# huawei-noah/Speech-Backbones

Measured on NVIDIA B200. Metric: mel-frames/sec at N=50 reverse-diffusion steps, higher is better.
Workload: dtype f32

## Files before the change

### speech-backbones_b200/csrc/sbk_api.cu

```cuda
#include "../../include/sbk.h"
#include "sbk_internal.h"

#include <cuda_fp16.h>
#include <math.h>
#include <stdarg.h>
#include <stdio.h>
#include <stdlib.h>
#include <string.h>

#include <algorithm>
#include <map>
#include <string>
#include <vector>

using namespace sbk;

static thread_local char g_err[1024] = "";
static int fail(int code, const char* fmt, ...) {
    va_list ap;
    va_start(ap, fmt);
    vsnprintf(g_err, sizeof(g_err), fmt, ap);
    va_end(ap);
    return code;
}
int sbk_set_error(int code, const char* fmt, ...) {
    va_list ap;
    va_start(ap, fmt);
    vsnprintf(g_err, sizeof(g_err), fmt, ap);
    va_end(ap);
    return code;
}
#define CU(x)                                                                                          \
    do {                                                                                               \
        cudaError_t e_ = (x);                                                                          \
        if (e_ != cudaSuccess)                                                                         \
            return fail(SBK_ERR_CUDA, "%s failed: %s (%s:%d)", #x, cudaGetErrorString(e_), __FILE__, __LINE__); \
    } while (0)

#define TRY_RC(x) do { int rc__ = (x); if (rc__ != SBK_OK) return rc__; } while (0)

namespace {

struct WSpec { std::string name; std::vector<int64_t> shape; };
struct ResnetInfo { std::string prefix; int cin, cout; };
struct AttnInfo { std::string prefix; int c; };

__global__ void k_set_int(int* p, int v) { *p = v; }
__global__ void k_set_ptr(const float** p, const float* v) { *p = v; }
__global__ void k_loop_cond(cudaGraphConditionalHandle handle, const int* step_next, const int* step_end) {
    cudaGraphSetConditional(handle, *step_next < *step_end ? 1u : 0u);
}

struct Arena {
    char* base = nullptr; size_t cap = 0, off = 0;
    void* take(size_t bytes) {
        off = (off + 255) & ~size_t(255);
        void* r = base ? base + off : nullptr;
        off += bytes;
        return r;
    }
};

enum OpKind { OP_FIRST, OP_IGEMM, OP_RESFINAL, OP_CTX, OP_MIX, OP_FINAL, OP_CONVTC, OP_GNACT };
struct Op {
    OpKind kind; std::string name;
    FirstConvParams fc; IgemmParams ig; ConvTcParams tc; GnActParams ga; ResFinalParams rf; AttnCtxParams cx; AttnMixParams mx; FinalParams fn;
    const float* dbg_ptr = nullptr; int64_t dbg_numel = 0;
    int dbg_fmt = 0;
    double flops = 0, bytes = 0;
    float* dbg_copy = nullptr;
};

struct Plan {
    int B = 0, T = 0, tb_rows = 0, noise_cap_steps = 0;
    void* mem = nullptr; size_t bytes = 0, cap = 0;
    std::vector<Op> ops;
    int final_op = -1;
    float *xt = nullptr, *mu = nullptr, *mask = nullptr, *spk_s = nullptr, *spk_in = nullptr;
    double* stats = nullptr; int n_stat_doubles = 0;
    float *tb = nullptr, *t_rows = nullptr; float4* coef = nullptr;
    int* step_cur = nullptr; int* step_next = nullptr;
    const float** noise_pp = nullptr;
    float *vc_cond = nullptr, *vc_wextra = nullptr, *vc_rextra = nullptr;
    int first_op = -1, first_res_op = -1;
    int tb_stride = 0;
    cudaGraphExec_t gexec[4] = {nullptr, nullptr, nullptr, nullptr};
    cudaGraphExec_t gloop[4] = {nullptr, nullptr, nullptr, nullptr};
    int loop_state[4] = {0, 0, 0, 0};
    int* step_end = nullptr;
    int launches_per_step = 0;
};

}

struct sbk_handle {
    sbk_config cfg;
    std::vector<WSpec> spec;
    std::vector<ResnetInfo> resnets;
    std::vector<AttnInfo> attns;
    std::map<std::string, float*> raw;
    std::map<std::string, float*> packed;
    std::vector<void*> owned;
    float* d_freqs = nullptr;
    float* d_zero = nullptr;
    void* ref_mem = nullptr; size_t ref_bytes = 0;
    bool is_packed = false;
    Plan plan;
    cudaStream_t cap_stream = nullptr;
    int64_t last_launches = 0;
    int last_host_launches = 0;
    bool capture = false;
    int tb_off[16];
    int tb_total = 0;
};

static void build_spec(sbk_handle* h) {
    const sbk_config& c = h->cfg;
    const int dim = c.dim;
    const bool vc = c.model == SBK_MODEL_DIFFVC;
    const int d[4] = {vc ? 2 + c.dim_cond : 2 + (c.n_spks > 1 ? 1 : 0), dim, dim * 2, dim * 4};
    auto add = [&](const std::string& n, std::vector<int64_t> s) { h->spec.push_back({n, s}); };
    auto resnet = [&](const std::string& p, int cin, int cout) {
        add(p + ".mlp.1.weight", {cout, dim});
        add(p + ".mlp.1.bias", {cout});
        const char* blk[2] = {"block1", "block2"};
        for (int k = 0; k < 2; ++k) {
            const int ci = k == 0 ? cin : cout;
            add(p + "." + blk[k] + ".block.0.weight", {cout, ci, 3, 3});
            add(p + "." + blk[k] + ".block.0.bias", {cout});
            add(p + "." + blk[k] + ".block.1.weight", {cout});
            add(p + "." + blk[k] + ".block.1.bias", {cout});
        }
        if (cin != cout) {
            add(p + ".res_conv.weight", {cout, cin, 1, 1});
            add(p + ".res_conv.bias", {cout});
        }
        h->resnets.push_back({p, cin, cout});
    };
    auto attn = [&](const std::string& p, int ch) {
        add(p + ".fn.g", {1});
        add(p + ".fn.fn.to_qkv.weight", {kAttnHidden * 3, ch, 1, 1});
        add(p + ".fn.fn.to_out.weight", {ch, kAttnHidden, 1, 1});
        add(p + ".fn.fn.to_out.bias", {ch});
        h->attns.push_back({p, ch});
    };
    if (c.n_spks > 1) {
        add("estimator.spk_mlp.0.weight", {c.spk_emb_dim * 4, c.spk_emb_dim});
        add("estimator.spk_mlp.0.bias", {c.spk_emb_dim * 4});
        add("estimator.spk_mlp.2.weight", {c.n_feats, c.spk_emb_dim * 4});
        add("estimator.spk_mlp.2.bias", {c.n_feats});
    }
    add("estimator.mlp.0.weight", {dim * 4, dim});
    add("estimator.mlp.0.bias", {dim * 4});
    add("estimator.mlp.2.weight", {dim, dim * 4});
    add("estimator.mlp.2.bias", {dim});
    if (vc) {
        const int dc = c.dim_cond, base = dc / 4;
        int cond_total = dim + 256;
        if (c.use_ref_t) {
            add("estimator.ref_block.mlp1.1.weight", {base, dim}); add("estimator.ref_block.mlp1.1.bias", {base});
            add("estimator.ref_block.mlp2.1.weight", {2 * base, dim}); add("estimator.ref_block.mlp2.1.bias", {2 * base});
            const char* nm[6] = {"block11", "block12", "block21", "block22", "block31", "block32"};
            const int ci[6] = {1, base, base, 2 * base, 2 * base, 4 * base}, co[6] = {2 * base, 2 * base, 4 * base, 4 * base, 8 * base, 8 * base};
            for (int k = 0; k < 6; ++k) {
                const std::string q = std::string("estimator.ref_block.") + nm[k];
                add(q + ".0.weight", {co[k], ci[k], 3, 3}); add(q + ".0.bias", {co[k]});
                add(q + ".1.weight", {co[k]}); add(q + ".1.bias", {co[k]});
            }
            add("estimator.ref_block.final_conv.weight", {dc, 4 * base, 1, 1});
            add("estimator.ref_block.final_conv.bias", {dc});
            cond_total += dc;
        }
        add("estimator.cond_block.0.weight", {4 * dc, cond_total}); add("estimator.cond_block.0.bias", {4 * dc});
        add("estimator.cond_block.2.weight", {dc, 4 * dc}); add("estimator.cond_block.2.bias", {dc});
    }
    for (int l = 0; l < 3; ++l) {
        const std::string p = "estimator.downs." + std::to_string(l);
        resnet(p + ".0", d[l], d[l + 1]);
        resnet(p + ".1", d[l + 1], d[l + 1]);
        attn(p + ".2", d[l + 1]);
        if (l < 2) {
            add(p + ".3.conv.weight", {d[l + 1], d[l + 1], 3, 3});
            add(p + ".3.conv.bias", {d[l + 1]});
        }
    }
    resnet("estimator.mid_block1", d[3], d[3]);
    attn("estimator.mid_attn", d[3]);
    resnet("estimator.mid_block2", d[3], d[3]);
    const int up_in[2] = {d[2], d[1]}, up_out[2] = {d[3], d[2]};
    for (int j = 0; j < 2; ++j) {
        const std::string p = "estimator.ups." + std::to_string(j);
        resnet(p + ".0", up_out[j] * 2, up_in[j]);
        resnet(p + ".1", up_in[j], up_in[j]);
        attn(p + ".2", up_in[j]);
        add(p + ".3.conv.weight", {up_in[j], up_in[j], 4, 4});
        add(p + ".3.conv.bias", {up_in[j]});
    }
    add("estimator.final_block.block.0.weight", {dim, dim, 3, 3});
    add("estimator.final_block.block.0.bias", {dim});
    add("estimator.final_block.block.1.weight", {dim});
    add("estimator.final_block.block.1.bias", {dim});
    add("estimator.final_conv.weight", {1, dim, 1, 1});
    add("estimator.final_conv.bias", {1});
    int off = 0;
    for (size_t k = 0; k < h->resnets.size(); ++k) { h->tb_off[k] = off; off += h->resnets[k].cout; }
    h->tb_total = off;
}

static int64_t numel_of(const std::vector<int64_t>& s) { int64_t n = 1; for (auto v : s) n *= v; return n; }

extern "C" const char* sbk_last_error(void) { return g_err; }
extern "C" const char* sbk_version(void) { return "sbk 0.1 (sm_100a)"; }

extern "C" int sbk_create(const sbk_config* cfg, sbk_handle** out) {
    if (!cfg || !out) return fail(SBK_ERR_ARG, "sbk_create: null argument");
    if (cfg->model != SBK_MODEL_GRADTTS && cfg->model != SBK_MODEL_DIFFVC) return fail(SBK_ERR_UNSUPPORTED, "sbk_create: model %d not supported", cfg->model);
    if (cfg->model == SBK_MODEL_DIFFVC && (cfg->dim_cond <= 0 || cfg->dim_cond % 4 != 0)) return fail(SBK_ERR_ARG, "sbk_create: DiffVC needs dim_cond > 0 (multiple of 4), got %d", cfg->dim_cond);
    if (cfg->model == SBK_MODEL_DIFFVC && cfg->use_ref_t && cfg->dim_cond % 128 != 0)
        return fail(SBK_ERR_ARG, "sbk_create: the native RefBlock needs dim_cond to be a multiple of 128 (its first conv writes 64-channel "
                                 "tiles and every conv reads 32-channel K stages), got %d", cfg->dim_cond);
    if (cfg->dim <= 0 || cfg->dim % 64 != 0) return fail(SBK_ERR_ARG, "sbk_create: dim must be a positive multiple of 64 (got %d)", cfg->dim);
    if (cfg->n_feats <= 0 || cfg->n_feats % 4 != 0) return fail(SBK_ERR_ARG, "sbk_create: n_feats must be a multiple of 4 (two stride-2 levels), got %d", cfg->n_feats);
    if (cfg->n_spks < 1 || cfg->spk_emb_dim <= 0) return fail(SBK_ERR_ARG, "sbk_create: bad speaker configuration");
    if (cfg->precision < SBK_PREC_FP32 || cfg->precision > SBK_PREC_FP32X3) return fail(SBK_ERR_ARG, "sbk_create: unknown precision %d", cfg->precision);
    sbk_handle* h = new sbk_handle();
    h->cfg = *cfg;
    build_spec(h);
    *out = h;
    return SBK_OK;
}

static void free_plan(sbk_handle* h, bool release_arena = true) {
    Plan& p = h->plan;
    for (int i = 0; i < 4; ++i) if (p.gexec[i]) { cudaGraphExecDestroy(p.gexec[i]); p.gexec[i] = nullptr; }
    for (int i = 0; i < 4; ++i) if (p.gloop[i]) { cudaGraphExecDestroy(p.gloop[i]); p.gloop[i] = nullptr; }
    for (auto& op : p.ops) if (op.dbg_copy) cudaFree(op.dbg_copy);
    void* mem = p.mem; const size_t cap = p.cap;
    if (mem && release_arena) { cudaFree(mem); mem = nullptr; }
    p = Plan();
    if (mem) { p.mem = mem; p.cap = cap; }
}

extern "C" void sbk_destroy(sbk_handle* h) {
    if (!h) return;
    free_plan(h);
    for (auto& kv : h->raw) cudaFree(kv.second);
    for (void* p : h->owned) cudaFree(p);
    if (h->ref_mem) cudaFree(h->ref_mem);
    if (h->cap_stream) cudaStreamDestroy(h->cap_stream);
    delete h;
}

extern "C" int sbk_num_weights(const sbk_handle* h) { return h ? (int)h->spec.size() : 0; }
extern "C" const char* sbk_weight_name(const sbk_handle* h, int i) {
    if (!h || i < 0 || i >= (int)h->spec.size()) return nullptr;
    return h->spec[i].name.c_str();
}

extern "C" int sbk_set_weight(sbk_handle* h, const char* name, const void* data, const int64_t* shape, int ndim) {
    if (!h || !name || !data || !shape) return fail(SBK_ERR_ARG, "sbk_set_weight: null argument");
    const WSpec* ws = nullptr;
    for (auto& s : h->spec) if (s.name == name) { ws = &s; break; }
    if (!ws) return fail(SBK_ERR_ARG, "sbk_set_weight: unexpected key '%s' (strict)", name);
    if ((int)ws->shape.size() != ndim) return fail(SBK_ERR_ARG, "sbk_set_weight: '%s' rank %d, expected %d", name, ndim, (int)ws->shape.size());
    for (int i = 0; i < ndim; ++i)
        if (ws->shape[i] != shape[i]) return fail(SBK_ERR_ARG, "sbk_set_weight: '%s' dim %d is %lld, expected %lld", name, i, (long long)shape[i], (long long)ws->shape[i]);
    CU(cudaSetDevice(h->cfg.device));
    const size_t bytes = numel_of(ws->shape) * sizeof(float);
    float*& dst = h->raw[name];
    if (!dst) CU(cudaMalloc(&dst, bytes));
    CU(cudaMemcpy(dst, data, bytes, cudaMemcpyDefault));
    h->is_packed = false;
    return SBK_OK;
}

template <class F>
static int repack(sbk_handle* h, const std::string& src, const std::string& key, size_t out_floats, F f) {
    const WSpec* ws = nullptr;
    for (auto& s : h->spec) if (s.name == src) { ws = &s; break; }
    if (!ws) return fail(SBK_ERR_STATE, "repack: no spec for %s", src.c_str());
    std::vector<float> hs(numel_of(ws->shape)), hd(out_floats);
    CU(cudaMemcpy(hs.data(), h->raw[src], hs.size() * sizeof(float), cudaMemcpyDeviceToHost));
    f(hd.data(), hs.data(), ws->shape);
    float*& d = h->packed[key];
    if (!d) { CU(cudaMalloc(&d, out_floats * sizeof(float))); h->owned.push_back(d); }
    CU(cudaMemcpy(d, hd.data(), out_floats * sizeof(float), cudaMemcpyHostToDevice));
    return SBK_OK;
}

static int attn_x3_chunk_items(int items_per_sample, int B) {
    (void)items_per_sample; (void)B;
    return 4;
}

static uint32_t f32_to_tf32_rna(float x) {
    uint32_t u; memcpy(&u, &x, 4);
    if ((u & 0x7F800000u) != 0x7F800000u) u += 0x1000u;
    return u & 0xFFFFE000u;
}
static uint16_t f32_to_f16_rn(float x) {
    if (x > 65504.f) x = 65504.f;
    if (x < -65504.f) x = -65504.f;
    const __half h = __float2half_rn(x);
    uint16_t u; memcpy(&u, &h, 2);
    return u;
}
static uint16_t f32_to_bf16_rn(float x) {
    uint32_t u; memcpy(&u, &x, 4);
    if ((u & 0x7FFFFFFFu) > 0x7F800000u) return (uint16_t)((u >> 16) | 0x40);
    u += 0x7FFFu + ((u >> 16) & 1u);
    return (uint16_t)(u >> 16);
}
static int pack_tc_host(sbk_handle* h, const std::vector<float>& hs, const std::string& key, int cout, int cin, int geom, bool bf16, int nt_override = 0);
static bool packs_x3(const sbk_handle* h) { return h->cfg.precision == SBK_PREC_FP32X3 || h->cfg.precision == SBK_PREC_FP32; }
static int pack_tc_rs(sbk_handle* h, const std::vector<float>& hs, const std::string& key, int cout, int cin, bool bf16) {
    const bool x3 = !bf16 && packs_x3(h);
    const int NT = 64, CPS = conv_tc_stage_channels(G_C3, bf16 ? 1 : 0), EPC = bf16 ? 8 : 4, KCHK = CPS / EPC, ksteps = cin / CPS;
    const size_t esz = bf16 ? 2 : 4, img = (size_t)3 * KCHK * 3 * NT * EPC;
    std::vector<uint8_t> hd((size_t)cout * cin * 9 * esz * (x3 ? 2 : 1));
    for (int nt = 0; nt < cout / NT; ++nt) for (int ks = 0; ks < ksteps; ++ks) for (int sx = 0; sx < 3; ++sx)
        for (int k = 0; k < KCHK; ++k) for (int kr = 0; kr < 3; ++kr) for (int col = 0; col < NT; ++col) for (int e = 0; e < EPC; ++e) {
            const int co = nt * NT + col, ci = ks * CPS + k * EPC + e;
            const float w = hs[((size_t)co * cin + ci) * 9 + kr * 3 + sx];
            const size_t in_img = ((((size_t)sx * KCHK + k) * 3 + (2 - kr)) * NT + col) * EPC + e;
            const size_t stage = ((size_t)nt * ksteps + ks) * (x3 ? 2 : 1);
            if (x3) {
                const uint32_t uh = f32_to_tf32_rna(w);
                float fh; memcpy(&fh, &uh, 4);
                reinterpret_cast<uint32_t*>(hd.data())[stage * img + in_img] = uh;
                uint16_t* cc = reinterpret_cast<uint16_t*>(hd.data()) + 2 * ((stage + 1) * img + in_img - e);
                cc[e] = f32_to_f16_rn(w);
                cc[4 + e] = f32_to_f16_rn((w - fh) * 4096.f);
            } else if (bf16) {
                reinterpret_cast<uint16_t*>(hd.data())[stage * img + in_img] = f32_to_bf16_rn(w);
            } else {
                reinterpret_cast<uint32_t*>(hd.data())[stage * img + in_img] = f32_to_tf32_rna(w);
            }
        }
    float*& d = h->packed[key];
    if (!d) { CU(cudaMalloc(&d, hd.size())); h->owned.push_back(d); }
    CU(cudaMemcpy(d, hd.data(), hd.size(), cudaMemcpyHostToDevice));
    return SBK_OK;
}
static int pack_tc(sbk_handle* h, const std::string& src, const std::string& key, int cout, int cin, int geom, bool bf16) {
    const int taps = conv_tc_taps(geom);
    std::vector<float> hs((size_t)cout * cin * taps);
    CU(cudaMemcpy(hs.data(), h->raw[src], hs.size() * sizeof(float), cudaMemcpyDeviceToHost));
    TRY_RC(pack_tc_host(h, hs, key, cout, cin, geom, bf16));
    if (geom == G_C3 && conv_tc_ntile(geom, cout) == 128) TRY_RC(pack_tc_host(h, hs, key + "64", cout, cin, geom, bf16, 64));
    if (geom == G_C3 && conv_tc_ntile(geom, cout) == 64) TRY_RC(pack_tc_host(h, hs, key + "32", cout, cin, geom, bf16, 32));
    if (geom == G_C3 && conv_tc_ntile(geom, cout) == 64) TRY_RC(pack_tc_rs(h, hs, key + "rs", cout, cin, bf16));
    return SBK_OK;
}
static int pack_tc_kv(sbk_handle* h, const std::string& src, const std::string& key, int C, bool bf16) {
    std::vector<float> q((size_t)384 * C);
    CU(cudaMemcpy(q.data(), h->raw[src], q.size() * sizeof(float), cudaMemcpyDeviceToHost));
    const int EPC = bf16 ? 8 : 4, CPS = 8 * EPC;
    std::vector<uint8_t> m((size_t)256 * C * (bf16 ? 2 : 4));
    for (int ks = 0; ks < C / CPS; ++ks) for (int kv = 0; kv < 2; ++kv) for (int k = 0; k < 8; ++k)
        for (int row = 0; row < 128; ++row) for (int e = 0; e < EPC; ++e) {
            const size_t idx = ((((size_t)ks * 2 + kv) * 8 + k) * 128 + row) * EPC + e;
            const float w = q[(size_t)(128 + kv * 128 + row) * C + ks * CPS + k * EPC + e];
            if (bf16) reinterpret_cast<uint16_t*>(m.data())[idx] = f32_to_bf16_rn(w);
            else reinterpret_cast<uint32_t*>(m.data())[idx] = f32_to_tf32_rna(w);
        }
    float*& d = h->packed[key];
    if (!d) { CU(cudaMalloc(&d, m.size())); h->owned.push_back(d); }
    CU(cudaMemcpy(d, m.data(), m.size(), cudaMemcpyHostToDevice));
    return SBK_OK;
}
static int pack_tc_kvx(sbk_handle* h, const std::string& src, const std::string& key, int C) {
    std::vector<float> q((size_t)384 * C);
    CU(cudaMemcpy(q.data(), h->raw[src], q.size() * sizeof(float), cudaMemcpyDeviceToHost));
    std::vector<uint8_t> m((size_t)2 * 256 * C * 4);
    for (int ks = 0; ks < C / 32; ++ks) for (int kv = 0; kv < 2; ++kv) for (int k = 0; k < 8; ++k)
        for (int row = 0; row < 128; ++row) for (int e = 0; e < 4; ++e) {
            const size_t chunk_hi = (((((size_t)ks * 2 + 0) * 2 + kv) * 8 + k) * 128 + row) * 4;
            const size_t chunk_c = (((((size_t)ks * 2 + 1) * 2 + kv) * 8 + k) * 128 + row) * 4;
            const float w = q[(size_t)(128 + kv * 128 + row) * C + ks * 32 + k * 4 + e];
            const uint32_t uh = f32_to_tf32_rna(w);
            float fh; memcpy(&fh, &uh, 4);
            reinterpret_cast<uint32_t*>(m.data())[chunk_hi + e] = uh;
            uint16_t* cc = reinterpret_cast<uint16_t*>(m.data()) + 2 * chunk_c;
            cc[e] = f32_to_f16_rn(w);
            cc[4 + e] = f32_to_f16_rn((w - fh) * 4096.f);
        }
    float*& d = h->packed[key];
    if (!d) { CU(cudaMalloc(&d, m.size())); h->owned.push_back(d); }
    CU(cudaMemcpy(d, m.data(), m.size(), cudaMemcpyHostToDevice));
    return SBK_OK;
}
static int pack_tc_up(sbk_handle* h, const std::string& src, const std::string& key, int C, bool bf16) {
    std::vector<float> w((size_t)C * C * 16), m((size_t)C * C * 16);
    CU(cudaMemcpy(w.data(), h->raw[src], w.size() * sizeof(float), cudaMemcpyDeviceToHost));
    for (int ci = 0; ci < C; ++ci) for (int co = 0; co < C; ++co) for (int t = 0; t < 16; ++t)
        m[((size_t)co * C + ci) * 16 + t] = w[((size_t)ci * C + co) * 16 + t];
    return pack_tc_host(h, m, key, C, C, G_UP, bf16);
}
static int pack_tc_host(sbk_handle* h, const std::vector<float>& hs, const std::string& key, int cout, int cin, int geom, bool bf16, int nt_override) {
    const int taps = conv_tc_taps(geom);
    const bool x3 = !bf16 && packs_x3(h);
    const int NT = nt_override ? nt_override : (x3 ? conv_tc_ntile_x3(geom, cout) : conv_tc_ntile(geom, cout)), CPS = conv_tc_stage_channels(geom, bf16 ? 1 : 0), EPC = bf16 ? 8 : 4, KCHK = CPS / EPC;
    const int ksteps = cin / CPS;
    const size_t esz = bf16 ? 2 : 4;
    std::vector<uint8_t> hd((size_t)cout * cin * taps * esz * (x3 ? 2 : 1));
    for (int nt = 0; nt < cout / NT; ++nt) for (int ks = 0; ks < ksteps; ++ks) for (int tap = 0; tap < taps; ++tap)
        for (int k = 0; k < KCHK; ++k) for (int col = 0; col < NT; ++col) for (int e = 0; e < EPC; ++e) {
            const int co = nt * NT + col, ci = ks * CPS + k * EPC + e;
            const float w = hs[((size_t)co * cin + ci) * taps + tap];
            if (x3) {
                const size_t ih = ((((((size_t)nt * ksteps + ks) * 2) * taps + tap) * KCHK + k) * NT + col) * EPC + e;
                const uint32_t uh = f32_to_tf32_rna(w);
                float fh; memcpy(&fh, &uh, 4);
                reinterpret_cast<uint32_t*>(hd.data())[ih] = uh;
                uint16_t* cc = reinterpret_cast<uint16_t*>(hd.data()) + 2 * ((ih - e) + (size_t)taps * KCHK * NT * EPC);
                cc[e] = f32_to_f16_rn(w);
                cc[4 + e] = f32_to_f16_rn((w - fh) * 4096.f);
                continue;
            }
            const size_t idx = (((((size_t)nt * ksteps + ks) * taps + tap) * KCHK + k) * NT + col) * EPC + e;
            if (bf16) reinterpret_cast<uint16_t*>(hd.data())[idx] = f32_to_bf16_rn(w);
            else reinterpret_cast<uint32_t*>(hd.data())[idx] = f32_to_tf32_rna(w);
        }
    float*& d = h->packed[key];
    if (!d) { CU(cudaMalloc(&d, hd.size())); h->owned.push_back(d); }
    CU(cudaMemcpy(d, hd.data(), hd.size(), cudaMemcpyHostToDevice));
    return SBK_OK;
}

#define TRY(x) do { int rc_ = (x); if (rc_ != SBK_OK) return rc_; } while (0)

extern "C" int sbk_pack(sbk_handle* h) {
    if (!h) return fail(SBK_ERR_ARG, "sbk_pack: null handle");
    for (auto& s : h->spec)
        if (!h->raw.count(s.name)) return fail(SBK_ERR_STATE, "sbk_pack: missing key '%s' (strict)", s.name.c_str());
    CU(cudaSetDevice(h->cfg.device));
    auto conv_pack = [](float* d, const float* s, const std::vector<int64_t>& sh) {
        const int64_t co = sh[0], ci = sh[1], kk = sh[2] * sh[3];
        for (int64_t o = 0; o < co; ++o) for (int64_t i = 0; i < ci; ++i) for (int64_t t = 0; t < kk; ++t)
            d[(t * ci + i) * co + o] = s[(o * ci + i) * kk + t];
    };
    auto convt_pack = [](float* d, const float* s, const std::vector<int64_t>& sh) {
        const int64_t ci = sh[0], co = sh[1], kk = sh[2] * sh[3];
        for (int64_t i = 0; i < ci; ++i) for (int64_t o = 0; o < co; ++o) for (int64_t t = 0; t < kk; ++t)
            d[(t * ci + i) * co + o] = s[(i * co + o) * kk + t];
    };
    auto first_pack = [](float* d, const float* s, const std::vector<int64_t>& sh) {
        const int64_t co = sh[0], ci = sh[1];
        for (int64_t o = 0; o < co; ++o) for (int64_t i = 0; i < ci; ++i) for (int64_t t = 0; t < 9; ++t)
            d[(i * 9 + t) * co + o] = s[(o * ci + i) * 9 + t];
    };
    auto kv_pack = [](float* d, const float* s, const std::vector<int64_t>& sh) {
        const int64_t C = sh[1];
        for (int64_t ci = 0; ci < C; ++ci) for (int hd = 0; hd < kHeads; ++hd) for (int x = 0; x < 32; ++x) {
            d[ci * 256 + hd * 64 + x] = s[(128 + hd * 32 + x) * C + ci];
            d[ci * 256 + hd * 64 + 32 + x] = s[(256 + hd * 32 + x) * C + ci];
        }
    };
    for (size_t k = 0; k < h->resnets.size(); ++k) {
        const ResnetInfo& r = h->resnets[k];
        if (k == 0) TRY(repack(h, r.prefix + ".block1.block.0.weight", r.prefix + ".block1.w", (size_t)r.cin * 9 * r.cout, first_pack));
        else TRY(repack(h, r.prefix + ".block1.block.0.weight", r.prefix + ".block1.w", (size_t)r.cin * 9 * r.cout, conv_pack));
        TRY(repack(h, r.prefix + ".block2.block.0.weight", r.prefix + ".block2.w", (size_t)r.cout * 9 * r.cout, conv_pack));
        if (r.cin != r.cout) TRY(repack(h, r.prefix + ".res_conv.weight", r.prefix + ".res.w", (size_t)r.cin * r.cout, conv_pack));
    }
    const bool x3 = h->cfg.precision == SBK_PREC_FP32X3;
    if (h->cfg.precision != SBK_PREC_FP32) {
        const bool bf = h->cfg.precision == SBK_PREC_BF16;
        const int cps3 = conv_tc_stage_channels(G_C3, bf ? 1 : 0), cps1 = conv_tc_stage_channels(G_PW, bf ? 1 : 0);
        for (auto& r : h->resnets) {
            if (r.cin % cps3 == 0) TRY(pack_tc(h, r.prefix + ".block1.block.0.weight", r.prefix + ".block1.wtc", r.cout, r.cin, G_C3, bf));
            TRY(pack_tc(h, r.prefix + ".block2.block.0.weight", r.prefix + ".block2.wtc", r.cout, r.cout, G_C3, bf));
            if (r.cin != r.cout && r.cin % cps1 == 0) TRY(pack_tc(h, r.prefix + ".res_conv.weight", r.prefix + ".res.wtc", r.cout, r.cin, G_PW, bf));
        }
        TRY(pack_tc(h, "estimator.final_block.block.0.weight", "estimator.final_block.wtc", h->cfg.dim, h->cfg.dim, G_C3, bf));
        for (auto& a : h->attns)
            if (a.c % cps1 == 0) {
                if (x3) TRY(pack_tc_kvx(h, a.prefix + ".fn.fn.to_qkv.weight", a.prefix + ".kvx.wtc", a.c));
                else TRY(pack_tc_kv(h, a.prefix + ".fn.fn.to_qkv.weight", a.prefix + ".kv.wtc", a.c, bf));
            }
        for (int l = 0; l < 2; ++l) {
            const std::string p = "estimator.downs." + std::to_string(l) + ".3.conv";
            TRY(pack_tc(h, p + ".weight", p + ".wtc", h->cfg.dim << l, h->cfg.dim << l, G_DOWN, bf));
        }
        for (int j = 0; j < 2; ++j) {
            const std::string p = "estimator.ups." + std::to_string(j) + ".3.conv";
            TRY(pack_tc_up(h, p + ".weight", p + ".wtc", h->cfg.dim << (1 - j), bf));
        }
    }
    if (h->cfg.model == SBK_MODEL_DIFFVC && h->cfg.use_ref_t) {
        const int base = h->cfg.dim_cond / 4;
        const char* nm[5] = {"block12", "block21", "block22", "block31", "block32"};
        const int ci[5] = {base, base, 2 * base, 2 * base, 4 * base}, co[5] = {2 * base, 4 * base, 4 * base, 8 * base, 8 * base};
        for (int k = 0; k < 5; ++k) {
            const std::string q = std::string("estimator.ref_block.") + nm[k];
            TRY(pack_tc(h, q + ".0.weight", q + ".wtc", co[k], ci[k], G_C3, false));
        }
        TRY(repack(h, "estimator.ref_block.block11.0.weight", "estimator.ref_block.block11.w", (size_t)9 * 2 * base, first_pack));
    }
    for (auto& a : h->attns) TRY(repack(h, a.prefix + ".fn.fn.to_qkv.weight", a.prefix + ".kv.w", (size_t)a.c * 256, kv_pack));
    for (int l = 0; l < 2; ++l) {
        const std::string p = "estimator.downs." + std::to_string(l) + ".3.conv";
        const int c = h->cfg.dim << l;
        TRY(repack(h, p + ".weight", p + ".w", (size_t)c * c * 9, conv_pack));
    }
    for (int j = 0; j < 2; ++j) {
        const std::string p = "estimator.ups." + std::to_string(j) + ".3.conv";
        const int c = h->cfg.dim << (1 - j);
        TRY(repack(h, p + ".weight", p + ".w", (size_t)c * c * 16, convt_pack));
    }
    TRY(repack(h, "estimator.final_block.block.0.weight", "estimator.final_block.w", (size_t)h->cfg.dim * h->cfg.dim * 9, conv_pack));
    {
        const int half = h->cfg.dim / 2;
        std::vector<float> f(half);
        const float neg = (float)(-(log(10000.0) / (double)(half - 1)));
        for (int j = 0; j < half; ++j) f[j] = expf((float)j * neg);
        if (!h->d_freqs) { CU(cudaMalloc(&h->d_freqs, half * sizeof(float))); h->owned.push_back(h->d_freqs); }
        CU(cudaMemcpy(h->d_freqs, f.data(), half * sizeof(float), cudaMemcpyHostToDevice));
    }
    if (!h->d_zero) {
        CU(cudaMalloc(&h->d_zero, 8192));
        h->owned.push_back(h->d_zero);
        CU(cudaMemset(h->d_zero, 0, 8192));
    }
    free_plan(h, false);
    h->is_packed = true;
    return SBK_OK;
}

namespace {
struct Bufs {
    float *A[3], *Bf[3], *X[3], *Y[3], *S[3], *D[3], *U1;
    float *kv_part, *ctx, *w_eff, *b_eff;
    std::map<const void*, float*> lo;
};
}

static size_t layout(const sbk_handle* h, int B, int T, int tb_rows, Arena& ar, Bufs* bf, Plan* pl) {
    const sbk_config& c = h->cfg;
    const int dim = c.dim, H = c.n_feats;
    const size_t P[3] = {(size_t)H * T, (size_t)(H / 2) * (T / 2), (size_t)(H / 4) * (T / 4)};
    const int C[3] = {dim, dim * 2, dim * 4};
    auto f = [&](size_t n) { return (float*)ar.take(n * sizeof(float)); };
    const size_t osz = c.precision == SBK_PREC_BF16 ? 2 : 4;
    const bool x3 = c.precision == SBK_PREC_FP32X3;
    Bufs b{};
    auto fo = [&](size_t n) {
        float* r = (float*)ar.take(n * osz);
        if (x3) { float* l = (float*)ar.take(n * osz); if (r) b.lo[r] = l; }
        return r;
    };
    for (int l = 0; l < 3; ++l) {
        const size_t n = (size_t)B * P[l] * C[l];
        b.A[l] = f(n); b.Bf[l] = fo(n); b.X[l] = fo(n); b.Y[l] = fo(n);
        b.S[l] = l > 0 ? fo(n) : nullptr;
        b.D[l] = l > 0 ? fo((size_t)B * P[l] * C[l - 1]) : nullptr;
    }
    b.U1 = fo((size_t)B * P[1] * C[1]);
    size_t mt0 = (P[0] + 127) / 128;
    if (x3) {
        mt0 = 0;
        for (int l = 0; l < 3; ++l) {
            const int items = (int)((P[l] + attn_kv_x3_item_pixels() - 1) / attn_kv_x3_item_pixels());
            const int ci = attn_x3_chunk_items(items, B);
            mt0 = std::max(mt0, (size_t)((items + ci - 1) / ci));
        }
    }
    b.kv_part = f((size_t)B * mt0 * kHeads * kKvPartFloats);
    b.ctx = f((size_t)B * kHeads * 1024);
    b.w_eff = f((size_t)B * C[2] * C[2] * (x3 ? 2 : 1));
    b.b_eff = f(C[2]);
    if (bf) *bf = b;
    Plan dummy;
    Plan& p = pl ? *pl : dummy;
    p.xt = f((size_t)B * H * T); p.mu = f((size_t)B * H * T); p.mask = f((size_t)B * T);
    p.spk_s = f((size_t)B * H); p.spk_in = f((size_t)B * c.spk_emb_dim);
    p.n_stat_doubles = 25 * B * kGroups * 2;
    p.stats = (double*)ar.take(p.n_stat_doubles * sizeof(double));
    p.tb_stride = h->tb_total;
    p.tb = f((size_t)tb_rows * h->tb_total);
    p.t_rows = f(tb_rows);
    p.coef = (float4*)ar.take((size_t)tb_rows * sizeof(float4));
    p.step_cur = (int*)ar.take(sizeof(int));
    p.step_next = (int*)ar.take(sizeof(int));
    p.step_end = (int*)ar.take(sizeof(int));
    p.noise_pp = (const float**)ar.take(sizeof(float*));
    if (c.model == SBK_MODEL_DIFFVC) {
        p.vc_cond = f((size_t)tb_rows * B * c.dim_cond);
        p.vc_wextra = f((size_t)tb_rows * B * 9 * dim);
        p.vc_rextra = f((size_t)tb_rows * B * dim);
    }
    return ar.off + 256;
}

static int table_rows(int B, int n_timesteps) { const int r = B > n_timesteps ? B : n_timesteps; return r < 64 ? 64 : r; }

extern "C" size_t sbk_workspace_bytes_n(const sbk_handle* h, int B, int T, int n_timesteps) {
    if (!h || B <= 0 || T <= 0 || T % 4 != 0 || n_timesteps < 1) return 0;
    Arena ar;
    return layout(h, B, T, table_rows(B, n_timesteps), ar, nullptr, nullptr);
}
extern "C" size_t sbk_workspace_bytes(const sbk_handle* h, int B, int T) { return sbk_workspace_bytes_n(h, B, T, 1024); }

static int build_plan(sbk_handle* h, int B, int T, int tb_rows) {
    free_plan(h, false);
    Plan& pl = h->plan;
    const sbk_config& c = h->cfg;
    Arena probe;
    const size_t bytes = layout(h, B, T, tb_rows, probe, nullptr, nullptr);
    if (bytes > pl.cap) {
        if (pl.mem) { cudaFree(pl.mem); pl.mem = nullptr; pl.cap = 0; }
        const cudaError_t e = cudaMalloc(&pl.mem, bytes);
        if (e != cudaSuccess) {
            pl.mem = nullptr;
            cudaGetLastError();
            return fail(SBK_ERR_CUDA, "out of memory: the (B=%d, T=%d) workspace needs %zu bytes (%s); free cached blocks "
                                      "(torch.cuda.empty_cache()) or split the batch", B, T, bytes, cudaGetErrorString(e));
        }
        pl.cap = bytes;
    }
    pl.bytes = bytes;
    Arena ar; ar.base = (char*)pl.mem; ar.cap = bytes;
    Bufs bf;
    layout(h, B, T, tb_rows, ar, &bf, &pl);
    pl.B = B; pl.T = T; pl.tb_rows = tb_rows;

    const int dim = c.dim, H0 = c.n_feats;
    const int Hs[3] = {H0, H0 / 2, H0 / 4}, Ws[3] = {T, T / 2, T / 4};
    const bool vc = c.model == SBK_MODEL_DIFFVC;
    const int cin0 = vc ? 3 : 2 + (c.n_spks > 1 ? 1 : 0);
    int gn_slot = 0;
    auto stats_slot = [&]() { return pl.stats + (size_t)(gn_slot++) * B * kGroups * 2; };
    auto W = [&](const std::string& k) -> const float* {
        auto it = h->packed.find(k);
        if (it != h->packed.end()) return it->second;
        auto it2 = h->raw.find(k);
        return it2 != h->raw.end() ? it2->second : nullptr;
    };
    auto gnref = [&](const double* st, const std::string& blk, int C, int lvl) {
        GnRef g; g.stats = st; g.gamma = W(blk + ".block.1.weight"); g.beta = W(blk + ".block.1.bias");
        g.inv_count = 1.0f / ((float)(C / kGroups) * (float)Hs[lvl] * (float)Ws[lvl]);
        return g;
    };
    auto base_ig = [&](int geom, int lvl_in, int lvl_out) {
        IgemmParams p; memset(&p, 0, sizeof(p));
        p.geom = geom; p.B = B; p.T = T;
        p.Hin = Hs[lvl_in]; p.Win = Ws[lvl_in]; p.Hout = Hs[lvl_out]; p.Wout = Ws[lvl_out];
        p.in_lvl = lvl_in; p.out_lvl = lvl_out; p.mask = pl.mask; p.step = pl.step_cur;
        return p;
    };
    const bool use_tc = c.precision != SBK_PREC_FP32;
    const bool x3 = c.precision == SBK_PREC_FP32X3;
    auto LO = [&](const void* q) -> float* { auto it = bf.lo.find(q); return it == bf.lo.end() ? nullptr : it->second; };
    int num_sms = 148;
    cudaDeviceGetAttribute(&num_sms, cudaDevAttrMultiProcessorCount, c.device);
    const bool b16 = c.precision == SBK_PREC_BF16;
    const double osz = b16 ? 2.0 : 4.0;
    const int fmt_raw = use_tc ? 1 : 0, fmt_opnd = b16 ? 2 : fmt_raw;
    const int tc_cps3 = conv_tc_stage_channels(G_C3, b16 ? 1 : 0), tc_cps1 = conv_tc_stage_channels(G_PW, b16 ? 1 : 0);
    auto push = [&](Op& op, const float* dbg, int64_t numel) {
        op.dbg_ptr = dbg; op.dbg_numel = numel;
        const bool raw_out = op.kind == OP_FIRST || op.kind == OP_CTX || (op.kind == OP_CONVTC && op.tc.geom == G_C3) ||
                             (op.kind == OP_IGEMM && op.ig.epi == EPI_PLAIN && op.ig.ostats);
        op.dbg_fmt = raw_out ? fmt_raw : fmt_opnd;
        if (op.kind == OP_IGEMM) {
            const IgemmParams& p = op.ig;
            const double cin = p.c0 + p.c1, opx = (double)B * p.Hout * p.Wout, ipx = (double)B * p.Hin * p.Win;
            const double taps = p.geom == G_PW ? 1 : (p.geom == G_UP ? 4 : 9);
            op.flops = 2.0 * opx * p.Cout * cin * taps;
            op.bytes = 4.0 * (ipx * cin + (p.epi == EPI_KV ? 0.0 : opx * p.Cout) + (p.epi == EPI_RES ? opx * p.Cout : 0.0));
        } else if (op.kind == OP_FIRST) {
            op.flops = 2.0 * B * H0 * T * op.fc.C * op.fc.cin * 9;
            op.bytes = 4.0 * B * H0 * T * (op.fc.cin + op.fc.C);
        } else if (op.kind == OP_RESFINAL) {
            op.bytes = (4.0 + (op.rf.x ? osz : 0.0) + osz) * B * op.rf.H * op.rf.W * op.rf.C;
        } else if (op.kind == OP_FINAL) {
            op.flops = 2.0 * B * H0 * T * op.fn.C;
            op.bytes = 4.0 * B * H0 * T * (op.fn.C + 3.0);
        }
        pl.ops.push_back(op);
    };
    auto npix = [&](int lvl) { return (int64_t)B * Hs[lvl] * Ws[lvl]; };

    auto tc_conv = [&](const std::string& name, int geom, const std::string& wkey, const std::string& bkey, int lvl,
                       const float* in0, int c0, const float* in1, int c1, int cout, float* out, double* st) {
        Op op; op.name = name; op.kind = OP_CONVTC;
        ConvTcParams& p = op.tc; memset(&p, 0, sizeof(p));
        p.geom = geom; p.in0 = in0; p.c0 = c0; p.in1 = in1; p.c1 = c1; p.H = Hs[lvl]; p.W = Ws[lvl]; p.B = B;
        p.Ho = p.H; p.Wo = p.W;
        p.wpk = W(wkey); p.bias = bkey.empty() ? nullptr : W(bkey); p.out = out; p.Cout = cout;
        p.epi = EPI_PLAIN; p.ostats = st; p.mask = pl.mask; p.T = T; p.lvl = lvl; p.zero_page = h->d_zero;
        p.bf16 = b16 ? 1 : 0;
        if (x3) {
            p.x3 = 1; p.in0_lo = LO(in0); p.in1_lo = LO(in1); p.out_lo = geom != G_C3 ? LO(out) : nullptr;
            static const int flush_env = getenv("SBK_X3_FLUSH") ? atoi(getenv("SBK_X3_FLUSH")) : 0;
            p.flush = flush_env;
        }
        if (geom == G_C3 && conv_tc_ntile(geom, cout) == 128 && getenv("SBK_FORCE_PAIR") == nullptr) {
            const long long tiles = (long long)B * ((Ws[lvl] + 127) / 128) * ((Hs[lvl] + 1) / 2) * (cout / 128);
            if (tiles * 2 <= num_sms && h->packed.count(wkey + "64")) { p.nt = 64; p.wpk = W(wkey + "64"); }
        }
        if (geom == G_C3 && conv_tc_ntile(geom, cout) == 64 && h->packed.count(wkey + "rs") && getenv("SBK_FORCE_PAIR") == nullptr &&
            ((!x3 && getenv("SBK_NO_RS") == nullptr) || getenv("SBK_FORCE_RS") != nullptr)) {
            p.rs = 1; p.wpk = W(wkey + "rs");
        }
        if (geom == G_C3 && !p.nt && !p.rs) {
            const bool no_pair = getenv("SBK_NO_PAIR") != nullptr, force_pair = getenv("SBK_FORCE_PAIR") != nullptr;
            const int ntile = conv_tc_ntile(geom, cout);
            const std::string half = wkey + (ntile == 128 ? "64" : "32");
            const long long ptiles = (long long)B * conv_tc_pair_tiles(Hs[lvl], Ws[lvl]) * (cout / ntile);
            if (!no_pair && h->packed.count(half) && (force_pair || (!b16 && ptiles >= num_sms / 2))) { p.pair = 1; p.wpk = W(half); }
        }
        const double taps = geom == G_PW ? 1.0 : (geom == G_UP ? 4.0 : 9.0);
        op.flops = 2.0 * B * Hs[lvl] * Ws[lvl] * cout * (c0 + c1) * taps;
        op.bytes = (double)B * Hs[lvl] * Ws[lvl] * (osz * (c0 + c1) + (geom == G_C3 ? 4.0 : osz) * cout);
        return op;
    };
    auto ffma_block_conv = [&](const std::string& name, const std::string& wkey, const std::string& bkey, int lvl,
                               const float* in0, int c0, const float* in1, int c1, int cout, float* out, double* st,
                               int pro, const GnRef* pgn, int tb_k) {
        Op op; op.name = name; op.kind = OP_IGEMM;
        op.ig = base_ig(G_C3, lvl, lvl);
        IgemmParams& p = op.ig;
        p.in0 = in0; p.c0 = c0; p.in1 = in1; p.c1 = c1; p.w = W(wkey); p.bias = W(bkey);
        p.out = out; p.Cout = cout; p.pro = pro; p.epi = EPI_PLAIN; p.ostats = st;
        if (pgn) { p.pgn = *pgn; p.tb = pl.tb + h->tb_off[tb_k]; p.tb_stride = pl.tb_stride; }
        push(op, out, npix(lvl) * cout);
    };
    auto resnet = [&](int k, int lvl, const float* in0, int c0, const float* in1, int c1, float* out, bool store_masked) {
        const ResnetInfo& r = h->resnets[k];
        float* A = bf.A[lvl]; float* Bb = bf.Bf[lvl];
        double* st1 = stats_slot(); double* st2 = stats_slot();
        const bool tc1 = use_tc && k != 0 && (c0 + c1) % tc_cps3 == 0 && c0 % tc_cps3 == 0;
        if (k == 0) {
            Op op; op.kind = OP_FIRST; op.name = r.prefix + ".block1.raw";
            FirstConvParams& p = op.fc; memset(&p, 0, sizeof(p));
            p.mu = pl.mu; p.xt = pl.xt; p.spk_s = pl.spk_s; p.mask = pl.mask;
            p.w = W(r.prefix + ".block1.w"); p.bias = W(r.prefix + ".block1.block.0.bias");
            p.out = A; p.ostats = st1; p.B = B; p.H = H0; p.T = T; p.cin = cin0; p.C = r.cout; p.chw4 = use_tc ? 1 : 0;
            if (vc) { p.w_extra = pl.vc_wextra; p.step = pl.step_cur; }
            pl.first_op = (int)pl.ops.size();
            push(op, A, npix(lvl) * r.cout);
        } else if (tc1) {
            Op op = tc_conv(r.prefix + ".block1.raw", G_C3, r.prefix + ".block1.wtc", r.prefix + ".block1.block.0.bias", lvl,
                            in0, c0, in1, c1, r.cout, A, st1);
            push(op, A, npix(lvl) * r.cout);
        } else {
            ffma_block_conv(r.prefix + ".block1.raw", r.prefix + ".block1.w", r.prefix + ".block1.block.0.bias", lvl,
                            in0, c0, in1, c1, r.cout, A, st1, PRO_MASK, nullptr, k);
        }
        const GnRef g1 = gnref(st1, r.prefix + ".block1", r.cout, lvl);
        float* h2 = Bb;
        if (use_tc) {
            {
                Op op; op.kind = OP_GNACT; op.name = r.prefix + ".block1.act";
                GnActParams& p = op.ga; memset(&p, 0, sizeof(p));
                p.raw = A; p.gn = g1; p.tb = pl.tb + h->tb_off[k]; p.tb_stride = pl.tb_stride; p.step = pl.step_cur;
                p.mask = pl.mask; p.T = T; p.lvl = lvl; p.out = Bb; p.B = B; p.H = Hs[lvl]; p.W = Ws[lvl]; p.C = r.cout;
                p.round_tf32 = (b16 || x3) ? 0 : 1; p.chw4 = 1; p.out_bf16 = b16 ? 1 : 0; p.out_lo = LO(Bb);
                op.bytes = (4.0 + osz) * npix(lvl) * r.cout;
                push(op, nullptr, 0);
            }
            Op op = tc_conv(r.prefix + ".block2.raw", G_C3, r.prefix + ".block2.wtc", r.prefix + ".block2.block.0.bias", lvl,
                            Bb, r.cout, nullptr, 0, r.cout, A, st2);
            push(op, A, npix(lvl) * r.cout);
            h2 = A;
        } else {
            ffma_block_conv(r.prefix + ".block2.raw", r.prefix + ".block2.w", r.prefix + ".block2.block.0.bias", lvl,
                            A, r.cout, nullptr, 0, r.cout, Bb, st2, PRO_GN, &g1, k);
        }
        const GnRef g2 = gnref(st2, r.prefix + ".block2", r.cout, lvl);
        if (k == 0 || r.cin == r.cout) {
            Op op; op.kind = OP_RESFINAL; op.name = r.prefix + ".out";
            ResFinalParams& p = op.rf; memset(&p, 0, sizeof(p));
            p.h2raw = h2; p.gn = g2;
            p.mask = pl.mask; p.T = T; p.lvl = lvl; p.out = out; p.B = B; p.H = Hs[lvl]; p.W = Ws[lvl]; p.C = r.cout;
            p.out_mask = store_masked ? 1 : 0; p.chw4 = use_tc ? 1 : 0; p.bf16 = b16 ? 1 : 0; p.out_lo = LO(out);
            if (k == 0) {
                p.x = nullptr; p.mu = pl.mu; p.xt = pl.xt; p.spk_s = pl.spk_s; p.cin = cin0;
                p.wres = W(r.prefix + ".res.w"); p.bres = W(r.prefix + ".res_conv.bias");
                if (vc) { p.r_extra = pl.vc_rextra; p.step = pl.step_cur; }
                pl.first_res_op = (int)pl.ops.size();
            } else {
                p.x = in0;
            }
            op.bytes = (4.0 + (k == 0 ? 0.0 : osz) + osz) * npix(lvl) * r.cout;
            push(op, out, npix(lvl) * r.cout);
        } else if (use_tc && (c0 + c1) % tc_cps1 == 0 && c0 % tc_cps1 == 0) {
            Op op = tc_conv(r.prefix + ".out", G_PW, r.prefix + ".res.wtc", r.prefix + ".res_conv.bias", lvl,
                            in0, c0, in1, c1, r.cout, out, nullptr);
            op.tc.epi = EPI_RES; op.tc.rraw = h2; op.tc.rgn = g2; op.tc.out_mask = store_masked ? 1 : 0;
            op.bytes += 4.0 * npix(lvl) * r.cout;
            push(op, out, npix(lvl) * r.cout);
        } else {
            Op op; op.kind = OP_IGEMM; op.name = r.prefix + ".out";
            op.ig = base_ig(G_PW, lvl, lvl);
            IgemmParams& p = op.ig;
            p.in0 = in0; p.c0 = c0; p.in1 = in1; p.c1 = c1;
            p.w = W(r.prefix + ".res.w"); p.bias = W(r.prefix + ".res_conv.bias");
            p.out = out; p.Cout = r.cout; p.pro = PRO_MASK; p.epi = EPI_RES;
            p.rraw = h2; p.rgn = g2; p.out_mask = store_masked ? 1 : 0;
            push(op, out, npix(lvl) * r.cout);
        }
    };
    auto attention = [&](int k, int lvl, const float* x, float* out) {
        const AttnInfo& a = h->attns[k];
        int mt = igemm_mtiles(G_PW, Hs[lvl], Ws[lvl], Hs[lvl], Ws[lvl]);
        const bool tc_apply = use_tc && a.c % tc_cps1 == 0;
        if (tc_apply && x3) {
            Op op = tc_conv(a.prefix + ".kvpart", G_PW, a.prefix + ".kvx.wtc", "", lvl, x, a.c, nullptr, 0, 256, nullptr, nullptr);
            const int items = (Hs[lvl] * Ws[lvl] + attn_kv_x3_item_pixels() - 1) / attn_kv_x3_item_pixels();
            const int chunk_items = attn_x3_chunk_items(items, B);
            mt = (items + chunk_items - 1) / chunk_items;
            op.tc.epi = EPI_KV; op.tc.kv_part = bf.kv_part; op.tc.Ho = chunk_items; op.tc.Wo = mt;
            op.bytes = 8.0 * npix(lvl) * a.c;
            op.flops += 2.0 * npix(lvl) * 4096.0;
            push(op, nullptr, 0);
        } else if (tc_apply) {
            Op op = tc_conv(a.prefix + ".kvpart", G_PW, a.prefix + ".kv.wtc", "", lvl, x, a.c, nullptr, 0, 256, nullptr, nullptr);
            op.tc.epi = EPI_KV; op.tc.kv_part = bf.kv_part;
            op.bytes = osz * npix(lvl) * a.c;
            op.flops += 2.0 * npix(lvl) * 4096.0;
            mt = (Hs[lvl] * Ws[lvl] + attn_kv_tile_pixels() - 1) / attn_kv_tile_pixels();
            push(op, nullptr, 0);
        } else {
            Op op; op.kind = OP_IGEMM; op.name = a.prefix + ".kvpart";
            op.ig = base_ig(G_PW, lvl, lvl);
            IgemmParams& p = op.ig;
            p.in0 = x; p.c0 = a.c; p.w = W(a.prefix + ".kv.w"); p.Cout = 256; p.pro = PRO_NONE; p.epi = EPI_KV;
            p.kv_part = bf.kv_part; p.out = nullptr;
            push(op, nullptr, 0);
        }
        {
            Op op; op.kind = OP_CTX; op.name = a.prefix + ".ctx";
            op.cx.kv_part = bf.kv_part; op.cx.mtiles = mt; op.cx.ctx = bf.ctx; op.cx.B = B;
            push(op, bf.ctx, (int64_t)B * kHeads * 1024);
        }
        {
            Op op; op.kind = OP_MIX; op.name = a.prefix + ".mix";
            AttnMixParams& p = op.mx; memset(&p, 0, sizeof(p));
            p.ctx = bf.ctx; p.wq = W(a.prefix + ".fn.fn.to_qkv.weight"); p.wout = W(a.prefix + ".fn.fn.to_out.weight");
            p.bout = W(a.prefix + ".fn.fn.to_out.bias"); p.g = W(a.prefix + ".fn.g");
            p.w_eff = bf.w_eff; p.b_eff = bf.b_eff; p.B = B; p.C = a.c;
            if (tc_apply) { p.tc_nt = x3 ? conv_tc_ntile_x3(G_PW, a.c) : conv_tc_ntile(G_PW, a.c); p.tc_cps = tc_cps1; p.tc_bf16 = b16 ? 1 : 0; p.tc_x3 = x3 ? 1 : 0; }
            push(op, nullptr, 0);
        }
        if (tc_apply) {
            Op op = tc_conv(a.prefix + ".out", G_PW, "", "", lvl, x, a.c, nullptr, 0, a.c, out, nullptr);
            op.tc.wpk = bf.w_eff; op.tc.w_bstride_bytes = (long long)a.c * a.c * (b16 ? 2 : (x3 ? 8 : 4)); op.tc.bias = bf.b_eff;
            op.tc.out_mask = 1; op.tc.addin = x;
            op.bytes += osz * npix(lvl) * a.c;
            push(op, out, npix(lvl) * a.c);
        } else {
            Op op; op.kind = OP_IGEMM; op.name = a.prefix + ".out";
            op.ig = base_ig(G_PW, lvl, lvl);
            IgemmParams& p = op.ig;
            p.in0 = x; p.c0 = a.c; p.w = bf.w_eff; p.w_bstride = (long long)a.c * a.c; p.bias = bf.b_eff;
            p.out = out; p.Cout = a.c; p.pro = PRO_NONE; p.epi = EPI_PLAIN; p.out_mask = use_tc ? 1 : 0;
            push(op, out, npix(lvl) * a.c);
        }
    };
    auto resample = [&](int geom, const std::string& pre, int lvl_in, int lvl_out, const float* x, int C, float* out) {
        if (use_tc && C % tc_cps3 == 0 && C % 64 == 0) {
            Op op = tc_conv(pre + ".out", geom, pre + ".conv.wtc", pre + ".conv.bias", lvl_in, x, C, nullptr, 0, C, out, nullptr);
            op.tc.Ho = Hs[lvl_out]; op.tc.Wo = Ws[lvl_out]; op.tc.lvl = lvl_out; op.tc.out_mask = 1;
            op.flops = 2.0 * npix(lvl_out) * C * C * (geom == G_UP ? 4.0 : 9.0);
            op.bytes = osz * C * (npix(lvl_in) + npix(lvl_out));
            push(op, out, npix(lvl_out) * C);
            return;
        }
        Op op; op.kind = OP_IGEMM; op.name = pre + ".out";
        op.ig = base_ig(geom, lvl_in, lvl_out);
        IgemmParams& p = op.ig;
        p.in0 = x; p.c0 = C; p.w = W(pre + ".conv.w"); p.bias = W(pre + ".conv.bias");
        p.out = out; p.Cout = C; p.pro = PRO_MASK; p.epi = EPI_PLAIN; p.out_mask = use_tc ? 1 : 0;
        push(op, out, npix(lvl_out) * C);
    };

    const int C1 = dim, C2 = dim * 2, C3 = dim * 4;
    const bool sm = use_tc;
    resnet(0, 0, nullptr, cin0, nullptr, 0, bf.X[0], sm);
    resnet(1, 0, bf.X[0], C1, nullptr, 0, bf.Y[0], false);
    attention(0, 0, bf.Y[0], bf.X[0]);
    resample(G_DOWN, "estimator.downs.0.3", 0, 1, bf.X[0], C1, bf.D[1]);
    resnet(2, 1, bf.D[1], C1, nullptr, 0, bf.X[1], sm);
    resnet(3, 1, bf.X[1], C2, nullptr, 0, bf.Y[1], false);
    attention(1, 1, bf.Y[1], bf.S[1]);
    resample(G_DOWN, "estimator.downs.1.3", 1, 2, bf.S[1], C2, bf.D[2]);
    resnet(4, 2, bf.D[2], C2, nullptr, 0, bf.X[2], sm);
    resnet(5, 2, bf.X[2], C3, nullptr, 0, bf.Y[2], false);
    attention(2, 2, bf.Y[2], bf.S[2]);
    resnet(6, 2, bf.S[2], C3, nullptr, 0, bf.X[2], false);
    attention(3, 2, bf.X[2], bf.Y[2]);
    resnet(7, 2, bf.Y[2], C3, nullptr, 0, bf.X[2], sm);
    resnet(8, 2, bf.X[2], C3, bf.S[2], C3, bf.Y[2], sm);
    resnet(9, 2, bf.Y[2], C2, nullptr, 0, bf.X[2], false);
    attention(4, 2, bf.X[2], bf.Y[2]);
    resample(G_UP, "estimator.ups.0.3", 2, 1, bf.Y[2], C2, bf.U1);
    resnet(10, 1, bf.U1, C2, bf.S[1], C2, bf.X[1], sm);
    resnet(11, 1, bf.X[1], C1, nullptr, 0, bf.Y[1], false);
    attention(5, 1, bf.Y[1], bf.X[1]);
    resample(G_UP, "estimator.ups.1.3", 1, 0, bf.X[1], C1, bf.Y[0]);
    double* stf = stats_slot();
    if (use_tc) {
        Op op = tc_conv("estimator.final_block.raw", G_C3, "estimator.final_block.wtc", "estimator.final_block.block.0.bias", 0,
                        bf.Y[0], C1, nullptr, 0, C1, bf.A[0], stf);
        push(op, bf.A[0], npix(0) * C1);
    } else {
        ffma_block_conv("estimator.final_block.raw", "estimator.final_block.w", "estimator.final_block.block.0.bias", 0,
                        bf.Y[0], C1, nullptr, 0, C1, bf.A[0], stf, PRO_MASK, nullptr, 0);
    }
    {
        Op op; op.kind = OP_FINAL; op.name = "estimator.out";
        FinalParams& p = op.fn; memset(&p, 0, sizeof(p));
        p.raw = bf.A[0]; p.gn = gnref(stf, "estimator.final_block", C1, 0);
        p.wfin = W("estimator.final_conv.weight"); p.bfin = W("estimator.final_conv.bias");
        p.mask = pl.mask; p.mu = pl.mu; p.xt_in = pl.xt; p.xt_out = pl.xt;
        p.coef = pl.coef; p.step = pl.step_cur; p.B = B; p.H = H0; p.T = T; p.C = C1; p.chw4 = use_tc ? 1 : 0; p.exact = x3 ? 1 : 0;
        pl.final_op = (int)pl.ops.size();
        push(op, nullptr, 0);
    }
    pl.launches_per_step = (int)pl.ops.size() + 1;
    return SBK_OK;
}

static int launch_op(const Op& op, cudaStream_t s) {
    switch (op.kind) {
        case OP_FIRST: return launch_first_conv(op.fc, s);
        case OP_IGEMM: return launch_igemm(op.ig, s);
        case OP_RESFINAL: return launch_resfinal(op.rf, s);
        case OP_CTX: return launch_attn_ctx(op.cx, s);
        case OP_MIX: return launch_attn_mix(op.mx, s);
        case OP_FINAL: return launch_final(op.fn, s);
        case OP_CONVTC: return launch_conv_tc(op.tc, s);
        case OP_GNACT: return launch_gn_act(op.ga, s);
    }
    return -1;
}

static int run_ops(sbk_handle* h, cudaStream_t s) {
    Plan& pl = h->plan;
    StepBeginParams sb{pl.stats, pl.n_stat_doubles, pl.step_cur, pl.step_next};
    int n = launch_step_begin(sb, s);
    for (auto& op : pl.ops) {
        const int k = launch_op(op, s);
        if (k < 0) { fail(SBK_ERR_CUDA, "launch of '%s' was refused (device attribute / layout)", op.name.c_str()); return -1; }
        n += k;
        if (h->capture && op.dbg_ptr && op.dbg_numel > 0) {
            const size_t esz = op.dbg_fmt == 2 ? 2 : 4;
            if (!op.dbg_copy) cudaMalloc(&op.dbg_copy, op.dbg_numel * esz);
            cudaMemcpyAsync(op.dbg_copy, op.dbg_ptr, op.dbg_numel * esz, cudaMemcpyDeviceToDevice, s);
        }
    }
    return n;
}

static int ensure_plan(sbk_handle* h, int B, int T, int rows) {
    if (!h->is_packed) return fail(SBK_ERR_STATE, "weights not packed: call sbk_set_weight for every key, then sbk_pack");
    if (B <= 0 || T <= 0 || T % 4 != 0) return fail(SBK_ERR_ARG, "B must be > 0 and T a positive multiple of 4 (fix_len_compatibility), got B=%d T=%d", B, T);
    CU(cudaSetDevice(h->cfg.device));
    Plan& pl = h->plan;
    if (pl.mem && pl.B == B && pl.T == T && pl.tb_rows >= rows) return SBK_OK;
    int cap = rows < 64 ? 64 : rows;
    if (pl.mem && pl.B == B && pl.T == T && cap < pl.tb_rows) cap = pl.tb_rows;
    return build_plan(h, B, T, cap);
}

static int time_table(sbk_handle* h, int rows, cudaStream_t s) {
    Plan& pl = h->plan;
    TimeTableParams p; memset(&p, 0, sizeof(p));
    p.t_rows = pl.t_rows; p.rows = rows; p.freqs = h->d_freqs; p.pe_scale = h->cfg.pe_scale; p.dim = h->cfg.dim;
    p.w0 = h->raw["estimator.mlp.0.weight"]; p.b0 = h->raw["estimator.mlp.0.bias"];
    p.w2 = h->raw["estimator.mlp.2.weight"]; p.b2 = h->raw["estimator.mlp.2.bias"];
    p.nproj = (int)h->resnets.size();
    for (int k = 0; k < p.nproj; ++k) {
        p.pw[k] = h->raw[h->resnets[k].prefix + ".mlp.1.weight"];
        p.pb[k] = h->raw[h->resnets[k].prefix + ".mlp.1.bias"];
        p.pc[k] = h->resnets[k].cout; p.poff[k] = h->tb_off[k];
    }
    p.tb = pl.tb; p.tb_stride = pl.tb_stride;
    return launch_time_table(p, s);
}

static int speaker(sbk_handle* h, const float* spk, int B, cudaStream_t s) {
    if (h->cfg.n_spks < 2) return 0;
    Plan& pl = h->plan;
    SpkParams p; p.spk = spk; p.B = B; p.E = h->cfg.spk_emb_dim; p.n_feats = h->cfg.n_feats; p.out = pl.spk_s;
    p.w0 = h->raw["estimator.spk_mlp.0.weight"]; p.b0 = h->raw["estimator.spk_mlp.0.bias"];
    p.w2 = h->raw["estimator.spk_mlp.2.weight"]; p.b2 = h->raw["estimator.spk_mlp.2.bias"];
    return launch_spk(p, s);
}

static void set_mode(Plan& pl, int mode, bool per_sample_t, float* out) {
    for (auto& op : pl.ops)
        if (op.kind == OP_IGEMM && op.ig.pro == PRO_GN) op.ig.tb_per_sample = per_sample_t ? 1 : 0;
    for (auto& op : pl.ops)
        if (op.kind == OP_GNACT) op.ga.tb_per_sample = per_sample_t ? 1 : 0;
    if (pl.first_op >= 0) pl.ops[pl.first_op].fc.extra_per_sample_row = per_sample_t ? 1 : 0;
    if (pl.first_res_op >= 0) pl.ops[pl.first_res_op].rf.extra_per_sample_row = per_sample_t ? 1 : 0;
    FinalParams& f = pl.ops[pl.final_op].fn;
    f.mode = mode; f.xt_out = out; f.noise_pp = pl.noise_pp;
}

extern "C" int sbk_estimator(sbk_handle* h, const float* x, const float* mask, const float* mu, const float* t,
                             const float* spk, float* out, int B, int T, void* stream) {
    if (!h || !x || !mask || !mu || !t || !out) return fail(SBK_ERR_ARG, "sbk_estimator: null argument");
    if (h->cfg.model != SBK_MODEL_GRADTTS) return fail(SBK_ERR_ARG, "sbk_estimator: this handle is a DiffVC model, use sbk_vc_*");
    if (h->cfg.n_spks > 1 && !spk) return fail(SBK_ERR_ARG, "sbk_estimator: spk is required when n_spks > 1");
    TRY(ensure_plan(h, B, T, B));
    cudaStream_t s = (cudaStream_t)stream;
    Plan& pl = h->plan;
    const size_t nb = (size_t)B * h->cfg.n_feats * T * sizeof(float);
    CU(cudaMemcpyAsync(pl.xt, x, nb, cudaMemcpyDeviceToDevice, s));
    CU(cudaMemcpyAsync(pl.mu, mu, nb, cudaMemcpyDeviceToDevice, s));
    CU(cudaMemcpyAsync(pl.mask, mask, (size_t)B * T * sizeof(float), cudaMemcpyDeviceToDevice, s));
    CU(cudaMemcpyAsync(pl.t_rows, t, (size_t)B * sizeof(float), cudaMemcpyDeviceToDevice, s));
    int64_t n = 0;
    n += speaker(h, spk, B, s);
    n += time_table(h, B, s);
    set_mode(pl, 0, true, out);
    k_set_int<<<1, 1, 0, s>>>(pl.step_next, 0); ++n;
    { const int k = run_ops(h, s); if (k < 0) return SBK_ERR_CUDA; n += k; }
    CU(cudaGetLastError());
    h->last_launches = n;
    return SBK_OK;
}

static void step_coefs(const sbk_config& c, int n_timesteps, int i, float* t_out, float4* cf) {
    const double hd = 1.0 / n_timesteps;
    const float t = (float)(1.0 - (i + 0.5) * hd);
    const float beta = c.beta_min + (float)((double)c.beta_max - (double)c.beta_min) * t;
    const float hf = (float)hd;
    *t_out = t;
    *cf = make_float4(beta, hf, sqrtf(beta * hf), 0.f);
}

static bool build_loop_graph(sbk_handle* h, int mode) {
    Plan& pl = h->plan;
    if (pl.loop_state[mode] != 0) return pl.loop_state[mode] > 0;
    pl.loop_state[mode] = -1;
    if (!h->cap_stream && cudaStreamCreateWithFlags(&h->cap_stream, cudaStreamNonBlocking) != cudaSuccess) return false;
    cudaGraph_t g = nullptr;
    cudaGraphExec_t exec = nullptr;
    bool ok = false;
    do {
        if (cudaGraphCreate(&g, 0) != cudaSuccess) break;
        cudaGraphConditionalHandle handle;
        if (cudaGraphConditionalHandleCreate(&handle, g, 1, cudaGraphCondAssignDefault) != cudaSuccess) break;
        cudaGraphNodeParams np = {cudaGraphNodeTypeConditional};
        np.type = cudaGraphNodeTypeConditional;
        np.conditional.handle = handle;
        np.conditional.type = cudaGraphCondTypeWhile;
        np.conditional.size = 1;
        cudaGraphNode_t node;
        if (cudaGraphAddNode(&node, g, nullptr, 0, &np) != cudaSuccess) break;
        cudaGraph_t body = np.conditional.phGraph_out[0];
        if (cudaStreamBeginCaptureToGraph(h->cap_stream, body, nullptr, nullptr, 0, cudaStreamCaptureModeThreadLocal) != cudaSuccess) break;
        const int k = run_ops(h, h->cap_stream);
        k_loop_cond<<<1, 1, 0, h->cap_stream>>>(handle, pl.step_next, pl.step_end);
        cudaGraph_t dummy = nullptr;
        if (cudaStreamEndCapture(h->cap_stream, &dummy) != cudaSuccess || k < 0) break;
        if (cudaGraphInstantiate(&exec, g, 0) != cudaSuccess) break;
        ok = true;
    } while (0);
    if (!ok) {
        const cudaError_t e = cudaGetLastError();
        fail(SBK_ERR_CUDA, "single-launch loop graph unavailable (%s): falling back to one graph launch per step", cudaGetErrorString(e));
        if (exec) cudaGraphExecDestroy(exec);
    } else {
        pl.gloop[mode] = exec;
        pl.loop_state[mode] = 1;
    }
    if (g) cudaGraphDestroy(g);
    return ok;
}

static int run_steps(sbk_handle* h, const float* noise, int B, int T, int N, int s0, int s1, int stoc, cudaStream_t s, int64_t* launches) {
    Plan& pl = h->plan;
    const int mode = h->cfg.model == SBK_MODEL_DIFFVC ? 3 : (stoc ? 2 : 1);
    set_mode(pl, mode, false, pl.xt);
    const float* nbase = noise ? noise - (long long)s0 * B * h->cfg.n_feats * T : nullptr;
    k_set_int<<<1, 1, 0, s>>>(pl.step_next, s0);
    k_set_ptr<<<1, 1, 0, s>>>(pl.noise_pp, nbase);
    *launches += 2;
    h->last_host_launches = s1 - s0;
    if (h->cfg.use_graph && s1 > s0 && build_loop_graph(h, mode)) {
        k_set_int<<<1, 1, 0, s>>>(pl.step_end, s1);
        CU(cudaGraphLaunch(pl.gloop[mode], s));
        *launches += 1 + (int64_t)(s1 - s0) * (pl.launches_per_step + 1);
        h->last_host_launches = 1;
    } else if (h->cfg.use_graph) {
        if (!pl.gexec[mode]) {
            if (!h->cap_stream) CU(cudaStreamCreateWithFlags(&h->cap_stream, cudaStreamNonBlocking));
            cudaGraph_t g = nullptr;
            CU(cudaStreamBeginCapture(h->cap_stream, cudaStreamCaptureModeThreadLocal));
            const int k = run_ops(h, h->cap_stream);
            CU(cudaStreamEndCapture(h->cap_stream, &g));
            if (k < 0) { if (g) cudaGraphDestroy(g); return SBK_ERR_CUDA; }
            CU(cudaGraphInstantiate(&pl.gexec[mode], g, 0));
            CU(cudaGraphDestroy(g));
        }
        for (int i = s0; i < s1; ++i) CU(cudaGraphLaunch(pl.gexec[mode], s));
        *launches += (int64_t)(s1 - s0) * pl.launches_per_step;
    } else {
        for (int i = s0; i < s1; ++i) { const int k = run_ops(h, s); if (k < 0) return SBK_ERR_CUDA; *launches += k; }
    }
    CU(cudaGetLastError());
    (void)N;
    return SBK_OK;
}

static int prepare_loop(sbk_handle* h, const float* mask, const float* mu, const float* spk, int B, int T, int N,
                        cudaStream_t s, int64_t* launches) {
    Plan& pl = h->plan;
    const size_t nb = (size_t)B * h->cfg.n_feats * T * sizeof(float);
    if (mu != pl.mu) CU(cudaMemcpyAsync(pl.mu, mu, nb, cudaMemcpyDeviceToDevice, s));
    if (mask != pl.mask) CU(cudaMemcpyAsync(pl.mask, mask, (size_t)B * T * sizeof(float), cudaMemcpyDeviceToDevice, s));
    std::vector<float> tr(N); std::vector<float4> cf(N);
    for (int i = 0; i < N; ++i) step_coefs(h->cfg, N, i, &tr[i], &cf[i]);
    CU(cudaMemcpyAsync(pl.t_rows, tr.data(), N * sizeof(float), cudaMemcpyHostToDevice, s));
    CU(cudaMemcpyAsync(pl.coef, cf.data(), N * sizeof(float4), cudaMemcpyHostToDevice, s));
    *launches += speaker(h, spk, B, s);
    *launches += time_table(h, N, s);
    return SBK_OK;
}

extern "C" int sbk_reverse_steps(sbk_handle* h, float* xt, const float* mask, const float* mu, const float* spk,
                                 const float* noise, int B, int T, int n_timesteps, int step_begin, int step_end,
                                 int stoc, void* stream) {
    if (!h || !xt || !mask || !mu) return fail(SBK_ERR_ARG, "sbk_reverse_steps: null argument");
    if (n_timesteps < 1 || step_begin < 0 || step_end > n_timesteps || step_begin > step_end)
        return fail(SBK_ERR_ARG, "sbk_reverse_steps: bad step range [%d,%d) of %d", step_begin, step_end, n_timesteps);
    if (stoc && !noise) return fail(SBK_ERR_ARG, "sbk_reverse_steps: stoc=1 needs a noise buffer");
    if (h->cfg.model != SBK_MODEL_GRADTTS) return fail(SBK_ERR_ARG, "sbk_reverse_steps: this handle is a DiffVC model, use sbk_vc_*");
    if (h->cfg.n_spks > 1 && !spk) return fail(SBK_ERR_ARG, "sbk_reverse_steps: spk is required when n_spks > 1");
    TRY(ensure_plan(h, B, T, n_timesteps));
    cudaStream_t s = (cudaStream_t)stream;
    Plan& pl = h->plan;
    int64_t n = 0;
    const size_t nb = (size_t)B * h->cfg.n_feats * T * sizeof(float);
    CU(cudaMemcpyAsync(pl.xt, xt, nb, cudaMemcpyDeviceToDevice, s));
    TRY(prepare_loop(h, mask, mu, spk, B, T, n_timesteps, s, &n));
    TRY(run_steps(h, noise, B, T, n_timesteps, step_begin, step_end, stoc, s, &n));
    CU(cudaMemcpyAsync(xt, pl.xt, nb, cudaMemcpyDeviceToDevice, s));
    h->last_launches = n;
    return SBK_OK;
}

extern "C" int sbk_reverse_diffusion(sbk_handle* h, const float* z, const float* mask, const float* mu, const float* spk,
                                     const float* noise, float* out, int B, int T, int n_timesteps, int stoc, void* stream) {
    if (!h || !z || !mask || !mu || !out) return fail(SBK_ERR_ARG, "sbk_reverse_diffusion: null argument");
    if (n_timesteps < 1) return fail(SBK_ERR_ARG, "sbk_reverse_diffusion: n_timesteps must be >= 1");
    if (stoc && !noise) return fail(SBK_ERR_ARG, "sbk_reverse_diffusion: stoc=1 needs a noise buffer");
    if (h->cfg.model != SBK_MODEL_GRADTTS) return fail(SBK_ERR_ARG, "sbk_reverse_diffusion: this handle is a DiffVC model, use sbk_vc_*");
    if (h->cfg.n_spks > 1 && !spk) return fail(SBK_ERR_ARG, "sbk_reverse_diffusion: spk is required when n_spks > 1");
    TRY(ensure_plan(h, B, T, n_timesteps));
    cudaStream_t s = (cudaStream_t)stream;
    Plan& pl = h->plan;
    int64_t n = 0;
    const size_t nb = (size_t)B * h->cfg.n_feats * T * sizeof(float);
    TRY(prepare_loop(h, mask, mu, spk, B, T, n_timesteps, s, &n));
    n += launch_scale_mask(z, pl.mask, pl.xt, 0, B, h->cfg.n_feats, T, s);
    TRY(run_steps(h, noise, B, T, n_timesteps, 0, n_timesteps, stoc, s, &n));
    CU(cudaMemcpyAsync(out, pl.xt, nb, cudaMemcpyDeviceToDevice, s));
    h->last_launches = n;
    return SBK_OK;
}

extern "C" int sbk_reverse_diffusion_host(sbk_handle* h, const float* z, const float* mask, const float* mu, const float* spk,
                                          const float* noise, float* out, int B, int T, int n_timesteps, int stoc) {
    if (!h || !z || !mask || !mu || !out) return fail(SBK_ERR_ARG, "sbk_reverse_diffusion_host: null argument");
    if (n_timesteps < 1) return fail(SBK_ERR_ARG, "sbk_reverse_diffusion_host: n_timesteps must be >= 1");
    if (stoc && !noise) return fail(SBK_ERR_ARG, "sbk_reverse_diffusion_host: stoc=1 needs a noise buffer");
    if (h->cfg.model != SBK_MODEL_GRADTTS) return fail(SBK_ERR_ARG, "sbk_reverse_diffusion_host: this handle is a DiffVC model, use sbk_vc_*");
    if (h->cfg.n_spks > 1 && !spk) return fail(SBK_ERR_ARG, "sbk_reverse_diffusion_host: spk is required when n_spks > 1");
    TRY(ensure_plan(h, B, T, n_timesteps));
    if (!h->cap_stream) CU(cudaStreamCreateWithFlags(&h->cap_stream, cudaStreamNonBlocking));
    cudaStream_t s = h->cap_stream;
    Plan& pl = h->plan;
    const size_t nb = (size_t)B * h->cfg.n_feats * T * sizeof(float);
    float* d_z = nullptr; float* d_noise = nullptr;
    CU(cudaMallocAsync(&d_z, nb, s));
    CU(cudaMemcpyAsync(d_z, z, nb, cudaMemcpyHostToDevice, s));
    CU(cudaMemcpyAsync(pl.mu, mu, nb, cudaMemcpyHostToDevice, s));
    CU(cudaMemcpyAsync(pl.mask, mask, (size_t)B * T * sizeof(float), cudaMemcpyHostToDevice, s));
    if (spk) CU(cudaMemcpyAsync(pl.spk_in, spk, (size_t)B * h->cfg.spk_emb_dim * sizeof(float), cudaMemcpyHostToDevice, s));
    if (stoc) {
        CU(cudaMallocAsync(&d_noise, nb * n_timesteps, s));
        CU(cudaMemcpyAsync(d_noise, noise, nb * n_timesteps, cudaMemcpyHostToDevice, s));
    }
    int64_t n = 0;
    TRY(prepare_loop(h, pl.mask, pl.mu, spk ? pl.spk_in : nullptr, B, T, n_timesteps, s, &n));
    n += launch_scale_mask(d_z, pl.mask, pl.xt, 0, B, h->cfg.n_feats, T, s);
    TRY(run_steps(h, d_noise, B, T, n_timesteps, 0, n_timesteps, stoc, s, &n));
    CU(cudaMemcpyAsync(out, pl.xt, nb, cudaMemcpyDeviceToHost, s));
    CU(cudaFreeAsync(d_z, s));
    if (d_noise) CU(cudaFreeAsync(d_noise, s));
    CU(cudaStreamSynchronize(s));
    h->last_launches = n;
    return SBK_OK;
}

extern "C" int sbk_profile_ops(sbk_handle* h, float* ms, double* flops, double* bytes, int cap, int* n_ops) {
    if (!h || !ms || !n_ops) return fail(SBK_ERR_ARG, "sbk_profile_ops: null argument");
    Plan& pl = h->plan;
    if (pl.ops.empty()) return fail(SBK_ERR_STATE, "sbk_profile_ops: no plan yet (run a sampler call first)");
    const int n = (int)pl.ops.size();
    if (cap < n) return fail(SBK_ERR_ARG, "sbk_profile_ops: need room for %d launches", n);
    CU(cudaSetDevice(h->cfg.device));
    if (!h->cap_stream) CU(cudaStreamCreateWithFlags(&h->cap_stream, cudaStreamNonBlocking));
    cudaStream_t s = h->cap_stream;
    CU(cudaDeviceSynchronize());
    std::vector<cudaEvent_t> ev(n + 1);
    for (auto& e : ev) CU(cudaEventCreate(&e));
    StepBeginParams sb{pl.stats, pl.n_stat_doubles, pl.step_cur, pl.step_next};
    k_set_int<<<1, 1, 0, s>>>(pl.step_next, 0);
    launch_step_begin(sb, s);
    for (int i = 0; i < n; ++i) {
        CU(cudaEventRecord(ev[i], s));
        if (launch_op(pl.ops[i], s) < 0) return fail(SBK_ERR_CUDA, "sbk_profile_ops: launch of '%s' was refused", pl.ops[i].name.c_str());
    }
    CU(cudaEventRecord(ev[n], s));
    CU(cudaStreamSynchronize(s));
    CU(cudaGetLastError());
    for (int i = 0; i < n; ++i) {
        CU(cudaEventElapsedTime(&ms[i], ev[i], ev[i + 1]));
        if (flops) flops[i] = pl.ops[i].flops;
        if (bytes) bytes[i] = pl.ops[i].bytes;
    }
    for (auto& e : ev) cudaEventDestroy(e);
    *n_ops = n;
    return SBK_OK;
}

static void vc_step_coefs(const sbk_config& c, int N, int i, int mode, float* t_out, float4* cf) {
    const double h = 1.0 / N, t = 1.0 - i * h;
    const double bmin = c.beta_min, bmax = c.beta_max;
    auto gamma = [&](double s, double tt, double p) {
        double bi = bmin + 0.5 * (bmax - bmin) * (tt + s);
        bi *= (tt - s);
        return exp(-0.5 * p * bi);
    };
    const double beta_t = bmin + (bmax - bmin) * t;
    double A, Bc, sigma;
    if (mode == 0) { A = 0.5 * beta_t * h; Bc = 0.5 * beta_t * h; sigma = 0.0; }
    else if (mode == 2) {
        double kappa = gamma(0, t - h, 1.0) * (1.0 - gamma(t - h, t, 2.0));
        kappa /= (gamma(0, t, 1.0) * beta_t * h);
        kappa -= 1.0;
        const double ct = 1.0 - gamma(0, t, 2.0);
        const double nu = gamma(0, t - h, 1.0) * (1.0 - gamma(t - h, t, 2.0)) / ct;
        const double mu = gamma(t - h, t, 1.0) * (1.0 - gamma(0, t - h, 2.0)) / ct;
        double omega = nu / gamma(0, t, 1.0);
        omega += mu;
        omega -= (0.5 * beta_t * h + 1.0);
        sigma = sqrt((1.0 - gamma(0, t - h, 2.0)) * (1.0 - gamma(t - h, t, 2.0)) / ct);
        A = 0.5 * beta_t * h + omega; Bc = (1.0 + kappa) * (beta_t * h);
    } else { A = 0.5 * beta_t * h; Bc = beta_t * h; sigma = sqrt(beta_t * h); }
    *t_out = (float)t;
    *cf = make_float4((float)A, (float)Bc, (float)sigma, 0.f);
}

static int vc_fold(sbk_handle* h, const float* cond, int rows, int B, cudaStream_t s) {
    Plan& pl = h->plan;
    const sbk_config& c = h->cfg;
    CU(cudaMemcpyAsync(pl.vc_cond, cond, (size_t)rows * B * c.dim_cond * sizeof(float), cudaMemcpyDeviceToDevice, s));
    CondFoldParams p;
    p.cond = pl.vc_cond; p.w1 = h->raw["estimator.downs.0.0.block1.block.0.weight"];
    p.wres = h->raw["estimator.downs.0.0.res_conv.weight"];
    p.w_extra = pl.vc_wextra; p.r_extra = pl.vc_rextra; p.rows = rows; p.B = B; p.dc = c.dim_cond; p.C = c.dim;
    return launch_cond_fold(p, s);
}

extern "C" int sbk_vc_estimator(sbk_handle* h, const float* x, const float* mask, const float* mean, const float* cond,
                                const float* t, float* out, int B, int T, void* stream) {
    if (!h || !x || !mask || !mean || !cond || !t || !out) return fail(SBK_ERR_ARG, "sbk_vc_estimator: null argument");
    if (h->cfg.model != SBK_MODEL_DIFFVC) return fail(SBK_ERR_ARG, "sbk_vc_estimator: this handle is not a DiffVC model");
    TRY(ensure_plan(h, B, T, B));
    cudaStream_t s = (cudaStream_t)stream;
    Plan& pl = h->plan;
    const size_t nb = (size_t)B * h->cfg.n_feats * T * sizeof(float);
    CU(cudaMemcpyAsync(pl.xt, x, nb, cudaMemcpyDeviceToDevice, s));
    CU(cudaMemcpyAsync(pl.mu, mean, nb, cudaMemcpyDeviceToDevice, s));
    CU(cudaMemcpyAsync(pl.mask, mask, (size_t)B * T * sizeof(float), cudaMemcpyDeviceToDevice, s));
    CU(cudaMemcpyAsync(pl.t_rows, t, (size_t)B * sizeof(float), cudaMemcpyDeviceToDevice, s));
    int64_t n = 0;
    n += vc_fold(h, cond, 1, B, s);
    n += time_table(h, B, s);
    set_mode(pl, 0, true, out);
    k_set_int<<<1, 1, 0, s>>>(pl.step_next, 0); ++n;
    { const int k = run_ops(h, s); if (k < 0) return SBK_ERR_CUDA; n += k; }
    CU(cudaGetLastError());
    h->last_launches = n;
    return SBK_OK;
}

extern "C" int sbk_vc_reverse_diffusion(sbk_handle* h, const float* z, const float* mask, const float* mean, const float* cond,
                                        const float* noise, float* out, int B, int T, int n_timesteps, int mode, void* stream) {
    if (!h || !z || !mask || !mean || !cond || !out) return fail(SBK_ERR_ARG, "sbk_vc_reverse_diffusion: null argument");
    if (h->cfg.model != SBK_MODEL_DIFFVC) return fail(SBK_ERR_ARG, "sbk_vc_reverse_diffusion: this handle is not a DiffVC model");
    if (mode < 0 || mode > 2) return fail(SBK_ERR_ARG, "sbk_vc_reverse_diffusion: mode must be 0 (pf), 1 (em) or 2 (ml)");
    if (n_timesteps < 1) return fail(SBK_ERR_ARG, "sbk_vc_reverse_diffusion: n_timesteps must be >= 1");
    if (mode != 0 && !noise) return fail(SBK_ERR_ARG, "sbk_vc_reverse_diffusion: modes em/ml need a noise buffer");
    TRY(ensure_plan(h, B, T, n_timesteps));
    cudaStream_t s = (cudaStream_t)stream;
    Plan& pl = h->plan;
    const int N = n_timesteps;
    const size_t nb = (size_t)B * h->cfg.n_feats * T * sizeof(float);
    int64_t n = 0;
    CU(cudaMemcpyAsync(pl.mu, mean, nb, cudaMemcpyDeviceToDevice, s));
    CU(cudaMemcpyAsync(pl.mask, mask, (size_t)B * T * sizeof(float), cudaMemcpyDeviceToDevice, s));
    std::vector<float> tr(N); std::vector<float4> cf(N);
    for (int i = 0; i < N; ++i) vc_step_coefs(h->cfg, N, i, mode, &tr[i], &cf[i]);
    CU(cudaMemcpyAsync(pl.t_rows, tr.data(), N * sizeof(float), cudaMemcpyHostToDevice, s));
    CU(cudaMemcpyAsync(pl.coef, cf.data(), N * sizeof(float4), cudaMemcpyHostToDevice, s));
    n += vc_fold(h, cond, N, B, s);
    n += time_table(h, N, s);
    n += launch_scale_mask(z, pl.mask, pl.xt, 0, B, h->cfg.n_feats, T, s);
    TRY(run_steps(h, noise, B, T, N, 0, N, mode != 0, s, &n));
    CU(cudaMemcpyAsync(out, pl.xt, nb, cudaMemcpyDeviceToDevice, s));
    h->last_launches = n;
    return SBK_OK;
}

extern "C" int sbk_vc_conditioning(sbk_handle* h, const float* ref, const float* ref_mask, const float* mean_ref, const float* c,
                                   float* cond_out, int B, int Tr, int n_timesteps, void* stream) {
    if (!h || !ref || !ref_mask || !mean_ref || !c || !cond_out) return fail(SBK_ERR_ARG, "sbk_vc_conditioning: null argument");
    if (h->cfg.model != SBK_MODEL_DIFFVC) return fail(SBK_ERR_ARG, "sbk_vc_conditioning: this handle is not a DiffVC model");
    if (!h->is_packed) return fail(SBK_ERR_STATE, "sbk_vc_conditioning: weights not packed");
    if (h->cfg.use_ref_t && h->cfg.dim_cond % 128 != 0) return fail(SBK_ERR_ARG, "sbk_vc_conditioning: dim_cond must be a multiple of 128");
    const bool x3 = packs_x3(h);
    if (B <= 0 || Tr <= 0 || n_timesteps < 1) return fail(SBK_ERR_ARG, "sbk_vc_conditioning: bad sizes");
    CU(cudaSetDevice(h->cfg.device));
    cudaStream_t s = (cudaStream_t)stream;
    const sbk_config& cf = h->cfg;
    const int H = cf.n_feats, dc = cf.dim_cond, base = dc / 4, N = n_timesteps, dim = cf.dim;
    const size_t px = (size_t)B * H * Tr;
    Arena probe;
    float* act_lo = nullptr;
    auto carve = [&](Arena& ar, float*& xt_ref, float*& raw, float*& act, double*& st, double*& ys, float*& tb, float*& trows) {
        xt_ref = (float*)ar.take(px * sizeof(float));
        raw = (float*)ar.take(px * 8 * base * sizeof(float));
        act = (float*)ar.take(px * 4 * base * sizeof(float));
        act_lo = x3 ? (float*)ar.take(px * 4 * base * sizeof(float)) : nullptr;
        st = (double*)ar.take((size_t)B * 8 * base * 2 * sizeof(double));
        ys = (double*)ar.take((size_t)B * dc * 2 * sizeof(double));
        tb = (float*)ar.take((size_t)N * 3 * base * sizeof(float));
        trows = (float*)ar.take((size_t)N * sizeof(float));
    };
    float *xt_ref, *raw, *act, *tb, *trows; double *st, *ys;
    carve(probe, xt_ref, raw, act, st, ys, tb, trows);
    const size_t need = probe.off + 256;
    if (need > h->ref_bytes) {
        if (h->ref_mem) CU(cudaFree(h->ref_mem));
        h->ref_mem = nullptr; h->ref_bytes = 0;
        CU(cudaMalloc(&h->ref_mem, need));
        h->ref_bytes = need;
    }
    Arena ar; ar.base = (char*)h->ref_mem; ar.cap = h->ref_bytes;
    carve(ar, xt_ref, raw, act, st, ys, tb, trows);
    std::vector<float> tr(N);
    for (int i = 0; i < N; ++i) tr[i] = (float)(1.0 - i * (1.0 / N));
    CU(cudaMemcpyAsync(trows, tr.data(), N * sizeof(float), cudaMemcpyHostToDevice, s));
    int64_t n = 0;
    if (cf.use_ref_t) {
        TimeTableParams tp; memset(&tp, 0, sizeof(tp));
        tp.t_rows = trows; tp.rows = N; tp.freqs = h->d_freqs; tp.pe_scale = 1000.0f; tp.dim = dim;
        tp.w0 = h->raw["estimator.mlp.0.weight"]; tp.b0 = h->raw["estimator.mlp.0.bias"];
        tp.w2 = h->raw["estimator.mlp.2.weight"]; tp.b2 = h->raw["estimator.mlp.2.bias"];
        tp.nproj = 2;
        tp.pw[0] = h->raw["estimator.ref_block.mlp1.1.weight"]; tp.pb[0] = h->raw["estimator.ref_block.mlp1.1.bias"]; tp.pc[0] = base; tp.poff[0] = 0;
        tp.pw[1] = h->raw["estimator.ref_block.mlp2.1.weight"]; tp.pb[1] = h->raw["estimator.ref_block.mlp2.1.bias"]; tp.pc[1] = 2 * base; tp.poff[1] = base;
        tp.tb = tb; tp.tb_stride = 3 * base;
        n += launch_time_table(tp, s);
    }
    auto W = [&](const std::string& k) -> const float* {
        auto it = h->packed.find(k);
        if (it != h->packed.end()) return it->second;
        auto it2 = h->raw.find(k);
        return it2 != h->raw.end() ? it2->second : nullptr;
    };
    auto gamma0 = [&](double t) {
        double bi = cf.beta_min + 0.5 * ((double)cf.beta_max - cf.beta_min) * t;
        bi *= t;
        return exp(-0.5 * bi);
    };
    auto conv = [&](const char* name, int cin, int cout) {
        ConvTcParams p; memset(&p, 0, sizeof(p));
        const std::string q = std::string("estimator.ref_block.") + name;
        p.geom = G_C3; p.in0 = act; p.c0 = cin; p.H = H; p.W = Tr; p.B = B; p.Ho = H; p.Wo = Tr;
        p.wpk = W(q + ".wtc"); p.bias = W(q + ".0.bias"); p.out = raw; p.Cout = cout; p.epi = EPI_PLAIN;
        p.mask = ref_mask; p.T = Tr; p.zero_page = h->d_zero;
        if (x3) { p.x3 = 1; p.in0_lo = act_lo; }
        return launch_conv_tc(p, s);
    };
    auto norm_glu = [&](const char* name, int C, const float* tbias) {
        const std::string q = std::string("estimator.ref_block.") + name;
        ChanStatsParams cs{raw, st, B, H, Tr, C};
        int k = launch_chan_stats(cs, s);
        InGluParams g; memset(&g, 0, sizeof(g));
        g.raw = raw; g.stats = st; g.gamma = W(q + ".1.weight"); g.beta = W(q + ".1.bias"); g.tb = tbias;
        g.mask = ref_mask; g.T = Tr; g.out = act; g.out_lo = act_lo; g.B = B; g.H = H; g.W = Tr; g.C = C;
        return k + launch_in_glu(g, s);
    };
    for (int i = 0; i < N; ++i) {
        if (cf.use_ref_t) {
            DiffMeanParams dm{ref, mean_ref, ref_mask, xt_ref, (float)gamma0(1.0 - i * (1.0 / N)), B, H, Tr};
            n += launch_diff_mean(dm, s);
            FirstConvParams fc; memset(&fc, 0, sizeof(fc));
            fc.mu = xt_ref; fc.xt = xt_ref; fc.mask = ref_mask; fc.w = W("estimator.ref_block.block11.w");
            fc.bias = W("estimator.ref_block.block11.0.bias"); fc.out = raw; fc.ostats = nullptr;
            fc.B = B; fc.H = H; fc.T = Tr; fc.cin = 1; fc.C = 2 * base; fc.chw4 = 1;
            n += launch_first_conv(fc, s);
            n += norm_glu("block11", 2 * base, nullptr);
            n += conv("block12", base, 2 * base);
            n += norm_glu("block12", 2 * base, tb + (size_t)i * 3 * base);
            n += conv("block21", base, 4 * base);
            n += norm_glu("block21", 4 * base, nullptr);
            n += conv("block22", 2 * base, 4 * base);
            n += norm_glu("block22", 4 * base, tb + (size_t)i * 3 * base + base);
            n += conv("block31", 2 * base, 8 * base);
            n += norm_glu("block31", 8 * base, nullptr);
            n += conv("block32", 4 * base, 8 * base);
            n += norm_glu("block32", 8 * base, nullptr);
            ChanStatsParams ysm{act, ys, B, H, Tr, 4 * base};
            n += launch_chan_stats(ysm, s);
        }
        VcCondParams vp; memset(&vp, 0, sizeof(vp));
        vp.ysum = ys; vp.mask = ref_mask; vp.Tr = Tr; vp.H = H;
        vp.wf = W("estimator.ref_block.final_conv.weight"); vp.bf = W("estimator.ref_block.final_conv.bias");
        vp.c = c; vp.freqs = h->d_freqs; vp.t = tr[i]; vp.dim = dim;
        vp.w0 = W("estimator.cond_block.0.weight"); vp.b0 = W("estimator.cond_block.0.bias");
        vp.w2 = W("estimator.cond_block.2.weight"); vp.b2 = W("estimator.cond_block.2.bias");
        vp.out = cond_out + (size_t)i * B * dc; vp.B = B; vp.dc = dc; vp.use_ref = cf.use_ref_t ? 1 : 0;
        n += launch_vc_cond(vp, s);
    }
    CU(cudaGetLastError());
    h->last_launches = n;
    return SBK_OK;
}

extern "C" int sbk_prior_expand(const float* mu_x, const float* w_ceil, const float* x_mask, const int64_t* y_lengths,
                                const float* noise_tf, float temperature, int B, int F, int Tx, int Ty,
                                float* mu_y, float* z, float* y_mask, float* attn, void* stream) {
    if (!mu_x || !w_ceil || !x_mask || !y_lengths || !mu_y || !z || !y_mask) return fail(SBK_ERR_ARG, "sbk_prior_expand: null argument");
    if (B <= 0 || F <= 0 || Tx <= 0 || Ty <= 0) return fail(SBK_ERR_ARG, "sbk_prior_expand: bad sizes B=%d F=%d Tx=%d Ty=%d", B, F, Tx, Ty);
    if (Tx > 12000) return fail(SBK_ERR_ARG, "sbk_prior_expand: Tx=%d exceeds the 12000-token shared-memory table", Tx);
    if (noise_tf && !(temperature > 0.f)) return fail(SBK_ERR_ARG, "sbk_prior_expand: temperature must be > 0");
    PriorExpandParams p;
    p.mu_x = mu_x; p.w_ceil = w_ceil; p.x_mask = x_mask; p.y_len = reinterpret_cast<const long long*>(y_lengths);
    p.noise_tf = noise_tf; p.temperature = temperature; p.B = B; p.F = F; p.Tx = Tx; p.Ty = Ty;
    p.mu_y = mu_y; p.z = z; p.y_mask = y_mask; p.attn = attn;
    launch_prior_expand(p, (cudaStream_t)stream);
    CU(cudaGetLastError());
    return SBK_OK;
}

extern "C" int64_t sbk_last_launch_count(const sbk_handle* h) { return h ? h->last_launches : 0; }
extern "C" int sbk_last_host_launches(const sbk_handle* h) { return h ? h->last_host_launches : 0; }

extern "C" int sbk_debug_capture(sbk_handle* h, int on) {
    if (!h) return fail(SBK_ERR_ARG, "sbk_debug_capture: null handle");
    h->capture = on != 0;
    return SBK_OK;
}
extern "C" int sbk_debug_layout(const sbk_handle* h) { return (h && h->cfg.precision != SBK_PREC_FP32) ? 1 : 0; }
extern "C" int sbk_debug_op_layout(const sbk_handle* h, const char* name) {
    if (!h || !name) return -1;
    for (auto& op : h->plan.ops) if (op.name == name) return op.dbg_fmt;
    return -1;
}
extern "C" int sbk_debug_num(const sbk_handle* h) { return h ? (int)h->plan.ops.size() : 0; }
extern "C" const char* sbk_debug_name(const sbk_handle* h, int i) {
    if (!h || i < 0 || i >= (int)h->plan.ops.size()) return nullptr;
    return h->plan.ops[i].name.c_str();
}
extern "C" int sbk_debug_read(sbk_handle* h, const char* name, float* dst, int64_t* numel) {
    if (!h || !name) return fail(SBK_ERR_ARG, "sbk_debug_read: null argument");
    for (auto& op : h->plan.ops) {
        if (op.name != name) continue;
        if (numel) *numel = op.dbg_numel;
        if (dst && op.dbg_ptr && op.dbg_numel > 0) {
            CU(cudaDeviceSynchronize());
            const void* src = op.dbg_copy ? (const void*)op.dbg_copy : (const void*)op.dbg_ptr;
            if (op.dbg_fmt == 2) {
                std::vector<uint16_t> tmp(op.dbg_numel);
                CU(cudaMemcpy(tmp.data(), src, op.dbg_numel * 2, cudaMemcpyDeviceToHost));
                for (int64_t i = 0; i < op.dbg_numel; ++i) { const uint32_t u = (uint32_t)tmp[i] << 16; memcpy(&dst[i], &u, 4); }
            } else {
                CU(cudaMemcpy(dst, src, op.dbg_numel * sizeof(float), cudaMemcpyDefault));
            }
        }
        return SBK_OK;
    }
    return fail(SBK_ERR_ARG, "sbk_debug_read: no intermediate named '%s'", name);
}
```

### speech-backbones_b200/csrc/sbk_conv_tc.cu

```cuda
#include "sbk_tc.cuh"

#include <type_traits>

namespace sbk {

namespace tc {

constexpr int ROWS = 2;
constexpr int TPX = 128;
constexpr int NPROD = 256;
constexpr int NTHREADS = NPROD + 64;

template <int GEOM> struct Geo;
template <> struct Geo<G_C3> { static constexpr int HR = ROWS + 2, PXP = TPX + 2, TAPS = 9, KCH = 2, NACC = ROWS; };
template <> struct Geo<G_PW> { static constexpr int HR = ROWS, PXP = TPX, TAPS = 1, KCH = 8, NACC = ROWS; };
template <> struct Geo<G_DOWN> { static constexpr int HR = 2 * ROWS + 1, PXP = 2 * (TPX + 1), TAPS = 9, KCH = 2, NACC = ROWS; };
template <> struct Geo<G_UP> { static constexpr int HR = ROWS + 2, PXP = TPX + 2, TAPS = 16, KCH = 2, NACC = 4 * ROWS; };

template <int K> struct GeoC1 { static constexpr int HR = 1, PXP = ROWS * TPX + 64, TAPS = K, KCH = 2, NACC = ROWS; };
template <> struct Geo<G_C1K3> : GeoC1<3> {};
template <> struct Geo<G_C1K7> : GeoC1<7> {};
template <> struct Geo<G_C1K11> : GeoC1<11> {};

}

using namespace tc;


constexpr int pow2_cols(int c) { return c <= 32 ? 32 : c <= 64 ? 64 : c <= 128 ? 128 : c <= 256 ? 256 : 512; }
template <int GEOM, int NT, bool X3 = false, bool PAIR = false> struct Depth {
    static constexpr int NB = PAIR ? NT / 2 : NT;
    static constexpr int STAGE_BYTES = Geo<GEOM>::KCH * Geo<GEOM>::HR * Geo<GEOM>::PXP * 16 + Geo<GEOM>::TAPS * Geo<GEOM>::KCH * NB * 16;
    static constexpr int SLOT_COLS = Geo<GEOM>::NACC * NT;
    static constexpr int FIT2 = (108 * 1024) / STAGE_BYTES;
    static constexpr int FIT1 = (220 * 1024) / STAGE_BYTES;
    static constexpr bool TMSUM = X3 && (GEOM == G_C3 || GEOM == G_PW);
    static constexpr bool TWO = X3 ? (TMSUM && 4 * NT <= 256 && FIT2 >= 3)
                                   : (FIT2 >= 2 && SLOT_COLS <= 256 && !(GEOM == G_C3 && NT == 128));
    static constexpr int NSLOT = TMSUM ? 2 : (TWO ? (2 * SLOT_COLS <= 256 ? 2 : 1) : (2 * SLOT_COLS <= 512 ? 2 : 1));
    static constexpr int TMEM_COLS = TMSUM ? 4 * NT : pow2_cols(NSLOT * SLOT_COLS);
    static constexpr int STAGES = TWO ? (FIT2 > 4 ? 4 : FIT2) : (FIT1 > 6 ? 6 : FIT1);
    static constexpr int MINB = TWO ? 2 : 1;
    static constexpr size_t SMEM = (size_t)STAGES * STAGE_BYTES + (3 * STAGES + 2 * NSLOT + 2) * 8 + 128 * 4 + 16 + 3 * NT * 4 + 64;
};

template <int GEOM, bool BF16, int NT, bool RES, bool X3, bool PAIR = false, bool RS = false>
__device__ __forceinline__ void conv_tc_body(const ConvTcParams& p) {
    static_assert(!(X3 && BF16), "fp32x3 runs on tf32 operands");
    static_assert(!PAIR || (GEOM == G_C3 && !RES), "CTA pairs: 3x3 convs only");
    static_assert(!RS || (GEOM == G_C3 && NT == 64 && !RES && !PAIR), "row-shared issue order: 64-channel 3x3 convs on single CTAs");
    using G = Geo<GEOM>;
    using D = Depth<GEOM, NT, X3, PAIR>;
    constexpr int NB = D::NB;
    constexpr bool TMSUM = D::TMSUM;
    constexpr bool CHUNKED = X3 && GEOM == G_DOWN;
    const int FLUSH = p.flush > 0 ? p.flush : 6;
    constexpr int STAGES = D::STAGES, NSLOT = D::NSLOT, SLOT_COLS = D::SLOT_COLS;
    constexpr int LAG = STAGES >= 3 ? STAGES - 2 : 0;
    static_assert(STAGES >= 2, "need at least 2 stages");
    constexpr int HR = G::HR, PXP = G::PXP, TAPS = G::TAPS, KCH = G::KCH;
    constexpr int EPC = BF16 ? 8 : 4;
    constexpr int CPS = KCH * EPC;
    constexpr bool OUT16 = BF16 && GEOM != G_C3;
    constexpr int PLANE = HR * PXP * 16;
    constexpr int A_STAGE_BYTES = KCH * PLANE;
    constexpr int B_STAGE_BYTES = TAPS * KCH * NB * 16;
    constexpr bool BULK = GEOM != G_DOWN;
    constexpr bool C1 = geom_is_c1(GEOM);
    constexpr int SPAN = C1 ? ROWS * TPX : TPX;

    extern __shared__ __align__(1024) uint8_t smem[];
    uint8_t* sA = smem;
    uint8_t* sB = sA + STAGES * A_STAGE_BYTES;
    uint64_t* bars = reinterpret_cast<uint64_t*>(sB + STAGES * B_STAGE_BYTES);
    float* s_st = reinterpret_cast<float*>(bars + 3 * STAGES + 2 * NSLOT + 2);
    uint32_t* s_tmem = reinterpret_cast<uint32_t*>(s_st + 128);
    float* s_rg = reinterpret_cast<float*>(s_tmem + 4);

    const int tid = threadIdx.x, warp = tid >> 5, lane = tid & 31;
    const int Cin = p.c0 + p.c1;
    const int HW = p.H * p.W;
    const int ksteps = Cin / CPS;
    const int ksteps_t = X3 ? 2 * ksteps : ksteps;
    const int nchunks = (CHUNKED || TMSUM) ? (ksteps_t + FLUSH - 1) / FLUSH : 1;
    const int wt_w = (GEOM == G_DOWN ? p.Wo : p.W), wt_h = (GEOM == G_DOWN ? p.Ho : p.H);
    const int wtiles = (wt_w + SPAN - 1) / SPAN;
    constexpr int TROWS = PAIR ? 2 * ROWS : ROWS;
    const int mtiles = GEOM == G_PW ? (HW + ROWS * TPX - 1) / (ROWS * TPX) : wtiles * ((wt_h + TROWS - 1) / TROWS);
    const int ntn = p.Cout / NT;
    const int total_tiles = p.B * mtiles * ntn;
    const uint32_t rank = PAIR ? cluster_ctarank() : 0u;
    const int tile0 = PAIR ? (int)(blockIdx.x >> 1) : (int)blockIdx.x, tstep = PAIR ? (int)(gridDim.x >> 1) : (int)gridDim.x;
    auto decode = [&](int t, int& b, int& h0, int& w0, int& n0, int& mt) {
        const int nt = t % ntn; const int r = t / ntn;
        mt = r % mtiles; b = r / mtiles; n0 = nt * NT;
        if (GEOM == G_PW) { w0 = 0; h0 = mt * ROWS; }
        else { w0 = (mt % wtiles) * SPAN; h0 = (mt / wtiles) * TROWS + (int)rank * ROWS; }
    };

    const uint32_t bar0 = smem_u32(bars);
    auto full_b = [&](int s) { return bar0 + 8u * s; };
    auto empty = [&](int s) { return bar0 + 8u * (STAGES + s); };
    auto tfull = [&](int a) { return bar0 + 8u * (2 * STAGES + a); };
    auto tempty = [&](int a) { return bar0 + 8u * (2 * STAGES + NSLOT + a); };
    auto full_a = [&](int s) { return bar0 + 8u * (2 * STAGES + 2 * NSLOT + s); };
    const uint32_t kv_bar = bar0 + 8u * (3 * STAGES + 2 * NSLOT);

    if (tid == 0) {
        for (int s = 0; s < STAGES; ++s) { mbar_init(full_a(s), NPROD / 32); mbar_init(full_b(s), (PAIR && rank == 0) ? 2 : 1); mbar_init(empty(s), 1); }
        for (int a = 0; a < NSLOT; ++a) { mbar_init(tfull(a), 1); mbar_init(tempty(a), (TMSUM ? NPROD / 64 : NPROD / 32) * (PAIR ? 2 : 1)); }
        mbar_init(kv_bar, 1);
        fence_barrier_init();
    }
    if (warp == NPROD / 32) { if constexpr (PAIR) tmem_alloc2(smem_u32(s_tmem), D::TMEM_COLS); else tmem_alloc(smem_u32(s_tmem), D::TMEM_COLS); }
    if (tid < 128) s_st[tid] = 0.f;
    tc_fence_before();
    if constexpr (PAIR) cluster_sync_all(); else __syncthreads();
    tc_fence_after();
    const uint32_t lead_bar0 = PAIR ? mapa_shared(bar0, 0u) : bar0;
    auto tempty_arrive = [&](int a) {
        if constexpr (PAIR) mbar_arrive_cluster(lead_bar0 + 8u * (2 * STAGES + NSLOT + a));
        else mbar_arrive(tempty(a));
    };
    const uint32_t tmem_base = *s_tmem;

    if (warp < NPROD / 32) {
        uint32_t it = 0;
        uint32_t ar = 0;
        for (int t = tile0; t < total_tiles; t += tstep) {
            int b, h0, w0, n0, mt;
            decode(t, b, h0, w0, n0, mt);
            float accr[CHUNKED ? NT : 1];
            int drained = 0;
            auto drain_run = [&]() {
                const int rs = ar % NSLOT;
                mbar_wait(tfull(rs), (ar / NSLOT) & 1);
                tc_fence_after();
                const uint32_t ta = tmem_base + rs * SLOT_COLS + ((uint32_t)((warp & 3) * 32) << 16) + (uint32_t)((warp >> 2) * NT);
#pragma unroll
                for (int cb = 0; cb < (CHUNKED ? NT : 0); cb += 32) {
                    uint32_t r[32];
                    tmem_ld32(ta + cb, r);
                    if (drained == 0) {
#pragma unroll
                        for (int i = 0; i < 32; ++i) accr[cb + i] = __uint_as_float(r[i]);
                    } else {
#pragma unroll
                        for (int i = 0; i < 32; ++i) accr[cb + i] += __uint_as_float(r[i]);
                    }
                }
                tc_fence_before();
                __syncwarp();
                if (lane == 0) tempty_arrive(rs);
                ++ar; ++drained;
            };
            if (!BULK) {
                constexpr int SLOTS = HR * PXP * KCH;
                constexpr int PER = (SLOTS + NPROD - 1) / NPROD;
                uint32_t sl_dst[PER]; long long sl_off[PER]; int sl_chunk[PER]; bool sl_ok[PER];
#pragma unroll
                for (int j = 0; j < PER; ++j) {
                    const int e = tid + j * NPROD;
                    const bool in = e < SLOTS;
                    const int k = in ? e / (HR * PXP) : 0, item = in ? e - k * (HR * PXP) : 0;
                    const int r = item / PXP, q = item - r * PXP;
                    const int par = q / (TPX + 1), i = q - par * (TPX + 1);
                    const int hi = 2 * h0 - 1 + r, wi = par == 0 ? 2 * w0 - 1 + 2 * i : 2 * w0 + 2 * i;
                    const bool ok = in && hi >= 0 && hi < p.H && wi >= 0 && wi < p.W && !(par == 1 && i == TPX);
                    sl_ok[j] = ok; sl_chunk[j] = k;
                    sl_off[j] = (ok ? (long long)(b * p.H + hi) : 0) * 1048576 + (ok ? wi : 0);
                    sl_dst[j] = in ? (uint32_t)(k * PLANE + (r * PXP + q) * 16) : 0xFFFFFFFFu;
                }
                const uint32_t a0 = smem_u32(sA);
                for (int ks = 0; ks < ksteps_t + LAG; ++ks) {
                    if (ks < ksteps_t) {
                        const uint32_t g = it + ks;
                        const int s = g % STAGES;
                        mbar_wait(empty(s), ((g / STAGES) & 1) ^ 1);
                        const int kb = X3 ? ks / 2 : ks;
                        const bool lo = X3 && (ks & 1) == 0;
                        const int ck = kb * KCH;
                        const bool second = ck * EPC >= p.c0;
                        const uint8_t* src = reinterpret_cast<const uint8_t*>(second ? (lo ? p.in1_lo : p.in1) : (lo ? p.in0_lo : p.in0));
                        const int chs = (second ? p.c1 : p.c0) / EPC;
                        const int c0k = second ? ck - p.c0 / EPC : ck;
#pragma unroll
                        for (int j = 0; j < PER; ++j) {
                            if (sl_dst[j] == 0xFFFFFFFFu) continue;
                            const long long row = sl_off[j] / 1048576, wi = sl_off[j] % 1048576;
                            const uint8_t* gp = src + ((row * chs + c0k + sl_chunk[j]) * p.W + wi) * 16;
                            cp_async16(a0 + s * A_STAGE_BYTES + sl_dst[j], gp, sl_ok[j] ? 16u : 0u);
                        }
                    }
                    cp_async_commit();
                    if (ks >= LAG) {
                        cp_async_wait<LAG>();
                        fence_proxy_async();
                        __syncwarp();
                        if (lane == 0) mbar_arrive(full_a((it + ks - LAG) % STAGES));
                        if constexpr (CHUNKED) {
                            while (drained < nchunks) {
                                const int last = (drained + 1) * FLUSH < ksteps_t ? (drained + 1) * FLUSH - 1 : ksteps_t - 1;
                                if (last > ks - LAG) break;
                                drain_run();
                            }
                        }
                    }
                }
                it += ksteps_t;
            }

            const int slot = ar % NSLOT;
            const uint32_t tslot = tmem_base + slot * SLOT_COLS;
            if constexpr (RES) {
                asm volatile("bar.sync 1, 256;" ::: "memory");
                const int cpg = p.Cout / kGroups;
                for (int i = tid; i < NT; i += NPROD) {
                    const int c = n0 + i, g = c / cpg;
                    const double sm_ = p.rgn.stats[(b * kGroups + g) * 2], ss = p.rgn.stats[(b * kGroups + g) * 2 + 1];
                    const double m = sm_ * (double)p.rgn.inv_count;
                    double var = ss * (double)p.rgn.inv_count - m * m;
                    var = var < 0.0 ? 0.0 : var;
                    s_rg[i] = (float)m;
                    s_rg[NT + i] = (float)(1.0 / sqrt(var + 1e-5)) * p.rgn.gamma[c];
                    s_rg[2 * NT + i] = p.rgn.beta[c];
                }
                asm volatile("bar.sync 1, 256;" ::: "memory");
            }
            bool acc_ready = false;
            const int q4 = warp & 3, jrow = warp >> 2;
            const int px = q4 * 32 + lane;
            const int Ho = (GEOM == G_DOWN || GEOM == G_UP) ? p.Ho : p.H, Wo = (GEOM == G_DOWN || GEOM == G_UP) ? p.Wo : p.W;
            const int CHo = p.Cout / 4;
            int ho, wo; bool valid;
            if (GEOM == G_C3 || GEOM == G_DOWN) {
                ho = h0 + jrow; wo = w0 + px;
                valid = ho < Ho && wo < Wo;
            } else if (C1) {
                ho = 0; wo = w0 + jrow * TPX + px;
                valid = wo < Wo;
            } else if (GEOM == G_UP) {
                valid = (h0 + jrow) < p.H && (w0 + px) < p.W;
                ho = 2 * (h0 + jrow); wo = 2 * (w0 + px);
            } else {
                const long long m = (long long)(h0 + jrow) * TPX + px;
                valid = m < HW;
                ho = valid ? (int)(m / p.W) : 0;
                wo = valid ? (int)(m - (long long)ho * p.W) : 0;
            }
            if (!valid) { ho = 0; wo = 0; }
        {
        const int cpg = p.Cout / kGroups;
        const float* bp = p.bias ? p.bias + (long long)b * p.bias_bstride + n0 : nullptr;
        constexpr int NPH = GEOM == G_UP ? 4 : 1;
#pragma unroll 1
        for (int phase = 0; phase < NPH; ++phase) {
        const int ho_p = GEOM == G_UP ? ho + (phase >> 1) : ho;
        const int wo_p = GEOM == G_UP ? wo + (phase & 1) : wo;
        const int acc = GEOM == G_UP ? phase * ROWS + jrow : jrow;
        const float mo = (p.out_mask || RES) ? __ldg(p.mask + (long long)b * p.T + ((long long)wo_p << p.lvl)) : 1.f;
        const long long obase = (((long long)(b * Ho + ho_p) * CHo + n0 / 4) * Wo + wo_p) * 4;
        const long long cstride = (long long)Wo * 4;
        const long long ochunk = OUT16 ? (((long long)(b * Ho + ho_p) * (p.Cout / 8) + n0 / 8) * Wo + wo_p) : 0;
        constexpr bool SIDE = GEOM == G_PW;
        const float* pre_src = RES ? p.rraw : nullptr;
        const bool pre_on = RES && valid && mo != 0.f;
        float4 pre[RES ? 8 : 1];
        if constexpr (RES) {
#pragma unroll
            for (int i = 0; i < 8; ++i)
                pre[i] = pre_on ? __ldg(reinterpret_cast<const float4*>(pre_src + obase + i * cstride)) : make_float4(0.f, 0.f, 0.f, 0.f);
        }
        if constexpr (CHUNKED) {
            while (drained < nchunks) drain_run();
            acc_ready = true;
        }
        if constexpr (TMSUM) {
            const uint32_t trun = tmem_base + ((uint32_t)(q4 * 32) << 16) + (uint32_t)(jrow * NT);
            const uint32_t tsum = trun + 2 * NT;
            for (int c = 0; c < nchunks; ++c, ++ar) {
                mbar_wait(tfull(jrow), ar & 1);
                tc_fence_after();
#pragma unroll 1
                for (int cb = 0; cb < NT; cb += 32) {
                    uint32_t r[32];
                    tmem_ld32(trun + cb, r);
                    if (c > 0) {
                        uint32_t q[32];
                        tmem_ld32(tsum + cb, q);
#pragma unroll
                        for (int i = 0; i < 32; ++i) r[i] = __float_as_uint(__uint_as_float(r[i]) + __uint_as_float(q[i]));
                    }
                    tmem_st32(tsum + cb, r);
                }
                tmem_wait_st();
                tc_fence_before();
                __syncwarp();
                if (lane == 0) tempty_arrive(jrow);
            }
            acc_ready = true;
        }
#pragma unroll (CHUNKED ? NT / 32 : 1)
        for (int cb = 0; cb < NT; cb += 32) {
            if (!acc_ready) {
                mbar_wait(tfull(slot), (ar / NSLOT) & 1);
                tc_fence_after();
                acc_ready = true;
            }
            uint32_t r[32];
            if constexpr (CHUNKED) {
#pragma unroll
                for (int i = 0; i < 32; ++i) r[i] = __float_as_uint(accr[cb + i]);
            } else if constexpr (TMSUM) {
                tmem_ld32(tmem_base + ((uint32_t)(q4 * 32) << 16) + (uint32_t)(2 * NT + acc * NT + cb), r);
            } else {
                tmem_ld32(tslot + ((uint32_t)(q4 * 32) << 16) + (uint32_t)(acc * NT + cb), r);
            }
            float v[32];
#pragma unroll
            for (int i = 0; i < 32; i += 4) {
                const float4 bb = bp ? __ldg(reinterpret_cast<const float4*>(bp + cb + i)) : make_float4(0.f, 0.f, 0.f, 0.f);
                v[i] = __uint_as_float(r[i]) + bb.x; v[i + 1] = __uint_as_float(r[i + 1]) + bb.y;
                v[i + 2] = __uint_as_float(r[i + 2]) + bb.z; v[i + 3] = __uint_as_float(r[i + 3]) + bb.w;
            }
            if constexpr (RES) {
                if (pre_on) {
#pragma unroll
                    for (int i = 0; i < 32; i += 4) {
                        const float rr[4] = {pre[i / 4].x, pre[i / 4].y, pre[i / 4].z, pre[i / 4].w};
#pragma unroll
                        for (int e = 0; e < 4; ++e) {
                            const int cl = cb + i + e;
                            const float xn = (rr[e] - s_rg[cl]) * s_rg[NT + cl] + s_rg[2 * NT + cl];
                            v[i + e] += X3 ? mish_exact(xn) : mish_fast(xn);
                        }
                    }
                    if (cb + 32 < NT) {
#pragma unroll
                        for (int i = 0; i < 8; ++i)
                            pre[i] = __ldg(reinterpret_cast<const float4*>(pre_src + obase + ((cb + 32) / 4 + i) * cstride));
                    }
                }
            } else if (p.addin && valid) {
                if constexpr (OUT16) {
                    const uint4* ap = reinterpret_cast<const uint4*>(p.addin) + ochunk + (long long)(cb / 8) * Wo;
#pragma unroll
                    for (int j = 0; j < 4; ++j) {
                        const uint4 a = __ldg(ap + (long long)j * Wo);
                        v[8 * j + 0] += bf16_lo(a.x); v[8 * j + 1] += bf16_hi(a.x); v[8 * j + 2] += bf16_lo(a.y); v[8 * j + 3] += bf16_hi(a.y);
                        v[8 * j + 4] += bf16_lo(a.z); v[8 * j + 5] += bf16_hi(a.z); v[8 * j + 6] += bf16_lo(a.w); v[8 * j + 7] += bf16_hi(a.w);
                    }
                } else {
                    const float* ap = p.addin + obase + (cb / 4) * cstride;
#pragma unroll
                    for (int i = 0; i < 32; i += 4) {
                        const float4 av = __ldg(reinterpret_cast<const float4*>(ap + (i / 4) * cstride));
                        v[i] += av.x; v[i + 1] += av.y; v[i + 2] += av.z; v[i + 3] += av.w;
                    }
                }
            }
            if (p.out_mask) {
#pragma unroll
                for (int i = 0; i < 32; ++i) v[i] *= mo;
            }
            if (C1 && p.act_out) {
#pragma unroll
                for (int i = 0; i < 32; ++i) v[i] = v[i] > 0.f ? v[i] : v[i] * p.slope;
            }
            if (valid) {
                if constexpr (OUT16) {
                    uint4* op = reinterpret_cast<uint4*>(p.out) + ochunk + (long long)(cb / 8) * Wo;
#pragma unroll
                    for (int j = 0; j < 4; ++j)
                        op[(long long)j * Wo] = make_uint4(pack_bf16x2(v[8 * j], v[8 * j + 1]), pack_bf16x2(v[8 * j + 2], v[8 * j + 3]),
                                                           pack_bf16x2(v[8 * j + 4], v[8 * j + 5]), pack_bf16x2(v[8 * j + 6], v[8 * j + 7]));
                } else {
                    float* op = p.out + obase + (cb / 4) * cstride;
#pragma unroll
                    for (int i = 0; i < 32; i += 4) *reinterpret_cast<float4*>(op + (i / 4) * cstride) = make_float4(v[i], v[i + 1], v[i + 2], v[i + 3]);
                    if (GEOM != G_C3 && p.out_lo) {
                        float* lp = p.out_lo + obase + (cb / 4) * cstride;
#pragma unroll
                        for (int i = 0; i < 32; i += 4) {
                            if (C1 && p.act_out2) {
                                const float sl = p.slope;
                                *reinterpret_cast<float4*>(lp + (i / 4) * cstride) =
                                    make_float4(v[i] > 0.f ? v[i] : v[i] * sl, v[i + 1] > 0.f ? v[i + 1] : v[i + 1] * sl,
                                                v[i + 2] > 0.f ? v[i + 2] : v[i + 2] * sl, v[i + 3] > 0.f ? v[i + 3] : v[i + 3] * sl);
                            } else {
                                *reinterpret_cast<float4*>(lp + (i / 4) * cstride) = corr_chunk(v[i], v[i + 1], v[i + 2], v[i + 3]);
                            }
                        }
                    }
                }
            }
            if (!SIDE && p.ostats) {
                float s8[4], q8[4];
#pragma unroll
                for (int k = 0; k < 4; ++k) {
                    float s = 0.f, q = 0.f;
#pragma unroll
                    for (int i = 0; i < 8; ++i) { const float x = valid ? v[8 * k + i] : 0.f; s += x; q = fmaf(x, x, q); }
                    s8[k] = s; q8[k] = q;
                }
                const int ngrp = cpg == 8 ? 4 : (cpg == 16 ? 2 : 1);
                if (ngrp == 2) { s8[0] += s8[1]; q8[0] += q8[1]; s8[1] = s8[2] + s8[3]; q8[1] = q8[2] + q8[3]; }
                if (ngrp == 1) { s8[0] += s8[1] + s8[2] + s8[3]; q8[0] += q8[1] + q8[2] + q8[3]; }
#pragma unroll
                for (int k = 0; k < 4; ++k) {
                    if (k < ngrp) {
                        float s = s8[k], q = q8[k];
#pragma unroll
                        for (int o = 16; o > 0; o >>= 1) { s += __shfl_xor_sync(0xffffffffu, s, o); q += __shfl_xor_sync(0xffffffffu, q, o); }
                        if (lane == 0) {
                            const int gl = (n0 + cb + k * (32 / ngrp)) / cpg - n0 / cpg;
                            s_st[(warp * 8 + gl) * 2] += s;
                            s_st[(warp * 8 + gl) * 2 + 1] += q;
                        }
                    }
                }
            }
        }
        }
        }
            if constexpr (!CHUNKED && !TMSUM) {
                tc_fence_before();
                __syncwarp();
                if (lane == 0) tempty_arrive(slot);
                ++ar;
            }
            if (GEOM != G_PW && p.ostats) {
                asm volatile("bar.sync 1, 256;" ::: "memory");
                const int cpg = p.Cout / kGroups, gb = n0 / cpg, ng = (NT + cpg - 1) / cpg;
                if (tid < ng * 2) {
                    double tot = 0.0;
#pragma unroll
                    for (int w8 = 0; w8 < NPROD / 32; ++w8) { tot += (double)s_st[w8 * 16 + tid]; s_st[w8 * 16 + tid] = 0.f; }
                    atomicAdd(&p.ostats[((long long)b * kGroups + gb + (tid >> 1)) * 2 + (tid & 1)], tot);
                }
                asm volatile("bar.sync 1, 256;" ::: "memory");
            }
        }
    } else if (warp == NPROD / 32) {
        if (PAIR && rank != 0) {
            const uint32_t lead_full0 = lead_bar0;
            uint32_t it = 0;
            for (int t = tile0; t < total_tiles; t += tstep)
                for (int ks = 0; ks < ksteps_t; ++ks, ++it) {
                    const int s = it % STAGES;
                    mbar_wait(full_b(s), (it / STAGES) & 1);
                    if (lane == 0) mbar_arrive_cluster(lead_full0 + 8u * s);
                    __syncwarp();
                }
        } else {
            const uint32_t idesc = make_idesc<BF16>(PAIR ? 2 * TPX : TPX, NT);
            const uint32_t idesc_c = make_idesc_fmt(0u, PAIR ? 2 * TPX : TPX, NT);
            const uint32_t a0 = smem_u32(sA), b0 = smem_u32(sB);
            constexpr uint32_t D_HI = desc_hi(128);
            auto mma = [&](auto kind16, uint32_t d, uint64_t ad, uint64_t bd, uint32_t idk, uint32_t acc) {
                if constexpr (PAIR) umma2<decltype(kind16)::value>(d, ad, bd, idk, acc);
                else umma<decltype(kind16)::value>(d, ad, bd, idk, acc);
            };
            auto commit = [&](uint32_t bar) { if constexpr (PAIR) umma_commit2(bar); else umma_commit(bar); };
            auto wait_full = [&](uint32_t bar, uint32_t ph) { if constexpr (PAIR) mbar_wait_cluster(bar, ph); else mbar_wait(bar, ph); };
            auto issue_rs = [&](auto kind16, const uint32_t id64, const uint32_t id128, const uint32_t tbase, const uint32_t a_st, const uint32_t b_st, const bool first) {
                constexpr uint32_t BL = 3 * NT;
#pragma unroll
                for (int sx = 0; sx < 3; ++sx) {
                    const uint32_t bs = b_st + (uint32_t)(sx * KCH) * BL;
                    const uint32_t acc0 = (first && sx == 0) ? 0u : 1u;
                    mma(kind16, tbase, desc_pack(a_st + (uint32_t)(0 * PXP + sx), D_HI), desc_pack(bs + 2 * NT, D_HI), id64, acc0);
                    mma(kind16, tbase + NT, desc_pack(a_st + (uint32_t)(3 * PXP + sx), D_HI), desc_pack(bs, D_HI), id64, acc0);
                    mma(kind16, tbase, desc_pack(a_st + (uint32_t)(1 * PXP + sx), D_HI), desc_pack(bs + NT, D_HI), id128, 1u);
                    mma(kind16, tbase, desc_pack(a_st + (uint32_t)(2 * PXP + sx), D_HI), desc_pack(bs, D_HI), id128, 1u);
                }
            };
            const uint32_t idesc_w = make_idesc<BF16>(TPX, 2 * NT), idesc_cw = make_idesc_fmt(0u, TPX, 2 * NT);
            uint32_t it = 0;
            uint32_t ar = 0;
            if constexpr (TMSUM) {
                for (int t = tile0; t < total_tiles; t += tstep) {
                    for (int c = 0; c < nchunks; ++c, ++ar) {
                        const int ks_lo = c * FLUSH, ks_hi = ks_lo + FLUSH < ksteps_t ? ks_lo + FLUSH : ksteps_t;
                        for (int ks = ks_lo; ks < ks_hi; ++ks, ++it) {
                            const int s = it % STAGES;
                            wait_full(full_b(s), (it / STAGES) & 1);
                            tc_fence_after();
                            if constexpr (RS) {
                                if (ks == ks_lo) {
                                    wait_full(tempty(0), (ar & 1) ^ 1);
                                    wait_full(tempty(1), (ar & 1) ^ 1);
                                    tc_fence_after();
                                }
                                const uint32_t a_st = desc_lo(a0 + s * A_STAGE_BYTES, PLANE), b_st = desc_lo(b0 + s * B_STAGE_BYTES, 3 * NT * 16);
                                if (elect_one()) {
                                    if ((ks & 1) == 0) issue_rs(std::true_type{}, idesc_c, idesc_cw, tmem_base, a_st, b_st, ks == ks_lo);
                                    else issue_rs(std::false_type{}, idesc, idesc_w, tmem_base, a_st, b_st, ks == ks_lo);
                                    commit(empty(s));
                                    if (ks == ks_hi - 1) { commit(tfull(0)); commit(tfull(1)); }
                                }
                                __syncwarp();
                                continue;
                            }
                            const uint32_t b_lo = desc_lo(b0 + s * B_STAGE_BYTES, NB * 16);
#pragma unroll
                            for (int j = 0; j < ROWS; ++j) {
                                if (ks == ks_lo) {
                                    wait_full(tempty(j), (ar & 1) ^ 1);
                                    tc_fence_after();
                                }
                                const uint32_t tslot = tmem_base + j * NT;
                                const uint32_t a_lo = desc_lo(a0 + s * A_STAGE_BYTES + (j * PXP) * 16, PLANE);
                                if (elect_one()) {
                                    auto issue = [&](auto kind16, const uint32_t idk) {
#pragma unroll
                                        for (int kk = 0; kk < KCH / 2; ++kk) {
#pragma unroll
                                            for (int tap = 0; tap < TAPS; ++tap) {
                                                const int r = TAPS == 9 ? tap / 3 : 0, sx = TAPS == 9 ? tap % 3 : 0;
                                                mma(kind16, tslot, desc_pack(a_lo + (uint32_t)(kk * 2 * (PLANE / 16) + r * PXP + sx), D_HI),
                                                    desc_pack(b_lo + (uint32_t)((kk * 2 + tap * KCH) * NB), D_HI), idk,
                                                    ((ks - ks_lo) | kk | tap) != 0 ? 1u : 0u);
                                            }
                                        }
                                    };
                                    if ((ks & 1) == 0) issue(std::true_type{}, idesc_c);
                                    else issue(std::false_type{}, idesc);
                                    if (j == ROWS - 1) commit(empty(s));
                                    if (ks == ks_hi - 1) commit(tfull(j));
                                }
                                __syncwarp();
                            }
                        }
                    }
                }
            } else
            for (int t = tile0; t < total_tiles; t += tstep) {
              for (int c = 0; c < nchunks; ++c, ++ar) {
                const int slot = ar % NSLOT;
                const uint32_t tslot = tmem_base + slot * SLOT_COLS;
                wait_full(tempty(slot), ((ar / NSLOT) & 1) ^ 1);
                tc_fence_after();
                const int ks_lo = CHUNKED ? c * FLUSH : 0, ks_hi = CHUNKED ? (ks_lo + FLUSH < ksteps_t ? ks_lo + FLUSH : ksteps_t) : ksteps_t;
                for (int ks = ks_lo; ks < ks_hi; ++ks, ++it) {
                    const int s = it % STAGES;
                    const uint32_t ph = (it / STAGES) & 1;
                    if (!BULK) mbar_wait(full_a(s), ph);
                    wait_full(full_b(s), ph);
                    tc_fence_after();
                    if constexpr (RS) {
                        const uint32_t a_st = desc_lo(a0 + s * A_STAGE_BYTES, PLANE), b_st = desc_lo(b0 + s * B_STAGE_BYTES, 3 * NT * 16);
                        if (elect_one()) {
                            issue_rs(std::integral_constant<bool, BF16>{}, idesc, idesc_w, tslot, a_st, b_st, ks == ks_lo);
                            commit(empty(s));
                            if (ks == ks_hi - 1) commit(tfull(slot));
                        }
                        __syncwarp();
                        continue;
                    }
                    const uint32_t a_lo = desc_lo(a0 + s * A_STAGE_BYTES, PLANE);
                    const uint32_t b_lo = desc_lo(b0 + s * B_STAGE_BYTES, NB * 16);
                    const uint32_t dil = C1 ? (uint32_t)p.dil : 0u;
                    if (elect_one()) {
                      auto issue = [&](auto kind16, const uint32_t idk) {
#pragma unroll
                        for (int kk = 0; kk < KCH / 2; ++kk) {
                            const uint32_t a_k = a_lo + (uint32_t)(kk * 2 * (PLANE / 16)), b_k = b_lo + (uint32_t)(kk * 2 * NB);
                            if (GEOM == G_UP) {
#pragma unroll
                                for (int phase = 0; phase < 4; ++phase) {
                                    const int pph = phase >> 1, pw = phase & 1;
#pragma unroll
                                    for (int t2 = 0; t2 < 4; ++t2) {
                                        const int a = t2 >> 1, bb = t2 & 1;
                                        const int kh = pph ? (a ? 2 : 0) : (a ? 3 : 1), kw = pw ? (bb ? 2 : 0) : (bb ? 3 : 1);
                                        const int dh = pph ? (a ? 0 : 1) : (a ? -1 : 0), dw = pw ? (bb ? 0 : 1) : (bb ? -1 : 0);
                                        const uint64_t bd = desc_pack(b_k + (uint32_t)((kh * 4 + kw) * KCH * NB), D_HI);
#pragma unroll
                                        for (int j = 0; j < ROWS; ++j)
                                            mma(kind16, tslot + (phase * ROWS + j) * NT, desc_pack(a_k + (uint32_t)((1 + j + dh) * PXP + 1 + dw), D_HI), bd,
                                                idk, ((ks - ks_lo) | kk | t2) != 0 ? 1u : 0u);
                                    }
                                }
                            } else {
#pragma unroll
                                for (int tap = 0; tap < TAPS; ++tap) {
                                    const int r = TAPS == 9 ? tap / 3 : 0, sx = TAPS == 9 ? tap % 3 : 0;
                                    const uint64_t bd = desc_pack(b_k + (uint32_t)(tap * KCH * NB), D_HI);
#pragma unroll
                                    for (int j = 0; j < ROWS; ++j) {
                                        const uint32_t aoff = GEOM == G_DOWN ? (uint32_t)((2 * j + r) * PXP + (sx == 1 ? TPX + 1 : (sx == 2 ? 1 : 0)))
                                                            : C1 ? (uint32_t)(j * TPX) + (uint32_t)tap * dil
                                                                 : (uint32_t)((r + j) * PXP + sx);
                                        mma(kind16, tslot + j * NT, desc_pack(a_k + aoff, D_HI), bd, idk, ((ks - ks_lo) | kk | tap) != 0 ? 1u : 0u);
                                    }
                                }
                            }
                        }
                      };
                        if (X3 && (ks & 1) == 0) issue(std::true_type{}, idesc_c);
                        else issue(std::integral_constant<bool, BF16>{}, idesc);
                        commit(empty(s));
                        if (ks == ks_hi - 1) commit(tfull(slot));
                    }
                    __syncwarp();
                }
              }
            }
        }
    } else {
        {
            uint32_t it = 0;
            const float* zero = p.zero_page;
            uint32_t stage_pat[STAGES];
#pragma unroll
            for (int i = 0; i < STAGES; ++i) stage_pat[i] = 0xFFFFFFFFu;
            for (int t = tile0; t < total_tiles; t += tstep) {
                int b, h0, w0, n0, mt;
                decode(t, b, h0, w0, n0, mt);
                const uint8_t* wsrc = reinterpret_cast<const uint8_t*>(p.wpk) + (size_t)b * p.w_bstride_bytes +
                                      (size_t)(PAIR ? 2 * (n0 / NT) + (int)rank : n0 / NT) * ksteps * (X3 ? 2 : 1) * B_STAGE_BYTES;
                for (int ks = 0; ks < ksteps_t; ++ks, ++it) {
                    const int s = it % STAGES;
                    const int kb = X3 ? ks / 2 : ks, var = X3 ? (ks & 1) : 1;
                    if (lane == 0) {
                        mbar_wait(empty(s), ((it / STAGES) & 1) ^ 1);
                        uint32_t a_tx = BULK ? A_STAGE_BYTES : 0;
                        if (BULK && GEOM != G_PW) {
                            const int pad = C1 ? p.pad : 1;
                            const int wlo = w0 - pad < 0 ? 0 : w0 - pad, whi = w0 + SPAN + pad > p.W ? p.W : w0 + SPAN + pad;
                            const int qlo = wlo - (w0 - pad), qhi = qlo + (whi - wlo);
                            const uint32_t pat = (uint32_t)qlo | ((uint32_t)qhi << 16);
                            if (stage_pat[s] != pat) {
                                stage_pat[s] = pat;
                                if (qlo > 0 || qhi < PXP) {
                                    uint8_t* st = sA + s * A_STAGE_BYTES;
                                    for (int k = 0; k < KCH; ++k)
                                        for (int r = 0; r < HR; ++r) {
                                            uint4* rowp = reinterpret_cast<uint4*>(st + k * PLANE + (r * PXP) * 16);
                                            for (int q = 0; q < qlo; ++q) rowp[q] = make_uint4(0u, 0u, 0u, 0u);
                                            for (int q = qhi; q < PXP; ++q) rowp[q] = make_uint4(0u, 0u, 0u, 0u);
                                        }
                                    fence_proxy_async();
                                }
                            }
                            int vrows = 0;
                            for (int r = 0; r < HR; ++r) { const int hi = C1 ? 0 : h0 - 1 + r; vrows += (hi >= 0 && hi < p.H) ? 1 : 0; }
                            a_tx -= (uint32_t)(KCH * vrows * (PXP - (qhi - qlo))) * 16u;
                        }
                        mbar_arrive_expect_tx(full_b(s), B_STAGE_BYTES + a_tx);
                        bulk_g2s(smem_u32(sB + s * B_STAGE_BYTES), wsrc + (size_t)(X3 ? 2 * kb + (var == 0) : ks) * B_STAGE_BYTES,
                                 B_STAGE_BYTES, full_b(s));
                    }
                    __syncwarp();
                    if (BULK && lane < KCH * HR) {
                        const uint32_t a_s = smem_u32(sA) + s * A_STAGE_BYTES;
                        const int k = lane / HR, r = lane - k * HR;
                        const int ck = kb * KCH + k;
                        const bool second = ck * EPC >= p.c0;
                        const uint8_t* src = reinterpret_cast<const uint8_t*>(var == 0 ? (second ? p.in1_lo : p.in0_lo) : (second ? p.in1 : p.in0));
                        const int chs = (second ? p.c1 : p.c0) / EPC;
                        const int cl = second ? ck - p.c0 / EPC : ck;
                        if (GEOM == G_PW) {
                            long long m = (long long)(h0 + r) * TPX;
                            const long long m_hi = m >= HW ? m : (m + TPX < HW ? m + TPX : HW);
                            int q = 0;
                            if (m < m_hi) {
                                int hh = (int)(m / p.W), ww = (int)(m - (long long)hh * p.W);
                                while (m < m_hi) {
                                    const int n = (int)((p.W - ww) < (m_hi - m) ? (p.W - ww) : (m_hi - m));
                                    bulk_g2s(a_s + k * PLANE + (r * PXP + q) * 16,
                                             src + (((long long)(b * p.H + hh) * chs + cl) * p.W + ww) * 16, (uint32_t)n * 16u, full_b(s));
                                    m += n; q += n; ++hh; ww = 0;
                                }
                            }
                            if (q < PXP) bulk_g2s(a_s + k * PLANE + (r * PXP + q) * 16, zero, (uint32_t)(PXP - q) * 16u, full_b(s));
                        } else {
                            const int pad = C1 ? p.pad : 1;
                            const int wlo = w0 - pad < 0 ? 0 : w0 - pad, whi = w0 + SPAN + pad > p.W ? p.W : w0 + SPAN + pad;
                            const int qlo = wlo - (w0 - pad);
                            const int hi = C1 ? 0 : h0 - 1 + r;
                            const uint32_t row_s = a_s + k * PLANE + (r * PXP) * 16;
                            if (hi < 0 || hi >= p.H) bulk_g2s(row_s, zero, PXP * 16u, full_b(s));
                            else bulk_g2s(row_s + qlo * 16, src + (((long long)(b * p.H + hi) * chs + cl) * p.W + wlo) * 16,
                                          (uint32_t)(whi - wlo) * 16u, full_b(s));
                        }
                    }
                }
            }
        }
    }

    if constexpr (PAIR) cluster_sync_all(); else __syncthreads();
    if (warp == NPROD / 32) {
        tc_fence_after();
        if constexpr (PAIR) tmem_dealloc2(tmem_base, D::TMEM_COLS); else tmem_dealloc(tmem_base, D::TMEM_COLS);
    }
}

template <int GEOM, bool BF16, int NT, bool RES = false>
__global__ void __launch_bounds__(NTHREADS, Depth<GEOM, NT, false>::MINB) k_conv_tc(const ConvTcParams p) {
    conv_tc_body<GEOM, BF16, NT, RES, false>(p);
}
template <int GEOM, int NT, bool RES = false>
__global__ void __launch_bounds__(NTHREADS, Depth<GEOM, NT, true>::MINB) k_conv_tc_x3(const ConvTcParams p) {
    conv_tc_body<GEOM, false, NT, RES, true>(p);
}
template <bool BF16>
__global__ void __launch_bounds__(NTHREADS, Depth<G_C3, 64, false>::MINB) k_conv_tc_rs(const ConvTcParams p) {
    conv_tc_body<G_C3, BF16, 64, false, false, false, true>(p);
}
__global__ void __launch_bounds__(NTHREADS, Depth<G_C3, 64, true>::MINB) k_conv_tc_x3_rs(const ConvTcParams p) {
    conv_tc_body<G_C3, false, 64, false, true, false, true>(p);
}
template <bool BF16, int NT>
__global__ void __launch_bounds__(NTHREADS, Depth<G_C3, NT, false, true>::MINB) k_conv_tc_pair(const ConvTcParams p) {
    conv_tc_body<G_C3, BF16, NT, false, false, true>(p);
}
template <int NT>
__global__ void __launch_bounds__(NTHREADS, Depth<G_C3, NT, true, true>::MINB) k_conv_tc_x3_pair(const ConvTcParams p) {
    conv_tc_body<G_C3, false, NT, false, true, true>(p);
}

template <int GEOM, bool BF16, int NT, bool RES = false, bool X3 = false, bool RS = false>
static int launch_tc(const ConvTcParams& p, cudaStream_t s) {
    using D = Depth<GEOM, NT, X3>;
    static DevCache cache;
    const void* fn;
    if constexpr (RS && X3) fn = reinterpret_cast<const void*>(k_conv_tc_x3_rs);
    else if constexpr (RS) fn = reinterpret_cast<const void*>(k_conv_tc_rs<BF16>);
    else if constexpr (X3) fn = reinterpret_cast<const void*>(k_conv_tc_x3<GEOM, NT, RES>);
    else fn = reinterpret_cast<const void*>(k_conv_tc<GEOM, BF16, NT, RES>);
    const int num_sms = cache.get(fn);
    if (num_sms <= 0) return -1;
    int mt;
    if (geom_is_c1(GEOM)) mt = (p.W + ROWS * TPX - 1) / (ROWS * TPX);
    else if (GEOM == G_C3 || GEOM == G_UP) mt = ((p.W + TPX - 1) / TPX) * ((p.H + ROWS - 1) / ROWS);
    else if (GEOM == G_DOWN) mt = ((p.Wo + TPX - 1) / TPX) * ((p.Ho + ROWS - 1) / ROWS);
    else mt = (p.H * p.W + ROWS * TPX - 1) / (ROWS * TPX);
    const long long total = (long long)mt * (p.Cout / NT) * p.B;
    const long long cap = (long long)num_sms * D::MINB;
    const int grid = (int)(total < cap ? total : cap);
    if constexpr (RS && X3) k_conv_tc_x3_rs<<<grid, NTHREADS, D::SMEM, s>>>(p);
    else if constexpr (RS) k_conv_tc_rs<BF16><<<grid, NTHREADS, D::SMEM, s>>>(p);
    else if constexpr (X3) k_conv_tc_x3<GEOM, NT, RES><<<grid, NTHREADS, D::SMEM, s>>>(p);
    else k_conv_tc<GEOM, BF16, NT, RES><<<grid, NTHREADS, D::SMEM, s>>>(p);
    return 1;
}

template <bool BF16, int NT, bool X3>
static int launch_tc_pair(const ConvTcParams& p, cudaStream_t s) {
    using D = Depth<G_C3, NT, X3, true>;
    static DevCache cache;
    const void* fn;
    if constexpr (X3) fn = reinterpret_cast<const void*>(k_conv_tc_x3_pair<NT>);
    else fn = reinterpret_cast<const void*>(k_conv_tc_pair<BF16, NT>);
    const int num_sms = cache.get(fn);
    if (num_sms <= 0) return -1;
    const long long total = (long long)conv_tc_pair_tiles(p.H, p.W) * (p.Cout / NT) * p.B;
    const long long cap = (long long)(num_sms / 2) * D::MINB;
    const unsigned clusters = (unsigned)(total < cap ? total : cap);
    cudaLaunchConfig_t cfg = {};
    cfg.gridDim = dim3(2 * clusters, 1, 1); cfg.blockDim = dim3(NTHREADS, 1, 1); cfg.dynamicSmemBytes = D::SMEM; cfg.stream = s;
    cudaLaunchAttribute at[1];
    at[0].id = cudaLaunchAttributeClusterDimension; at[0].val.clusterDim.x = 2; at[0].val.clusterDim.y = 1; at[0].val.clusterDim.z = 1;
    cfg.attrs = at; cfg.numAttrs = 1;
    cudaError_t e;
    if constexpr (X3) e = cudaLaunchKernelEx(&cfg, k_conv_tc_x3_pair<NT>, p);
    else e = cudaLaunchKernelEx(&cfg, k_conv_tc_pair<BF16, NT>, p);
    return e == cudaSuccess ? 1 : -1;
}

namespace kvk {
constexpr int PX = 128;
constexpr int KCH = 8;
constexpr int XS = KCH * PX * 16;
constexpr int WS = 2 * KCH * 128 * 16;
constexpr int STAGE = XS + WS;
constexpr int STAGES = 3;
constexpr int VT = (PX / 4) * 128 * 16;
constexpr int NPART = 4;
constexpr int PCOLS = PX / NPART;
constexpr int EPW = 4 * NPART;
constexpr int THREADS = (EPW + 3) * 32;
constexpr int RED = 2 * 2 * NPART * 128 * 4;
constexpr int NSLOT = 2, SLOT_COLS = 256;
constexpr int NBARS = 2 * STAGES + 4 * NSLOT;
constexpr size_t SMEM = (size_t)STAGES * STAGE + VT + RED + NBARS * 8 + 16;
static_assert(PCOLS == 32 || PCOLS == 64, "one or two 32-column TMEM loads per thread");
}

template <bool BF16>
__global__ void __launch_bounds__(kvk::THREADS, 1) k_attn_kv(const ConvTcParams p) {
    using namespace kvk;
    constexpr int EPC = BF16 ? 8 : 4;
    extern __shared__ __align__(1024) uint8_t smem[];
    uint8_t* sS = smem;
    uint8_t* vt = sS + STAGES * STAGE;
    float* s_mx = reinterpret_cast<float*>(vt + VT);
    float* s_z = s_mx + 2 * NPART * 128;
    uint64_t* bars = reinterpret_cast<uint64_t*>(s_z + 2 * NPART * 128);
    uint32_t* s_tmem = reinterpret_cast<uint32_t*>(bars + NBARS);

    const int tid = threadIdx.x, warp = tid >> 5, lane = tid & 31;
    const int HW = p.H * p.W;
    const int ksteps = p.c0 / (KCH * EPC);
    const int mtiles = (HW + PX - 1) / PX;
    const int total = p.B * mtiles;
    const uint32_t bar0 = smem_u32(bars);
    auto full = [&](int s) { return bar0 + 8u * s; };
    auto empty = [&](int s) { return bar0 + 8u * (STAGES + s); };
    auto tfull = [&](int a) { return bar0 + 8u * (2 * STAGES + a); };
    auto tempty = [&](int a) { return bar0 + 8u * (2 * STAGES + NSLOT + a); };
    auto pready = [&](int a) { return bar0 + 8u * (2 * STAGES + 2 * NSLOT + a); };
    auto kvdone = [&](int a) { return bar0 + 8u * (2 * STAGES + 3 * NSLOT + a); };

    if (tid == 0) {
        for (int s = 0; s < STAGES; ++s) { mbar_init(full(s), 1); mbar_init(empty(s), 1); }
        for (int a = 0; a < NSLOT; ++a) {
            mbar_init(tfull(a), 1); mbar_init(tempty(a), EPW); mbar_init(pready(a), EPW); mbar_init(kvdone(a), 1);
        }
        fence_barrier_init();
    }
    if (warp == EPW) tmem_alloc(smem_u32(s_tmem), 512);
    tc_fence_before();
    __syncthreads();
    tc_fence_after();
    const uint32_t tmem_base = *s_tmem;

    if (warp < EPW) {
        const int q = warp & 3, part = warp >> 2;
        const int row = q * 32 + lane;
        const int col0 = part * PCOLS;
        const uint32_t lane_sel = (uint32_t)(q * 32) << 16;
        int tl = 0;
        int pb = 0, pmt = 0; float pmd = 0.f;
        auto finish = [&](int ptl) {
            const int pslot = ptl & 1;
            mbar_wait(kvdone(pslot), (ptl >> 1) & 1);
            tc_fence_after();
            if (part == 0) {
                uint32_t r[32];
                tmem_ld32(tmem_base + pslot * SLOT_COLS + lane_sel + 128 + q * 32, r);
                float* pt = p.kv_part + (((long long)pb * mtiles + pmt) * kHeads + q) * kKvPartFloats;
                float z = 0.f;
#pragma unroll
                for (int j = 0; j < NPART; ++j) z += s_z[(pslot * NPART + j) * 128 + row];
                pt[lane] = pmd;
                pt[32 + lane] = z;
#pragma unroll
                for (int i = 0; i < 32; i += 4)
                    *reinterpret_cast<float4*>(&pt[64 + lane * 32 + i]) =
                        make_float4(__uint_as_float(r[i]), __uint_as_float(r[i + 1]), __uint_as_float(r[i + 2]), __uint_as_float(r[i + 3]));
            }
            tc_fence_before();
            __syncwarp();
            if (lane == 0) mbar_arrive(tempty(pslot));
        };
        for (int t = blockIdx.x; t < total; t += gridDim.x, ++tl) {
            const int b = t / mtiles, mt = t - b * mtiles;
            const int slot = tl & 1;
            const uint32_t tq = tmem_base + slot * SLOT_COLS + lane_sel;
            const int nvalid = min(PX, HW - mt * PX) - col0;
            mbar_wait(tfull(slot), (tl >> 1) & 1);
            tc_fence_after();
            uint32_t kr[PCOLS / 32][32];
            float mx = -INFINITY;
#pragma unroll
            for (int c = 0; c < PCOLS / 32; ++c) {
                tmem_ld32(tq + col0 + c * 32, kr[c]);
#pragma unroll
                for (int i = 0; i < 32; ++i) if (c * 32 + i < nvalid) mx = fmaxf(mx, __uint_as_float(kr[c][i]));
            }
            s_mx[(slot * NPART + part) * 128 + row] = mx;
            asm volatile("bar.sync 1, %0;" ::"n"(EPW * 32) : "memory");
            float md = s_mx[(slot * NPART) * 128 + row];
#pragma unroll
            for (int j = 1; j < NPART; ++j) md = fmaxf(md, s_mx[(slot * NPART + j) * 128 + row]);
            float z0 = 0.f, z1 = 0.f, z2 = 0.f, z3 = 0.f;
#pragma unroll
            for (int c = 0; c < PCOLS / 32; ++c) {
#pragma unroll
                for (int i = 0; i < 32; i += 4) {
                    const float e0 = c * 32 + i < nvalid ? __expf(__uint_as_float(kr[c][i]) - md) : 0.f;
                    const float e1 = c * 32 + i + 1 < nvalid ? __expf(__uint_as_float(kr[c][i + 1]) - md) : 0.f;
                    const float e2 = c * 32 + i + 2 < nvalid ? __expf(__uint_as_float(kr[c][i + 2]) - md) : 0.f;
                    const float e3 = c * 32 + i + 3 < nvalid ? __expf(__uint_as_float(kr[c][i + 3]) - md) : 0.f;
                    z0 += e0; z1 += e1; z2 += e2; z3 += e3;
                    kr[c][i] = __float_as_uint(e0); kr[c][i + 1] = __float_as_uint(e1);
                    kr[c][i + 2] = __float_as_uint(e2); kr[c][i + 3] = __float_as_uint(e3);
                }
                tmem_st32(tq + col0 + c * 32, kr[c]);
            }
            s_z[(slot * NPART + part) * 128 + row] = (z0 + z1) + (z2 + z3);
            if (tl > 0) finish(tl - 1);
#pragma unroll
            for (int c = 0; c < PCOLS; c += 32) {
                uint32_t r[32];
                tmem_ld32(tq + 128 + col0 + c, r);
#pragma unroll
                for (int i = 0; i < 32; i += 4)
                    *reinterpret_cast<uint4*>(vt + ((size_t)((col0 + c + i) / 4) * 128 + row) * 16) = make_uint4(r[i], r[i + 1], r[i + 2], r[i + 3]);
            }
            tmem_wait_st();
            fence_proxy_async();
            tc_fence_before();
            __syncwarp();
            if (lane == 0) mbar_arrive(pready(slot));
            pb = b; pmt = mt; pmd = md;
        }
        if (tl > 0) finish(tl - 1);
    } else if (warp == EPW) {
        {
            const uint32_t idesc = make_idesc<BF16>(128, PX);
            const uint32_t s0 = smem_u32(sS);
            constexpr uint32_t D_HI = desc_hi(128);
            uint32_t it = 0;
            int tl = 0;
            for (int t = blockIdx.x; t < total; t += gridDim.x, ++tl) {
                const int slot = tl & 1;
                const uint32_t tslot = tmem_base + slot * SLOT_COLS;
                mbar_wait(tempty(slot), ((tl >> 1) & 1) ^ 1);
                tc_fence_after();
                for (int ks = 0; ks < ksteps; ++ks, ++it) {
                    const int s = it % STAGES;
                    mbar_wait(full(s), (it / STAGES) & 1);
                    tc_fence_after();
                    const uint32_t xs = s0 + s * STAGE;
                    const uint32_t x_lo = desc_lo(xs, PX * 16), k_lo = desc_lo(xs + XS, 128 * 16), v_lo = desc_lo(xs + XS + KCH * 128 * 16, 128 * 16);
                    if (elect_one()) {
#pragma unroll
                        for (int kk = 0; kk < KCH / 2; ++kk) {
                            const uint64_t xd = desc_pack(x_lo + (uint32_t)(kk * 2 * PX), D_HI);
                            umma<BF16>(tslot, desc_pack(k_lo + (uint32_t)(kk * 2 * 128), D_HI), xd, idesc, (ks | kk) != 0 ? 1u : 0u);
                            umma<BF16>(tslot + 128, desc_pack(v_lo + (uint32_t)(kk * 2 * 128), D_HI), xd, idesc, (ks | kk) != 0 ? 1u : 0u);
                        }
                        umma_commit(empty(s));
                        if (ks == ksteps - 1) umma_commit(tfull(slot));
                    }
                    __syncwarp();
                }
            }
        }
    } else if (warp == EPW + 2) {
        {
            const uint32_t idesc2 = make_idesc<false>(128, 128);
            const uint32_t v_lo = desc_lo(smem_u32(vt), 128 * 16);
            constexpr uint32_t D_HI = desc_hi(128);
            int tl = 0;
            for (int t = blockIdx.x; t < total; t += gridDim.x, ++tl) {
                const int slot = tl & 1;
                const uint32_t tslot = tmem_base + slot * SLOT_COLS;
                mbar_wait(pready(slot), (tl >> 1) & 1);
                tc_fence_after();
                if (elect_one()) {
#pragma unroll
                    for (int kk = 0; kk < PX / 8; ++kk)
                        umma_ts_tf32(tslot + 128, tslot + kk * 8, desc_pack(v_lo + (uint32_t)(kk * 2 * 128), D_HI), idesc2, kk != 0 ? 1u : 0u);
                    umma_commit(kvdone(slot));
                }
                __syncwarp();
            }
        }
    } else {
        uint32_t it = 0;
        const int chs = p.c0 / EPC;
        const uint8_t* src = reinterpret_cast<const uint8_t*>(p.in0);
        for (int t = blockIdx.x; t < total; t += gridDim.x) {
            const int b = t / mtiles, mt = t - b * mtiles;
            const int m0 = mt * PX, m_hi = m0 + PX < HW ? m0 + PX : HW;
            const int hh0 = m0 / p.W, ww0 = m0 - hh0 * p.W;
            for (int ks = 0; ks < ksteps; ++ks, ++it) {
                const int s = it % STAGES;
                const uint32_t xs = smem_u32(sS) + s * STAGE;
                if (lane == 0) {
                    mbar_wait(empty(s), ((it / STAGES) & 1) ^ 1);
                    mbar_arrive_expect_tx(full(s), STAGE);
                    bulk_g2s(xs + XS, reinterpret_cast<const uint8_t*>(p.wpk) + (size_t)ks * WS, WS, full(s));
                }
                __syncwarp();
                if (lane < KCH) {
                    const int k = lane, cl = ks * KCH + k;
                    int m = m0, hh = hh0, ww = ww0, qx = 0;
                    while (m < m_hi) {
                        const int n = (p.W - ww) < (m_hi - m) ? (p.W - ww) : (m_hi - m);
                        bulk_g2s(xs + (k * PX + qx) * 16, src + (((long long)(b * p.H + hh) * chs + cl) * p.W + ww) * 16,
                                 (uint32_t)n * 16u, full(s));
                        m += n; qx += n; ++hh; ww = 0;
                    }
                    if (qx < PX) bulk_g2s(xs + (k * PX + qx) * 16, p.zero_page, (uint32_t)(PX - qx) * 16u, full(s));
                }
            }
        }
    }
    __syncthreads();
    if (warp == EPW) {
        tc_fence_after();
        tmem_dealloc(tmem_base, 512);
    }
}

template <bool BF16>
static int launch_attn_kv(const ConvTcParams& p, cudaStream_t s) {
    static DevCache cache;
    const int num_sms = cache.get(reinterpret_cast<const void*>(k_attn_kv<BF16>));
    if (num_sms <= 0) return -1;
    const long long total = (long long)p.B * ((p.H * p.W + kvk::PX - 1) / kvk::PX);
    const int grid = (int)(total < num_sms ? total : num_sms);
    k_attn_kv<BF16><<<grid, kvk::THREADS, kvk::SMEM, s>>>(p);
    return 1;
}
int attn_kv_tile_pixels() { return kvk::PX; }

int conv_tc_ntile(int geom, int Cout) {
    if (geom == G_UP || geom == G_DOWN) return 64;
    if (geom_is_c1(geom)) return Cout % 128 == 0 ? 128 : (Cout % 64 == 0 ? 64 : 32);
    return Cout % 128 == 0 ? 128 : 64;
}
int conv_tc_pair_tiles(int H, int W) { return ((W + TPX - 1) / TPX) * ((H + 2 * ROWS - 1) / (2 * ROWS)); }
int conv_tc_ntile_x3(int geom, int Cout) { return conv_tc_ntile(geom, Cout); }
int conv_tc_taps(int geom) {
    switch (geom) {
        case G_PW: return 1;
        case G_UP: return 16;
        case G_C1K3: return 3;
        case G_C1K7: return 7;
        case G_C1K11: return 11;
        default: return 9;
    }
}
int conv_tc_stage_channels(int geom, int bf16) {
    const int epc = bf16 ? 8 : 4;
    return (geom == G_PW ? Geo<G_PW>::KCH : Geo<G_C3>::KCH) * epc;
}

template <bool BF16>
static int dispatch_conv_tc(const ConvTcParams& p, cudaStream_t s) {
    const int nt = (p.nt == 64 && p.geom == G_C3) ? 64 : conv_tc_ntile(p.geom, p.Cout);
    switch (p.geom) {
        case G_C3:
            if (p.rs) return nt == 64 ? launch_tc<G_C3, BF16, 64, false, false, true>(p, s) : -1;
            if (p.pair) return nt == 128 ? launch_tc_pair<BF16, 128, false>(p, s) : launch_tc_pair<BF16, 64, false>(p, s);
            return nt == 128 ? launch_tc<G_C3, BF16, 128>(p, s) : launch_tc<G_C3, BF16, 64>(p, s);
        case G_PW:
            if (p.epi == EPI_KV) return launch_attn_kv<BF16>(p, s);
            if (p.epi == EPI_RES) return nt == 128 ? launch_tc<G_PW, BF16, 128, true>(p, s) : launch_tc<G_PW, BF16, 64, true>(p, s);
            return nt == 128 ? launch_tc<G_PW, BF16, 128>(p, s) : launch_tc<G_PW, BF16, 64>(p, s);
        case G_DOWN: return launch_tc<G_DOWN, BF16, 64>(p, s);
        case G_UP:   return launch_tc<G_UP, BF16, 64>(p, s);
        default:     return -1;
    }
}

template <int GEOM>
static int dispatch_conv1d(const ConvTcParams& p, cudaStream_t s) {
    if (p.dil < 1 || p.pad < 0 || 2 * p.pad > 64) return -1;
    switch (conv_tc_ntile(p.geom, p.Cout)) {
        case 128: return launch_tc<GEOM, false, 128>(p, s);
        case 64:  return launch_tc<GEOM, false, 64>(p, s);
        default:  return p.Cout % 32 == 0 ? launch_tc<GEOM, false, 32>(p, s) : -1;
    }
}

static int dispatch_conv_tc_x3(const ConvTcParams& p, cudaStream_t s) {
    const int nt = (p.nt == 64 && p.geom == G_C3) ? 64 : conv_tc_ntile(p.geom, p.Cout);
    switch (p.geom) {
        case G_C3:
            if (p.rs) return nt == 64 ? launch_tc<G_C3, false, 64, false, true, true>(p, s) : -1;
            if (p.pair) return nt == 128 ? launch_tc_pair<false, 128, true>(p, s) : launch_tc_pair<false, 64, true>(p, s);
            return nt == 128 ? launch_tc<G_C3, false, 128, false, true>(p, s) : launch_tc<G_C3, false, 64, false, true>(p, s);
        case G_PW:
            if (p.epi == EPI_KV) return launch_attn_kv_x3(p, s);
            if (p.epi == EPI_RES) return nt == 128 ? launch_tc<G_PW, false, 128, true, true>(p, s) : launch_tc<G_PW, false, 64, true, true>(p, s);
            return nt == 128 ? launch_tc<G_PW, false, 128, false, true>(p, s) : launch_tc<G_PW, false, 64, false, true>(p, s);
        case G_DOWN: return launch_tc<G_DOWN, false, 64, false, true>(p, s);
        default:     return launch_tc<G_UP, false, 64, false, true>(p, s);
    }
}

int launch_conv_tc(const ConvTcParams& p, cudaStream_t s) {
    if (geom_is_c1(p.geom)) {
        if (p.x3 || p.bf16) return -1;
        return p.geom == G_C1K3 ? dispatch_conv1d<G_C1K3>(p, s) : p.geom == G_C1K7 ? dispatch_conv1d<G_C1K7>(p, s) : dispatch_conv1d<G_C1K11>(p, s);
    }
    if (p.x3) return p.bf16 ? -1 : dispatch_conv_tc_x3(p, s);
    return p.bf16 ? dispatch_conv_tc<true>(p, s) : dispatch_conv_tc<false>(p, s);
}

}
```

### speech-backbones_b200/csrc/sbk_internal.h

```cpp
#pragma once
#include <cuda_runtime.h>
#include <stdint.h>

namespace sbk {

constexpr int kGroups = 8;
constexpr int kHeads = 4;
constexpr int kDimHead = 32;
constexpr int kAttnHidden = 128;
constexpr int kKvPartFloats = 32 + 32 + 32 * 32;

enum Geom { G_PW = 0, G_C3 = 1, G_DOWN = 2, G_UP = 3, G_C1K3 = 4, G_C1K7 = 5, G_C1K11 = 6 };
__host__ __device__ constexpr bool geom_is_c1(int g) { return g >= G_C1K3; }
enum Pro { PRO_NONE = 0, PRO_MASK = 1, PRO_GN = 2 };
enum Epi { EPI_PLAIN = 0, EPI_RES = 1, EPI_KV = 2 };

struct GnRef {
    const double* stats;
    const float* gamma;
    const float* beta;
    float inv_count;
};

struct IgemmParams {
    int geom;
    const float* in0; const float* in1; int c0, c1;
    int Hin, Win, Hout, Wout;
    int B;
    const float* w; long long w_bstride;
    const float* bias; long long bias_bstride;
    float* out; int Cout;
    int pro;
    const float* mask; int T; int in_lvl;
    GnRef pgn;
    const float* tb; int tb_stride; int tb_per_sample; const int* step;
    int epi;
    double* ostats;
    const float* rraw; GnRef rgn; int out_lvl;
    float* kv_part;
    int out_mask;
};

struct ConvTcParams {
    int geom;
    const void* in0; const void* in1; int c0, c1;
    int H, W, B;
    int Ho, Wo;
    const void* wpk; long long w_bstride_bytes;
    const float* bias; long long bias_bstride;
    float* out; int Cout;
    int epi;
    double* ostats;
    const float* mask; int T; int lvl; int out_mask;
    const float* rraw; GnRef rgn;
    float* kv_part;
    const float* addin;
    const float* zero_page;
    int bf16;
    int nt;
    int dil, pad; float slope; int act_out, act_out2;
    int rs;
    int pair;
    int x3;
    int flush;
    const void* in0_lo; const void* in1_lo;
    float* out_lo;
};

struct GnActParams {
    const float* raw; GnRef gn; const float* tb; int tb_stride; int tb_per_sample; const int* step;
    const float* mask; int T; int lvl;
    float* out; int B, H, W, C; int round_tf32;
    int chw4;
    int out_bf16;
    float* out_lo;
};

struct FirstConvParams {
    const float* mu; const float* xt; const float* spk_s;
    const float* mask;
    const float* w;
    const float* bias;
    float* out; double* ostats;
    int B, H, T, cin, C;
    int chw4;
    const float* w_extra; const int* step; int extra_per_sample_row;
};

struct ResFinalParams {
    const float* h2raw; GnRef gn;
    const float* x;
    const float* mu; const float* xt; const float* spk_s;
    const float* wres; const float* bres; int cin;
    const float* r_extra; const int* step; int extra_per_sample_row;
    const float* mask; int T; int lvl;
    float* out;
    int B, H, W, C;
    int out_mask;
    int chw4;
    int bf16;
    float* out_lo;
};

struct AttnCtxParams {
    const float* kv_part; int mtiles; float* ctx; int B;
};

struct AttnMixParams {
    const float* ctx;
    const float* wq;
    const float* wout;
    const float* bout;
    const float* g;
    float* w_eff;
    float* b_eff;
    int B, C;
    int tc_nt, tc_cps;
    int tc_bf16;
    int tc_x3;
};

struct FinalParams {
    const float* raw; GnRef gn;
    const float* wfin; const float* bfin;
    const float* mask; const float* mu;
    const float* xt_in; float* xt_out;
    const float* const* noise_pp;
    const float4* coef;
    const int* step;
    int mode;
    int B, H, T, C;
    int chw4;
    int exact;
};

struct TimeTableParams {
    const float* t_rows; int rows;
    const float* freqs;
    float pe_scale; int dim;
    const float* w0; const float* b0;
    const float* w2; const float* b2;
    int nproj;
    const float* pw[16]; const float* pb[16]; int pc[16]; int poff[16];
    float* tb; int tb_stride;
};

struct SpkParams {
    const float* spk; const float* w0; const float* b0; const float* w2; const float* b2;
    float* out; int B, E, n_feats;
};

struct CondFoldParams {
    const float* cond;
    const float* w1;
    const float* wres;
    float* w_extra;
    float* r_extra;
    int rows, B, dc, C;
};
int launch_cond_fold(const CondFoldParams& p, cudaStream_t s);

struct DiffMeanParams {
    const float* ref; const float* mean_ref; const float* mask; float* out; float g; int B, H, T;
};
struct ChanStatsParams {
    const float* x; double* stats; int B, H, W, C;
};
struct InGluParams {
    const float* raw; const double* stats; const float* gamma; const float* beta;
    const float* tb;
    const float* mask; int T;
    float* out; int B, H, W, C;
    float* out_lo;
};
struct VcCondParams {
    const double* ysum;
    const float* mask; int Tr; int H;
    const float* wf; const float* bf;
    const float* c;
    const float* freqs; float t; int dim;
    const float* w0; const float* b0; const float* w2; const float* b2;
    float* out;
    int B, dc, use_ref;
};
int launch_diff_mean(const DiffMeanParams& p, cudaStream_t s);
int launch_chan_stats(const ChanStatsParams& p, cudaStream_t s);
int launch_in_glu(const InGluParams& p, cudaStream_t s);
int launch_vc_cond(const VcCondParams& p, cudaStream_t s);

struct PriorExpandParams {
    const float* mu_x;
    const float* w_ceil;
    const float* x_mask;
    const long long* y_len;
    const float* noise_tf;
    float temperature;
    int B, F, Tx, Ty;
    float* mu_y; float* z;
    float* y_mask;
    float* attn;
};
int launch_prior_expand(const PriorExpandParams& p, cudaStream_t s);

struct StepBeginParams { double* stats; int n_doubles; int* step_cur; int* step_next; };

int launch_igemm(const IgemmParams& p, cudaStream_t s);
int launch_first_conv(const FirstConvParams& p, cudaStream_t s);
int launch_conv_tc(const ConvTcParams& p, cudaStream_t s);
int conv_tc_ntile(int geom, int Cout);
int conv_tc_ntile_x3(int geom, int Cout);
int conv_tc_pair_tiles(int H, int W);
int conv_tc_taps(int geom);
int conv_tc_stage_channels(int geom, int bf16);
int launch_gn_act(const GnActParams& p, cudaStream_t s);
int launch_resfinal(const ResFinalParams& p, cudaStream_t s);
int launch_attn_ctx(const AttnCtxParams& p, cudaStream_t s);
int attn_kv_tile_pixels();
int launch_attn_kv_x3(const ConvTcParams& p, cudaStream_t s);
int attn_kv_x3_item_pixels();
int launch_attn_mix(const AttnMixParams& p, cudaStream_t s);
int launch_final(const FinalParams& p, cudaStream_t s);
int launch_time_table(const TimeTableParams& p, cudaStream_t s);
int launch_spk(const SpkParams& p, cudaStream_t s);
int launch_step_begin(const StepBeginParams& p, cudaStream_t s);
int launch_scale_mask(const float* z, const float* mask, float* out, long long n_per_b_row, int B, int H, int T, cudaStream_t s);

__device__ __forceinline__ float tf32_lo(float x) { return x - __uint_as_float(__float_as_uint(x) & 0xFFFFE000u); }

constexpr float kCorrDown = 1.f / 4096.f;
constexpr float kCorrUp = 4096.f;
__device__ __forceinline__ uint32_t f16x2_sat(float e0, float e1) {
    uint32_t d;
    asm("cvt.rn.satfinite.f16x2.f32 %0, %1, %2;" : "=r"(d) : "f"(e1), "f"(e0));
    return d;
}
__device__ __forceinline__ float4 corr_chunk(float x0, float x1, float x2, float x3) {
    return make_float4(__uint_as_float(f16x2_sat(tf32_lo(x0), tf32_lo(x1))), __uint_as_float(f16x2_sat(tf32_lo(x2), tf32_lo(x3))),
                       __uint_as_float(f16x2_sat(x0 * kCorrDown, x1 * kCorrDown)), __uint_as_float(f16x2_sat(x2 * kCorrDown, x3 * kCorrDown)));
}

inline int igemm_mtiles(int geom, int Hout, int Wout, int Hin, int Win) {
    const int TM = 128;
    if (geom == G_UP) return 4 * ((Hin * Win + TM - 1) / TM);
    return (Hout * Wout + TM - 1) / TM;
}

}
```

### speech-backbones_b200/csrc/sbk_tc.cuh

```cuda
#pragma once
#include "sbk_internal.h"

#include <cuda_bf16.h>
#include <math.h>
#include <stdint.h>

namespace sbk {

namespace tc {

__device__ __forceinline__ uint32_t smem_u32(const void* p) { return (uint32_t)__cvta_generic_to_shared(p); }

__device__ __forceinline__ void mbar_init(uint32_t bar, uint32_t count) {
    asm volatile("mbarrier.init.shared::cta.b64 [%0], %1;" ::"r"(bar), "r"(count));
}
__device__ __forceinline__ void mbar_arrive(uint32_t bar) {
    asm volatile("mbarrier.arrive.shared::cta.b64 _, [%0];" ::"r"(bar) : "memory");
}
__device__ __forceinline__ void mbar_arrive_expect_tx(uint32_t bar, uint32_t bytes) {
    asm volatile("mbarrier.arrive.expect_tx.shared::cta.b64 _, [%0], %1;" ::"r"(bar), "r"(bytes) : "memory");
}
__device__ __forceinline__ bool mbar_try_wait(uint32_t bar, uint32_t parity) {
    uint32_t ok;
    asm volatile(
        "{\n\t.reg .pred p;\n\t"
        "mbarrier.try_wait.parity.shared::cta.b64 p, [%1], %2;\n\t"
        "selp.u32 %0, 1, 0, p;\n\t}"
        : "=r"(ok) : "r"(bar), "r"(parity) : "memory");
    return ok != 0;
}
__device__ __forceinline__ void mbar_wait(uint32_t bar, uint32_t parity) {
    uint32_t spins = 0;
    while (!mbar_try_wait(bar, parity)) {
        if (++spins > (1u << 24)) __trap();
    }
}
__device__ __forceinline__ void fence_barrier_init() { asm volatile("fence.mbarrier_init.release.cluster;" ::: "memory"); }
__device__ __forceinline__ void fence_proxy_async() { asm volatile("fence.proxy.async.shared::cta;" ::: "memory"); }
__device__ __forceinline__ void tc_fence_before() { asm volatile("tcgen05.fence::before_thread_sync;" ::: "memory"); }
__device__ __forceinline__ void tc_fence_after() { asm volatile("tcgen05.fence::after_thread_sync;" ::: "memory"); }

__device__ __forceinline__ void bulk_g2s(uint32_t dst, const void* src, uint32_t bytes, uint32_t bar) {
    asm volatile("cp.async.bulk.shared::cluster.global.mbarrier::complete_tx::bytes [%0], [%1], %2, [%3];"
                 ::"r"(dst), "l"(src), "r"(bytes), "r"(bar) : "memory");
}

__device__ __forceinline__ void tmem_alloc(uint32_t dst_smem, uint32_t ncols) {
    asm volatile("tcgen05.alloc.cta_group::1.sync.aligned.shared::cta.b32 [%0], %1;" ::"r"(dst_smem), "r"(ncols) : "memory");
    asm volatile("tcgen05.relinquish_alloc_permit.cta_group::1.sync.aligned;" ::: "memory");
}
__device__ __forceinline__ void tmem_dealloc(uint32_t taddr, uint32_t ncols) {
    asm volatile("tcgen05.dealloc.cta_group::1.sync.aligned.b32 %0, %1;" ::"r"(taddr), "r"(ncols) : "memory");
}

__device__ __forceinline__ uint64_t make_desc(uint32_t saddr, uint32_t lbo_bytes, uint32_t sbo_bytes) {
    uint64_t d = 0;
    d |= (uint64_t)((saddr >> 4) & 0x3FFF);
    d |= (uint64_t)((lbo_bytes >> 4) & 0x3FFF) << 16;
    d |= (uint64_t)((sbo_bytes >> 4) & 0x3FFF) << 32;
    d |= (uint64_t)1 << 46;
    return d;
}

__device__ __forceinline__ uint32_t desc_lo(uint32_t saddr, uint32_t lbo_bytes) {
    return ((saddr >> 4) & 0x3FFFu) | (((lbo_bytes >> 4) & 0x3FFFu) << 16);
}
__device__ __forceinline__ constexpr uint32_t desc_hi(uint32_t sbo_bytes) { return ((sbo_bytes >> 4) & 0x3FFFu) | (1u << 14); }
__device__ __forceinline__ uint64_t desc_pack(uint32_t lo, uint32_t hi) {
    uint64_t d;
    asm("mov.b64 %0, {%1, %2};" : "=l"(d) : "r"(lo), "r"(hi));
    return d;
}

__device__ __forceinline__ bool elect_one() {
    uint32_t pred = 0;
    asm volatile("{\n\t.reg .b32 rx;\n\t.reg .pred px;\n\telect.sync rx|px, 0xffffffff;\n\t@px mov.s32 %0, 1;\n\t}" : "+r"(pred));
    return pred != 0;
}

__device__ __forceinline__ uint32_t make_idesc_fmt(uint32_t fmt, int M, int N) {
    uint32_t d = 0;
    d |= 1u << 4;
    d |= fmt << 7;
    d |= fmt << 10;
    d |= (uint32_t)(N >> 3) << 17;
    d |= (uint32_t)(M >> 4) << 24;
    return d;
}
template <bool BF16>
__device__ __forceinline__ uint32_t make_idesc(int M, int N) { return make_idesc_fmt(BF16 ? 1u : 2u, M, N); }

template <bool BF16>
__device__ __forceinline__ void umma(uint32_t tmem_d, uint64_t adesc, uint64_t bdesc, uint32_t idesc, uint32_t accumulate) {
    if (BF16) {
        asm volatile("{\n\t.reg .pred p;\n\tsetp.ne.b32 p, %4, 0;\n\t"
                     "tcgen05.mma.cta_group::1.kind::f16 [%0], %1, %2, %3, p;\n\t}"
                     ::"r"(tmem_d), "l"(adesc), "l"(bdesc), "r"(idesc), "r"(accumulate) : "memory");
    } else {
        asm volatile("{\n\t.reg .pred p;\n\tsetp.ne.b32 p, %4, 0;\n\t"
                     "tcgen05.mma.cta_group::1.kind::tf32 [%0], %1, %2, %3, p;\n\t}"
                     ::"r"(tmem_d), "l"(adesc), "l"(bdesc), "r"(idesc), "r"(accumulate) : "memory");
    }
}
__device__ __forceinline__ void umma_commit(uint32_t bar) {
    asm volatile("tcgen05.commit.cta_group::1.mbarrier::arrive::one.shared::cluster.b64 [%0];" ::"r"(bar) : "memory");
}


__device__ __forceinline__ uint32_t cluster_ctarank() { uint32_t r; asm volatile("mov.u32 %0, %%cluster_ctarank;" : "=r"(r)); return r; }
__device__ __forceinline__ void cluster_sync_all() {
    asm volatile("barrier.cluster.arrive.release.aligned;" ::: "memory");
    asm volatile("barrier.cluster.wait.acquire.aligned;" ::: "memory");
}
__device__ __forceinline__ uint32_t mapa_shared(uint32_t saddr, uint32_t rank) {
    uint32_t r;
    asm volatile("mapa.shared::cluster.u32 %0, %1, %2;" : "=r"(r) : "r"(saddr), "r"(rank));
    return r;
}
__device__ __forceinline__ void mbar_arrive_cluster(uint32_t cluster_addr) {
    asm volatile("mbarrier.arrive.relaxed.cluster.shared::cluster.b64 _, [%0];" ::"r"(cluster_addr) : "memory");
}
__device__ __forceinline__ void mbar_wait_cluster(uint32_t bar, uint32_t parity) { mbar_wait(bar, parity); }
__device__ __forceinline__ void tmem_alloc2(uint32_t dst_smem, uint32_t ncols) {
    asm volatile("tcgen05.alloc.cta_group::2.sync.aligned.shared::cta.b32 [%0], %1;" ::"r"(dst_smem), "r"(ncols) : "memory");
    asm volatile("tcgen05.relinquish_alloc_permit.cta_group::2.sync.aligned;" ::: "memory");
}
__device__ __forceinline__ void tmem_dealloc2(uint32_t taddr, uint32_t ncols) {
    asm volatile("tcgen05.dealloc.cta_group::2.sync.aligned.b32 %0, %1;" ::"r"(taddr), "r"(ncols) : "memory");
}
template <bool K16>
__device__ __forceinline__ void umma2(uint32_t tmem_d, uint64_t adesc, uint64_t bdesc, uint32_t idesc, uint32_t accumulate) {
    if (K16) {
        asm volatile("{\n\t.reg .pred p;\n\tsetp.ne.b32 p, %4, 0;\n\t"
                     "tcgen05.mma.cta_group::2.kind::f16 [%0], %1, %2, %3, p;\n\t}"
                     ::"r"(tmem_d), "l"(adesc), "l"(bdesc), "r"(idesc), "r"(accumulate) : "memory");
    } else {
        asm volatile("{\n\t.reg .pred p;\n\tsetp.ne.b32 p, %4, 0;\n\t"
                     "tcgen05.mma.cta_group::2.kind::tf32 [%0], %1, %2, %3, p;\n\t}"
                     ::"r"(tmem_d), "l"(adesc), "l"(bdesc), "r"(idesc), "r"(accumulate) : "memory");
    }
}
__device__ __forceinline__ void umma_commit2(uint32_t bar) {
    asm volatile("tcgen05.commit.cta_group::2.mbarrier::arrive::one.shared::cluster.multicast::cluster.b64 [%0], %1;"
                 ::"r"(bar), "h"((uint16_t)3) : "memory");
}

__device__ __forceinline__ void tmem_ld32(uint32_t taddr, uint32_t (&r)[32]) {
    asm volatile(
        "tcgen05.ld.sync.aligned.32x32b.x32.b32 "
        "{%0, %1, %2, %3, %4, %5, %6, %7, %8, %9, %10, %11, %12, %13, %14, %15, "
        "%16, %17, %18, %19, %20, %21, %22, %23, %24, %25, %26, %27, %28, %29, %30, %31}, [%32];"
        : "=r"(r[0]), "=r"(r[1]), "=r"(r[2]), "=r"(r[3]), "=r"(r[4]), "=r"(r[5]), "=r"(r[6]), "=r"(r[7]),
          "=r"(r[8]), "=r"(r[9]), "=r"(r[10]), "=r"(r[11]), "=r"(r[12]), "=r"(r[13]), "=r"(r[14]), "=r"(r[15]),
          "=r"(r[16]), "=r"(r[17]), "=r"(r[18]), "=r"(r[19]), "=r"(r[20]), "=r"(r[21]), "=r"(r[22]), "=r"(r[23]),
          "=r"(r[24]), "=r"(r[25]), "=r"(r[26]), "=r"(r[27]), "=r"(r[28]), "=r"(r[29]), "=r"(r[30]), "=r"(r[31])
        : "r"(taddr) : "memory");
    asm volatile("tcgen05.wait::ld.sync.aligned;" ::: "memory");
}

__device__ __forceinline__ void tmem_st32(uint32_t taddr, const uint32_t (&r)[32]) {
    asm volatile(
        "tcgen05.st.sync.aligned.32x32b.x32.b32 [%0], "
        "{%1, %2, %3, %4, %5, %6, %7, %8, %9, %10, %11, %12, %13, %14, %15, %16, "
        "%17, %18, %19, %20, %21, %22, %23, %24, %25, %26, %27, %28, %29, %30, %31, %32};"
        :: "r"(taddr), "r"(r[0]), "r"(r[1]), "r"(r[2]), "r"(r[3]), "r"(r[4]), "r"(r[5]), "r"(r[6]), "r"(r[7]),
           "r"(r[8]), "r"(r[9]), "r"(r[10]), "r"(r[11]), "r"(r[12]), "r"(r[13]), "r"(r[14]), "r"(r[15]),
           "r"(r[16]), "r"(r[17]), "r"(r[18]), "r"(r[19]), "r"(r[20]), "r"(r[21]), "r"(r[22]), "r"(r[23]),
           "r"(r[24]), "r"(r[25]), "r"(r[26]), "r"(r[27]), "r"(r[28]), "r"(r[29]), "r"(r[30]), "r"(r[31])
        : "memory");
}
__device__ __forceinline__ void tmem_wait_st() { asm volatile("tcgen05.wait::st.sync.aligned;" ::: "memory"); }

__device__ __forceinline__ void umma_ts_tf32(uint32_t tmem_d, uint32_t tmem_a, uint64_t bdesc, uint32_t idesc, uint32_t accumulate) {
    asm volatile("{\n\t.reg .pred p;\n\tsetp.ne.b32 p, %4, 0;\n\t"
                 "tcgen05.mma.cta_group::1.kind::tf32 [%0], [%1], %2, %3, p;\n\t}"
                 ::"r"(tmem_d), "r"(tmem_a), "l"(bdesc), "r"(idesc), "r"(accumulate) : "memory");
}

__device__ __forceinline__ float mish_fast(float x) {
    const float n = __expf(fminf(x, 20.f));
    const float a = n * (n + 2.f);
    return x > 20.f ? x : x * __fdividef(a, a + 2.f);
}



__device__ __forceinline__ float mish_exact(float x) {
    const float n = expf(fminf(x, 20.f));
    const float a = n * (n + 2.f);
    return x > 20.f ? x : x * (a / (a + 2.f));
}

__device__ __forceinline__ float bf16_lo(uint32_t u) { return __uint_as_float(u << 16); }
__device__ __forceinline__ float bf16_hi(uint32_t u) { return __uint_as_float(u & 0xFFFF0000u); }
__device__ __forceinline__ uint32_t pack_bf16x2(float lo, float hi) {
    uint32_t d;
    asm("cvt.rn.bf16x2.f32 %0, %1, %2;" : "=r"(d) : "f"(hi), "f"(lo));
    return d;
}

__device__ __forceinline__ void cp_async16(uint32_t dst, const void* src, uint32_t src_bytes) {
    asm volatile("cp.async.cg.shared.global [%0], [%1], 16, %2;" ::"r"(dst), "l"(src), "r"(src_bytes) : "memory");
}
__device__ __forceinline__ void cp_async_commit() { asm volatile("cp.async.commit_group;" ::: "memory"); }
template <int N> __device__ __forceinline__ void cp_async_wait() { asm volatile("cp.async.wait_group %0;" ::"n"(N) : "memory"); }


}

struct DevCache {
    static constexpr int MAXDEV = 64;
    int sms[MAXDEV] = {};
    int get(const void* fn) {
        int dev = 0;
        if (cudaGetDevice(&dev) != cudaSuccess || dev < 0 || dev >= MAXDEV) return -1;
        if (sms[dev] == 0) {
            if (cudaFuncSetAttribute(fn, cudaFuncAttributeMaxDynamicSharedMemorySize, 227 * 1024) != cudaSuccess) return -1;
            int n = 0;
            if (cudaDeviceGetAttribute(&n, cudaDevAttrMultiProcessorCount, dev) != cudaSuccess || n <= 0) return -1;
            sms[dev] = n;
        }
        return sms[dev];
    }
};

}
```

Before: 25700.

## Load downsample conv tiles via strided TMA and merge upsample tap MMAs

Replaces the per-thread cp.async gather for the stride-2 downsample conv with 5D tensor-map TMA loads. An element stride of 2 splits odd and even columns into separate smem regions, and the loads complete on the existing full barrier, so the extra full_a barrier and the producer lag logic go away. Separately, the transposed upsample conv reorders its packed weight taps so that taps shared across output phases are contiguous. It then issues 11 wider MMAs (N=4·NT or 2·NT) instead of 16 per row, with the accumulator layout changed to row-major by phase. This adds host-side tensor map encoding per plan, a driver entry-point dependency, and a larger params struct passed as __grid_constant__.

New measurement: 25840, median of 6. Within noise of the previous version (+0.6%).

```diff
diff --git a/speech-backbones_b200/csrc/sbk_api.cu b/speech-backbones_b200/csrc/sbk_api.cu
--- a/speech-backbones_b200/csrc/sbk_api.cu
+++ b/speech-backbones_b200/csrc/sbk_api.cu
@@ -393,8 +393,8 @@
 static int pack_tc_up(sbk_handle* h, const std::string& src, const std::string& key, int C, bool bf16) {
     std::vector<float> w((size_t)C * C * 16), m((size_t)C * C * 16);
     CU(cudaMemcpy(w.data(), h->raw[src], w.size() * sizeof(float), cudaMemcpyDeviceToHost));
-    for (int ci = 0; ci < C; ++ci) for (int co = 0; co < C; ++co) for (int t = 0; t < 16; ++t)
-        m[((size_t)co * C + ci) * 16 + t] = w[((size_t)ci * C + co) * 16 + t];
+    for (int ci = 0; ci < C; ++ci) for (int co = 0; co < C; ++co) for (int sl = 0; sl < 16; ++sl)
+        m[((size_t)co * C + ci) * 16 + sl] = w[((size_t)ci * C + co) * 16 + kUpTapOfSlot[sl]];
     return pack_tc_host(h, m, key, C, C, G_UP, bf16);
 }
 static int pack_tc_host(sbk_handle* h, const std::vector<float>& hs, const std::string& key, int cout, int cin, int geom, bool bf16, int nt_override) {
@@ -408,8 +408,9 @@
         for (int k = 0; k < KCHK; ++k) for (int col = 0; col < NT; ++col) for (int e = 0; e < EPC; ++e) {
             const int co = nt * NT + col, ci = ks * CPS + k * EPC + e;
             const float w = hs[((size_t)co * cin + ci) * taps + tap];
+            const int in_stage = geom == G_UP ? k * taps + tap : tap * KCHK + k;
             if (x3) {
-                const size_t ih = ((((((size_t)nt * ksteps + ks) * 2) * taps + tap) * KCHK + k) * NT + col) * EPC + e;
+                const size_t ih = (((((size_t)nt * ksteps + ks) * 2) * taps * KCHK + in_stage) * NT + col) * EPC + e;
                 const uint32_t uh = f32_to_tf32_rna(w);
                 float fh; memcpy(&fh, &uh, 4);
                 reinterpret_cast<uint32_t*>(hd.data())[ih] = uh;
@@ -418,7 +419,7 @@
                 cc[4 + e] = f32_to_f16_rn((w - fh) * 4096.f);
                 continue;
             }
-            const size_t idx = (((((size_t)nt * ksteps + ks) * taps + tap) * KCHK + k) * NT + col) * EPC + e;
+            const size_t idx = ((((size_t)nt * ksteps + ks) * taps * KCHK + in_stage) * NT + col) * EPC + e;
             if (bf16) reinterpret_cast<uint16_t*>(hd.data())[idx] = f32_to_bf16_rn(w);
             else reinterpret_cast<uint32_t*>(hd.data())[idx] = f32_to_tf32_rna(w);
         }
@@ -860,10 +861,12 @@
             push(op, out, npix(lvl) * a.c);
         }
     };
+    bool maps_ok = true;
     auto resample = [&](int geom, const std::string& pre, int lvl_in, int lvl_out, const float* x, int C, float* out) {
         if (use_tc && C % tc_cps3 == 0 && C % 64 == 0) {
             Op op = tc_conv(pre + ".out", geom, pre + ".conv.wtc", pre + ".conv.bias", lvl_in, x, C, nullptr, 0, C, out, nullptr);
             op.tc.Ho = Hs[lvl_out]; op.tc.Wo = Ws[lvl_out]; op.tc.lvl = lvl_out; op.tc.out_mask = 1;
+            if (geom == G_DOWN && conv_tc_encode_down_maps(op.tc) != 0) maps_ok = false;
             op.flops = 2.0 * npix(lvl_out) * C * C * (geom == G_UP ? 4.0 : 9.0);
             op.bytes = osz * C * (npix(lvl_in) + npix(lvl_out));
             push(op, out, npix(lvl_out) * C);
@@ -919,6 +922,10 @@
         p.coef = pl.coef; p.step = pl.step_cur; p.B = B; p.H = H0; p.T = T; p.C = C1; p.chw4 = use_tc ? 1 : 0; p.exact = x3 ? 1 : 0;
         pl.final_op = (int)pl.ops.size();
         push(op, nullptr, 0);
+    }
+    if (!maps_ok) {
+        free_plan(h, false);
+        return fail(SBK_ERR_CUDA, "cuTensorMapEncodeTiled failed for a Downsample input (B=%d, T=%d)", B, T);
     }
     pl.launches_per_step = (int)pl.ops.size() + 1;
     return SBK_OK;
diff --git a/speech-backbones_b200/csrc/sbk_conv_tc.cu b/speech-backbones_b200/csrc/sbk_conv_tc.cu
--- a/speech-backbones_b200/csrc/sbk_conv_tc.cu
+++ b/speech-backbones_b200/csrc/sbk_conv_tc.cu
@@ -1,4 +1,6 @@
 #include "sbk_tc.cuh"
+
+#include <string.h>
 
 #include <type_traits>
 
@@ -14,7 +16,7 @@
 template <int GEOM> struct Geo;
 template <> struct Geo<G_C3> { static constexpr int HR = ROWS + 2, PXP = TPX + 2, TAPS = 9, KCH = 2, NACC = ROWS; };
 template <> struct Geo<G_PW> { static constexpr int HR = ROWS, PXP = TPX, TAPS = 1, KCH = 8, NACC = ROWS; };
-template <> struct Geo<G_DOWN> { static constexpr int HR = 2 * ROWS + 1, PXP = 2 * (TPX + 1), TAPS = 9, KCH = 2, NACC = ROWS; };
+template <> struct Geo<G_DOWN> { static constexpr int HR = 2 * ROWS + 1, EVEN = TPX + 8, PXP = EVEN + TPX, TAPS = 9, KCH = 2, NACC = ROWS; };
 template <> struct Geo<G_UP> { static constexpr int HR = ROWS + 2, PXP = TPX + 2, TAPS = 16, KCH = 2, NACC = 4 * ROWS; };
 
 template <int K> struct GeoC1 { static constexpr int HR = 1, PXP = ROWS * TPX + 64, TAPS = K, KCH = 2, NACC = ROWS; };
@@ -41,7 +43,7 @@
     static constexpr int TMEM_COLS = TMSUM ? 4 * NT : pow2_cols(NSLOT * SLOT_COLS);
     static constexpr int STAGES = TWO ? (FIT2 > 4 ? 4 : FIT2) : (FIT1 > 6 ? 6 : FIT1);
     static constexpr int MINB = TWO ? 2 : 1;
-    static constexpr size_t SMEM = (size_t)STAGES * STAGE_BYTES + (3 * STAGES + 2 * NSLOT + 2) * 8 + 128 * 4 + 16 + 3 * NT * 4 + 64;
+    static constexpr size_t SMEM = (size_t)STAGES * STAGE_BYTES + (2 * STAGES + 2 * NSLOT + 2) * 8 + 128 * 4 + 16 + 3 * NT * 4 + 64;
 };
 
 template <int GEOM, bool BF16, int NT, bool RES, bool X3, bool PAIR = false, bool RS = false>
@@ -56,7 +58,6 @@
     constexpr bool CHUNKED = X3 && GEOM == G_DOWN;
     const int FLUSH = p.flush > 0 ? p.flush : 6;
     constexpr int STAGES = D::STAGES, NSLOT = D::NSLOT, SLOT_COLS = D::SLOT_COLS;
-    constexpr int LAG = STAGES >= 3 ? STAGES - 2 : 0;
     static_assert(STAGES >= 2, "need at least 2 stages");
     constexpr int HR = G::HR, PXP = G::PXP, TAPS = G::TAPS, KCH = G::KCH;
     constexpr int EPC = BF16 ? 8 : 4;
@@ -65,7 +66,9 @@
     constexpr int PLANE = HR * PXP * 16;
     constexpr int A_STAGE_BYTES = KCH * PLANE;
     constexpr int B_STAGE_BYTES = TAPS * KCH * NB * 16;
-    constexpr bool BULK = GEOM != G_DOWN;
+    constexpr bool TMA = GEOM == G_DOWN;
+    constexpr int EVEN = TMA ? Geo<G_DOWN>::EVEN : 0;
+    constexpr uint32_t TMA_TX = (uint32_t)(KCH * HR * (2 * TPX + 1) * 16);
     constexpr bool C1 = geom_is_c1(GEOM);
     constexpr int SPAN = C1 ? ROWS * TPX : TPX;
 
@@ -73,7 +76,7 @@
     uint8_t* sA = smem;
     uint8_t* sB = sA + STAGES * A_STAGE_BYTES;
     uint64_t* bars = reinterpret_cast<uint64_t*>(sB + STAGES * B_STAGE_BYTES);
-    float* s_st = reinterpret_cast<float*>(bars + 3 * STAGES + 2 * NSLOT + 2);
+    float* s_st = reinterpret_cast<float*>(bars + 2 * STAGES + 2 * NSLOT + 2);
     uint32_t* s_tmem = reinterpret_cast<uint32_t*>(s_st + 128);
     float* s_rg = reinterpret_cast<float*>(s_tmem + 4);
 
@@ -103,11 +106,10 @@
     auto empty = [&](int s) { return bar0 + 8u * (STAGES + s); };
     auto tfull = [&](int a) { return bar0 + 8u * (2 * STAGES + a); };
     auto tempty = [&](int a) { return bar0 + 8u * (2 * STAGES + NSLOT + a); };
-    auto full_a = [&](int s) { return bar0 + 8u * (2 * STAGES + 2 * NSLOT + s); };
-    const uint32_t kv_bar = bar0 + 8u * (3 * STAGES + 2 * NSLOT);
+    const uint32_t kv_bar = bar0 + 8u * (2 * STAGES + 2 * NSLOT);
 
     if (tid == 0) {
-        for (int s = 0; s < STAGES; ++s) { mbar_init(full_a(s), NPROD / 32); mbar_init(full_b(s), (PAIR && rank == 0) ? 2 : 1); mbar_init(empty(s), 1); }
+        for (int s = 0; s < STAGES; ++s) { mbar_init(full_b(s), (PAIR && rank == 0) ? 2 : 1); mbar_init(empty(s), 1); }
         for (int a = 0; a < NSLOT; ++a) { mbar_init(tfull(a), 1); mbar_init(tempty(a), (TMSUM ? NPROD / 64 : NPROD / 32) * (PAIR ? 2 : 1)); }
         mbar_init(kv_bar, 1);
         fence_barrier_init();
@@ -125,7 +127,6 @@
     const uint32_t tmem_base = *s_tmem;
 
     if (warp < NPROD / 32) {
-        uint32_t it = 0;
         uint32_t ar = 0;
         for (int t = tile0; t < total_tiles; t += tstep) {
             int b, h0, w0, n0, mt;
@@ -154,61 +155,6 @@
                 if (lane == 0) tempty_arrive(rs);
                 ++ar; ++drained;
             };
-            if (!BULK) {
-                constexpr int SLOTS = HR * PXP * KCH;
-                constexpr int PER = (SLOTS + NPROD - 1) / NPROD;
-                uint32_t sl_dst[PER]; long long sl_off[PER]; int sl_chunk[PER]; bool sl_ok[PER];
-#pragma unroll
-                for (int j = 0; j < PER; ++j) {
-                    const int e = tid + j * NPROD;
-                    const bool in = e < SLOTS;
-                    const int k = in ? e / (HR * PXP) : 0, item = in ? e - k * (HR * PXP) : 0;
-                    const int r = item / PXP, q = item - r * PXP;
-                    const int par = q / (TPX + 1), i = q - par * (TPX + 1);
-                    const int hi = 2 * h0 - 1 + r, wi = par == 0 ? 2 * w0 - 1 + 2 * i : 2 * w0 + 2 * i;
-                    const bool ok = in && hi >= 0 && hi < p.H && wi >= 0 && wi < p.W && !(par == 1 && i == TPX);
-                    sl_ok[j] = ok; sl_chunk[j] = k;
-                    sl_off[j] = (ok ? (long long)(b * p.H + hi) : 0) * 1048576 + (ok ? wi : 0);
-                    sl_dst[j] = in ? (uint32_t)(k * PLANE + (r * PXP + q) * 16) : 0xFFFFFFFFu;
-                }
-                const uint32_t a0 = smem_u32(sA);
-                for (int ks = 0; ks < ksteps_t + LAG; ++ks) {
-                    if (ks < ksteps_t) {
-                        const uint32_t g = it + ks;
-                        const int s = g % STAGES;
-                        mbar_wait(empty(s), ((g / STAGES) & 1) ^ 1);
-                        const int kb = X3 ? ks / 2 : ks;
-                        const bool lo = X3 && (ks & 1) == 0;
-                        const int ck = kb * KCH;
-                        const bool second = ck * EPC >= p.c0;
-                        const uint8_t* src = reinterpret_cast<const uint8_t*>(second ? (lo ? p.in1_lo : p.in1) : (lo ? p.in0_lo : p.in0));
-                        const int chs = (second ? p.c1 : p.c0) / EPC;
-                        const int c0k = second ? ck - p.c0 / EPC : ck;
-#pragma unroll
-                        for (int j = 0; j < PER; ++j) {
-                            if (sl_dst[j] == 0xFFFFFFFFu) continue;
-                            const long long row = sl_off[j] / 1048576, wi = sl_off[j] % 1048576;
-                            const uint8_t* gp = src + ((row * chs + c0k + sl_chunk[j]) * p.W + wi) * 16;
-                            cp_async16(a0 + s * A_STAGE_BYTES + sl_dst[j], gp, sl_ok[j] ? 16u : 0u);
-                        }
-                    }
-                    cp_async_commit();
-                    if (ks >= LAG) {
-                        cp_async_wait<LAG>();
-                        fence_proxy_async();
-                        __syncwarp();
-                        if (lane == 0) mbar_arrive(full_a((it + ks - LAG) % STAGES));
-                        if constexpr (CHUNKED) {
-                            while (drained < nchunks) {
-                                const int last = (drained + 1) * FLUSH < ksteps_t ? (drained + 1) * FLUSH - 1 : ksteps_t - 1;
-                                if (last > ks - LAG) break;
-                                drain_run();
-                            }
-                        }
-                    }
-                }
-                it += ksteps_t;
-            }
 
             const int slot = ar % NSLOT;
             const uint32_t tslot = tmem_base + slot * SLOT_COLS;
@@ -257,7 +203,7 @@
         for (int phase = 0; phase < NPH; ++phase) {
         const int ho_p = GEOM == G_UP ? ho + (phase >> 1) : ho;
         const int wo_p = GEOM == G_UP ? wo + (phase & 1) : wo;
-        const int acc = GEOM == G_UP ? phase * ROWS + jrow : jrow;
+        const int acc = GEOM == G_UP ? jrow * 4 + phase : jrow;
         const float mo = (p.out_mask || RES) ? __ldg(p.mask + (long long)b * p.T + ((long long)wo_p << p.lvl)) : 1.f;
         const long long obase = (((long long)(b * Ho + ho_p) * CHo + n0 / 4) * Wo + wo_p) * 4;
         const long long cstride = (long long)Wo * 4;
@@ -476,6 +422,8 @@
                 }
             };
             const uint32_t idesc_w = make_idesc<BF16>(TPX, 2 * NT), idesc_cw = make_idesc_fmt(0u, TPX, 2 * NT);
+            const uint32_t idesc_2 = idesc_w, idesc_4 = make_idesc<BF16>(TPX, 4 * NT);
+            const uint32_t idesc_c2 = idesc_cw, idesc_c4 = make_idesc_fmt(0u, TPX, 4 * NT);
             uint32_t it = 0;
             uint32_t ar = 0;
             if constexpr (TMSUM) {
@@ -545,7 +493,6 @@
                 for (int ks = ks_lo; ks < ks_hi; ++ks, ++it) {
                     const int s = it % STAGES;
                     const uint32_t ph = (it / STAGES) & 1;
-                    if (!BULK) mbar_wait(full_a(s), ph);
                     wait_full(full_b(s), ph);
                     tc_fence_after();
                     if constexpr (RS) {
@@ -562,25 +509,25 @@
                     const uint32_t b_lo = desc_lo(b0 + s * B_STAGE_BYTES, NB * 16);
                     const uint32_t dil = C1 ? (uint32_t)p.dil : 0u;
                     if (elect_one()) {
-                      auto issue = [&](auto kind16, const uint32_t idk) {
+                      auto issue = [&](auto kind16, const uint32_t idk, const uint32_t idk_up2, const uint32_t idk_up4) {
 #pragma unroll
                         for (int kk = 0; kk < KCH / 2; ++kk) {
                             const uint32_t a_k = a_lo + (uint32_t)(kk * 2 * (PLANE / 16)), b_k = b_lo + (uint32_t)(kk * 2 * NB);
                             if (GEOM == G_UP) {
-#pragma unroll
-                                for (int phase = 0; phase < 4; ++phase) {
-                                    const int pph = phase >> 1, pw = phase & 1;
-#pragma unroll
-                                    for (int t2 = 0; t2 < 4; ++t2) {
-                                        const int a = t2 >> 1, bb = t2 & 1;
-                                        const int kh = pph ? (a ? 2 : 0) : (a ? 3 : 1), kw = pw ? (bb ? 2 : 0) : (bb ? 3 : 1);
-                                        const int dh = pph ? (a ? 0 : 1) : (a ? -1 : 0), dw = pw ? (bb ? 0 : 1) : (bb ? -1 : 0);
-                                        const uint64_t bd = desc_pack(b_k + (uint32_t)((kh * 4 + kw) * KCH * NB), D_HI);
-#pragma unroll
-                                        for (int j = 0; j < ROWS; ++j)
-                                            mma(kind16, tslot + (phase * ROWS + j) * NT, desc_pack(a_k + (uint32_t)((1 + j + dh) * PXP + 1 + dw), D_HI), bd,
-                                                idk, ((ks - ks_lo) | kk | t2) != 0 ? 1u : 0u);
-                                    }
+                                struct UpMma { int slot, n, phase, dh, dw; };
+                                constexpr UpMma ups[11] = {{0, 4, 0, 0, 0}, {4, 2, 0, -1, 0}, {6, 2, 2, 1, 0},
+                                                           {8, 1, 0, 0, -1}, {9, 1, 2, 0, -1}, {10, 1, 1, 0, 1}, {11, 1, 3, 0, 1},
+                                                           {12, 1, 0, -1, -1}, {13, 1, 1, -1, 1}, {14, 1, 2, 1, -1}, {15, 1, 3, 1, 1}};
+                                const uint32_t bu = desc_lo(b0 + s * B_STAGE_BYTES, TAPS * NB * 16);
+#pragma unroll
+                                for (int u = 0; u < 11; ++u) {
+                                    const uint32_t idu = ups[u].n == 4 ? idk_up4 : ups[u].n == 2 ? idk_up2 : idk;
+                                    const uint64_t bd = desc_pack(bu + (uint32_t)(ups[u].slot * NB), D_HI);
+#pragma unroll
+                                    for (int j = 0; j < ROWS; ++j)
+                                        mma(kind16, tslot + (j * 4 + ups[u].phase) * NT,
+                                            desc_pack(a_k + (uint32_t)((1 + j + ups[u].dh) * PXP + 1 + ups[u].dw), D_HI), bd, idu,
+                                            ((ks - ks_lo) | kk | u) != 0 ? 1u : 0u);
                                 }
                             } else {
 #pragma unroll
@@ -589,7 +536,7 @@
                                     const uint64_t bd = desc_pack(b_k + (uint32_t)(tap * KCH * NB), D_HI);
 #pragma unroll
                                     for (int j = 0; j < ROWS; ++j) {
-                                        const uint32_t aoff = GEOM == G_DOWN ? (uint32_t)((2 * j + r) * PXP + (sx == 1 ? TPX + 1 : (sx == 2 ? 1 : 0)))
+                                        const uint32_t aoff = GEOM == G_DOWN ? (uint32_t)((2 * j + r) * PXP + (sx == 1 ? EVEN : (sx == 2 ? 1 : 0)))
                                                             : C1 ? (uint32_t)(j * TPX) + (uint32_t)tap * dil
                                                                  : (uint32_t)((r + j) * PXP + sx);
                                         mma(kind16, tslot + j * NT, desc_pack(a_k + aoff, D_HI), bd, idk, ((ks - ks_lo) | kk | tap) != 0 ? 1u : 0u);
@@ -598,8 +545,8 @@
                             }
                         }
                       };
-                        if (X3 && (ks & 1) == 0) issue(std::true_type{}, idesc_c);
-                        else issue(std::integral_constant<bool, BF16>{}, idesc);
+                        if (X3 && (ks & 1) == 0) issue(std::true_type{}, idesc_c, idesc_c2, idesc_c4);
+                        else issue(std::integral_constant<bool, BF16>{}, idesc, idesc_2, idesc_4);
                         commit(empty(s));
                         if (ks == ks_hi - 1) commit(tfull(slot));
                     }
@@ -625,8 +572,8 @@
                     const int kb = X3 ? ks / 2 : ks, var = X3 ? (ks & 1) : 1;
                     if (lane == 0) {
                         mbar_wait(empty(s), ((it / STAGES) & 1) ^ 1);
-                        uint32_t a_tx = BULK ? A_STAGE_BYTES : 0;
-                        if (BULK && GEOM != G_PW) {
+                        uint32_t a_tx = TMA ? TMA_TX : A_STAGE_BYTES;
+                        if (GEOM != G_PW && !TMA) {
                             const int pad = C1 ? p.pad : 1;
                             const int wlo = w0 - pad < 0 ? 0 : w0 - pad, whi = w0 + SPAN + pad > p.W ? p.W : w0 + SPAN + pad;
                             const int qlo = wlo - (w0 - pad), qhi = qlo + (whi - wlo);
@@ -653,7 +600,7 @@
                                  B_STAGE_BYTES, full_b(s));
                     }
                     __syncwarp();
-                    if (BULK && lane < KCH * HR) {
+                    if (lane < KCH * HR) {
                         const uint32_t a_s = smem_u32(sA) + s * A_STAGE_BYTES;
                         const int k = lane / HR, r = lane - k * HR;
                         const int ck = kb * KCH + k;
@@ -661,7 +608,14 @@
                         const uint8_t* src = reinterpret_cast<const uint8_t*>(var == 0 ? (second ? p.in1_lo : p.in0_lo) : (second ? p.in1 : p.in0));
                         const int chs = (second ? p.c1 : p.c0) / EPC;
                         const int cl = second ? ck - p.c0 / EPC : ck;
-                        if (GEOM == G_PW) {
+                        if constexpr (TMA) {
+                            const CUtensorMap* map = &p.down_map[var == 0 ? 2 : 0];
+                            const int hi = 2 * h0 - 1 + r;
+                            const uint32_t row_s = a_s + k * PLANE + (r * PXP) * 16;
+                            tma_g2s_5d(row_s, map, 0, 2 * w0 - 1, cl, hi, b, full_b(s));
+                            tma_g2s_5d(row_s + TPX * 16, map + 1, 0, 2 * w0 + 2 * TPX - 1, cl, hi, b, full_b(s));
+                            tma_g2s_5d(row_s + EVEN * 16, map, 0, 2 * w0, cl, hi, b, full_b(s));
+                        } else if (GEOM == G_PW) {
                             long long m = (long long)(h0 + r) * TPX;
                             const long long m_hi = m >= HW ? m : (m + TPX < HW ? m + TPX : HW);
                             int q = 0;
@@ -699,11 +653,11 @@
 }
 
 template <int GEOM, bool BF16, int NT, bool RES = false>
-__global__ void __launch_bounds__(NTHREADS, Depth<GEOM, NT, false>::MINB) k_conv_tc(const ConvTcParams p) {
+__global__ void __launch_bounds__(NTHREADS, Depth<GEOM, NT, false>::MINB) k_conv_tc(const __grid_constant__ ConvTcParams p) {
     conv_tc_body<GEOM, BF16, NT, RES, false>(p);
 }
 template <int GEOM, int NT, bool RES = false>
-__global__ void __launch_bounds__(NTHREADS, Depth<GEOM, NT, true>::MINB) k_conv_tc_x3(const ConvTcParams p) {
+__global__ void __launch_bounds__(NTHREADS, Depth<GEOM, NT, true>::MINB) k_conv_tc_x3(const __grid_constant__ ConvTcParams p) {
     conv_tc_body<GEOM, false, NT, RES, true>(p);
 }
 template <bool BF16>
@@ -1017,6 +971,37 @@
     if (geom_is_c1(geom)) return Cout % 128 == 0 ? 128 : (Cout % 64 == 0 ? 64 : 32);
     return Cout % 128 == 0 ? 128 : 64;
 }
+int conv_tc_encode_down_maps(ConvTcParams& p) {
+    using Encode = CUresult (*)(CUtensorMap*, CUtensorMapDataType, cuuint32_t, void*, const cuuint64_t*, const cuuint64_t*,
+                                const cuuint32_t*, const cuuint32_t*, CUtensorMapInterleave, CUtensorMapSwizzle,
+                                CUtensorMapL2promotion, CUtensorMapFloatOOBfill);
+    static const Encode encode = []() -> Encode {
+        void* fn = nullptr;
+        cudaDriverEntryPointQueryResult q;
+        if (cudaGetDriverEntryPoint("cuTensorMapEncodeTiled", &fn, cudaEnableDefault, &q) != cudaSuccess || q != cudaDriverEntryPointSuccess)
+            return nullptr;
+        return reinterpret_cast<Encode>(fn);
+    }();
+    if (!encode || p.geom != G_DOWN || p.c1 != 0) return -1;
+    const int epc = p.bf16 ? 8 : 4;
+    const cuuint64_t chs = (cuuint64_t)(p.c0 / epc);
+    const cuuint64_t dims[5] = {4, (cuuint64_t)p.W, chs, (cuuint64_t)p.H, (cuuint64_t)p.B};
+    const cuuint64_t strides[4] = {16, 16ull * p.W, 16ull * p.W * chs, 16ull * p.W * chs * p.H};
+    const cuuint32_t box_main[5] = {4, 2 * TPX, 1, 1, 1}, box_tail[5] = {4, 1, 1, 1, 1};
+    const cuuint32_t es_main[5] = {1, 2, 1, 1, 1}, es_tail[5] = {1, 1, 1, 1, 1};
+    const void* src[2] = {p.in0, p.in0_lo};
+    memset(p.down_map, 0, sizeof(p.down_map));
+    for (int i = 0; i < (p.x3 ? 2 : 1); ++i) {
+        for (int j = 0; j < 2; ++j) {
+            const CUresult r = encode(&p.down_map[2 * i + j], CU_TENSOR_MAP_DATA_TYPE_UINT32, 5, const_cast<void*>(src[i]), dims, strides,
+                                      j == 0 ? box_main : box_tail, j == 0 ? es_main : es_tail, CU_TENSOR_MAP_INTERLEAVE_NONE,
+                                      CU_TENSOR_MAP_SWIZZLE_NONE, CU_TENSOR_MAP_L2_PROMOTION_L2_128B, CU_TENSOR_MAP_FLOAT_OOB_FILL_NONE);
+            if (r != CUDA_SUCCESS) return -1;
+        }
+    }
+    return 0;
+}
+
 int conv_tc_pair_tiles(int H, int W) { return ((W + TPX - 1) / TPX) * ((H + 2 * ROWS - 1) / (2 * ROWS)); }
 int conv_tc_ntile_x3(int geom, int Cout) { return conv_tc_ntile(geom, Cout); }
 int conv_tc_taps(int geom) {
diff --git a/speech-backbones_b200/csrc/sbk_internal.h b/speech-backbones_b200/csrc/sbk_internal.h
--- a/speech-backbones_b200/csrc/sbk_internal.h
+++ b/speech-backbones_b200/csrc/sbk_internal.h
@@ -1,4 +1,5 @@
 #pragma once
+#include <cuda.h>
 #include <cuda_runtime.h>
 #include <stdint.h>
 
@@ -65,6 +66,7 @@
     int flush;
     const void* in0_lo; const void* in1_lo;
     float* out_lo;
+    CUtensorMap down_map[4];
 };
 
 struct GnActParams {
@@ -207,7 +209,9 @@
 int launch_igemm(const IgemmParams& p, cudaStream_t s);
 int launch_first_conv(const FirstConvParams& p, cudaStream_t s);
 int launch_conv_tc(const ConvTcParams& p, cudaStream_t s);
+constexpr int kUpTapOfSlot[16] = {5, 6, 9, 10, 13, 14, 1, 2, 7, 11, 4, 8, 15, 12, 3, 0};
 int conv_tc_ntile(int geom, int Cout);
+int conv_tc_encode_down_maps(ConvTcParams& p);
 int conv_tc_ntile_x3(int geom, int Cout);
 int conv_tc_pair_tiles(int H, int W);
 int conv_tc_taps(int geom);
diff --git a/speech-backbones_b200/csrc/sbk_tc.cuh b/speech-backbones_b200/csrc/sbk_tc.cuh
--- a/speech-backbones_b200/csrc/sbk_tc.cuh
+++ b/speech-backbones_b200/csrc/sbk_tc.cuh
@@ -199,12 +199,10 @@
     return d;
 }
 
-__device__ __forceinline__ void cp_async16(uint32_t dst, const void* src, uint32_t src_bytes) {
-    asm volatile("cp.async.cg.shared.global [%0], [%1], 16, %2;" ::"r"(dst), "l"(src), "r"(src_bytes) : "memory");
-}
-__device__ __forceinline__ void cp_async_commit() { asm volatile("cp.async.commit_group;" ::: "memory"); }
-template <int N> __device__ __forceinline__ void cp_async_wait() { asm volatile("cp.async.wait_group %0;" ::"n"(N) : "memory"); }
-
+__device__ __forceinline__ void tma_g2s_5d(uint32_t dst, const CUtensorMap* map, int c0, int c1, int c2, int c3, int c4, uint32_t bar) {
+    asm volatile("cp.async.bulk.tensor.5d.shared::cluster.global.tile.mbarrier::complete_tx::bytes [%0], [%1, {%2, %3, %4, %5, %6}], [%7];"
+                 ::"r"(dst), "l"(map), "r"(c0), "r"(c1), "r"(c2), "r"(c3), "r"(c4), "r"(bar) : "memory");
+}
 
 }
 
```
